# facebookresearch/robust-dynrf

Hardware: AMD Instinct MI355X
Metric: training rays/sec (Nvidia Balloon1, configs/Nvidia.txt, static+dynamic TensorVMSplit) (higher is better)
Workload: dtype f32; 1 GPU; BASELINE.json configs[1]: Nvidia Balloon1, configs/Nvidia.txt, 4096 rays/iter/GPU, 1xMI355X per rank, static+dynamic TensorVMSplit; one step = 5 dynamic + 5 static forward passes, scene-flow MLP, induced flow/disparity, per-frame depth loss, distortion loss, compositor, factor regularisers, full backward, Adam; config=nvidia, stage=stage0, samples_per_ray=115, global_batch=4096, rays_per_gpu=4096, parallelism=ray-sharded dp1, ranks=1, dead_work=executed (work the reference also computes although nothing consumes it)

## Files before the change

### include/rodynrf.h

```cpp
#ifndef RODYNRF_H
#define RODYNRF_H
#include <stddef.h>
#include <stdint.h>

#ifdef __cplusplus
extern "C" {
#endif

#define RDRF_ABI_VERSION 6

typedef void* rdrf_stream_t;

enum { RDRF_RAY_NDC = 0, RDRF_RAY_CONTRACT = 1, RDRF_RAY_OTHER = 2 };
enum { RDRF_ACT_RELU = 0, RDRF_ACT_SOFTPLUS = 1 };
enum { RDRF_HEAD_MLP_FEA = 0, RDRF_HEAD_MLP_FEA_TIMEEMBEDDING = 1 };
enum { RDRF_SCATTER_RAY = 0, RDRF_SCATTER_SORTED = 1, RDRF_SCATTER_AUTO = 2, RDRF_SCATTER_SORTED_PLAIN = 3 };

typedef struct {
  float* plane[3];
  float* line[3];
  int C[3];
  int H[3], W[3];
  int L[3];
  int sH[3], sW[3];
} RdrfVM;

typedef struct {
  float aabb[6];
  float distance_scale;
  float weight_thres;
  float density_shift;
  int act;
  int ray_type;
  int static_head;
} RdrfFieldCfg;

typedef struct {
  RdrfVM density, app;
  float* basis;
  float *w1, *b1;
  float *w2, *b2;
  float *w3, *b3;
  const float* packed_fwd;
  const float* packed_bwd;
} RdrfStaticParams;

typedef struct {
  RdrfVM density, blending, app;
  float* basis;
  float *rw1, *rb1;
  float *rw2, *rb2;
  float *rwv, *rbv;
  float *l1w, *l1b;
  float *l2w, *l2b;
  float *l3w, *l3b;
  float *l4w, *l4b;
  float *l5w, *l5b;
  float *dw1, *db1, *dw2, *db2;
  float *bw1, *bb1, *bw2, *bb2;
  float *sfw[4], *sfb[4];
  const float* packed_fwd;
  const float* packed_bwd;
} RdrfDynamicParams;

int rdrf_abi_version(void);
const char* rdrf_last_error(void);

size_t rdrf_workspace_bytes(int N, int S);
size_t rdrf_forward_workspace_bytes(int N, int S);
size_t rdrf_saved_bytes(int kind, int N, int S);
#define RDRF_SAVE_NO_APP 1
size_t rdrf_saved_bytes_ex(int kind, int N, int S, int flags);
size_t rdrf_saved_row_bytes(int phase);

int rdrf_generate_rays(const int64_t* ids, const float* poses9, const float* focal, int N, int T,
                       int H, int W, int ndc, float near, float* rays, rdrf_stream_t stream);
int rdrf_generate_rays_bwd(const int64_t* ids, const float* poses9, const float* focal, int N,
                           int T, int H, int W, int ndc, float near, const float* grad_rays,
                           float* grad_poses9, float* grad_focal, rdrf_stream_t stream);

int rdrf_generate_rays_uv(const int64_t* ids, const float* uv, int view_shift, const float* poses9,
                          const float* focal, int N, int T, int H, int W, int ndc, float near, float* rays,
                          rdrf_stream_t stream);
int rdrf_generate_rays_uv_bwd(const int64_t* ids, const float* uv, int view_shift, const float* poses9,
                              const float* focal, int N, int T, int H, int W, int ndc, float near,
                              const float* grad_rays, float* grad_poses9, float* grad_focal,
                              rdrf_stream_t stream);

int rdrf_sample_ndc(const float* rays, int N, int S, float near, float far, const float* jitter,
                    const float aabb_host[6], float* xyz, float* z, uint8_t* valid,
                    rdrf_stream_t stream);
int rdrf_sample_contract(const float* rays, int N, int S, float near, float far,
                         const float* jitter_inner, const float* jitter_outer, float* xyz,
                         float* z, uint8_t* valid, rdrf_stream_t stream);
int rdrf_sample_bwd(const float* rays, const float* z, int N, int S, int ray_type,
                    const float* grad_xyz, float* grad_rays, rdrf_stream_t stream);

int rdrf_static_fwd(const RdrfStaticParams* P, const RdrfFieldCfg* cfg, const float* rays,
                    const float* ts, const float* xyz, const float* z, const uint8_t* valid, int N,
                    int S, float* rgb, float* sigma, float* weight, float* dists, void* saved,
                    size_t saved_bytes, void* ws, size_t ws_bytes, rdrf_stream_t stream);
int rdrf_static_fwd_ex(const RdrfStaticParams* P, const RdrfFieldCfg* cfg, const float* rays,
                       const float* ts, const float* xyz, const float* z, const uint8_t* valid, int N,
                       int S, float* rgb, float* sigma, float* weight, float* dists, void* saved,
                       size_t saved_bytes, void* ws, size_t ws_bytes, rdrf_stream_t stream, int flags);
int rdrf_static_bwd(const RdrfStaticParams* P, const RdrfFieldCfg* cfg, const float* rays,
                    const float* ts, const float* xyz, const float* z, const uint8_t* valid, int N,
                    int S, const float* g_rgb, const float* g_sigma, const float* g_weight,
                    const float* g_dists, const RdrfStaticParams* G, float* g_xyz, float* g_z,
                    float* g_rays, void* saved, size_t saved_bytes, void* ws, size_t ws_bytes,
                    rdrf_stream_t stream);

int rdrf_dynamic_fwd(const RdrfDynamicParams* P, const RdrfFieldCfg* cfg, const float* rays,
                     const float* ts, const float* xyz, const float* z, const uint8_t* valid,
                     int N, int S, float* blending, float* weight, float* xyz_prime, float* rgb,
                     float* sigma, float* dists, void* saved, size_t saved_bytes, void* ws,
                     size_t ws_bytes, rdrf_stream_t stream);
int rdrf_dynamic_fwd_ex(const RdrfDynamicParams* P, const RdrfFieldCfg* cfg, const float* rays,
                        const float* ts, const float* xyz, const float* z, const uint8_t* valid,
                        int N, int S, float* blending, float* weight, float* xyz_prime, float* rgb,
                        float* sigma, float* dists, void* saved, size_t saved_bytes, void* ws,
                        size_t ws_bytes, rdrf_stream_t stream, int flags);
int rdrf_dynamic_bwd(const RdrfDynamicParams* P, const RdrfFieldCfg* cfg, const float* rays,
                     const float* ts, const float* xyz, const float* z, const uint8_t* valid,
                     int N, int S, const float* g_blending, const float* g_weight,
                     const float* g_xyz_prime, const float* g_rgb, const float* g_sigma,
                     const float* g_dists, const RdrfDynamicParams* G, float* g_xyz, float* g_z,
                     float* g_rays, void* saved, size_t saved_bytes, void* ws, size_t ws_bytes,
                     rdrf_stream_t stream);

size_t rdrf_features_saved_bytes(int dynamic, int M);
size_t rdrf_features_workspace_bytes(int M);
size_t rdrf_features_bwd_workspace_bytes(int M);
int rdrf_static_features_fwd(const RdrfStaticParams* P, const RdrfFieldCfg* cfg, const float* xn, int M,
                             float* density, float* app, void* saved, size_t saved_bytes, void* ws,
                             size_t ws_bytes, rdrf_stream_t stream);
int rdrf_static_features_bwd(const RdrfStaticParams* P, const RdrfFieldCfg* cfg, const float* xn, int M,
                             const float* g_density, const float* g_app, const RdrfStaticParams* G,
                             float* g_xn, void* saved, size_t saved_bytes, void* ws, size_t ws_bytes,
                             rdrf_stream_t stream);
int rdrf_dynamic_features_fwd(const RdrfDynamicParams* P, const RdrfFieldCfg* cfg, const float* x,
                              const float* t, int M, int x_is_normalized, float* density, float* blending,
                              float* app, float* xyz_prime, void* saved, size_t saved_bytes, void* ws,
                              size_t ws_bytes, rdrf_stream_t stream);
int rdrf_dynamic_features_bwd(const RdrfDynamicParams* P, const RdrfFieldCfg* cfg, const float* x,
                              const float* t, int M, int x_is_normalized, const float* g_density,
                              const float* g_blending, const float* g_app, const float* g_xyz_prime,
                              const RdrfDynamicParams* G, float* g_x, void* saved, size_t saved_bytes,
                              void* ws, size_t ws_bytes, rdrf_stream_t stream);

int rdrf_scene_flow_fwd(const RdrfDynamicParams* P, const RdrfFieldCfg* cfg, const float* pts,
                        const float* ts, int N, int S, float* sf_f, float* sf_b, void* saved,
                        size_t saved_bytes, void* ws, size_t ws_bytes, rdrf_stream_t stream);
int rdrf_scene_flow_bwd(const RdrfDynamicParams* P, const RdrfFieldCfg* cfg, const float* pts,
// ... 212 lines not shown
```

### robust-dynrf_amd/_lib.py

```python
import ctypes as C
import os

import torch

_HERE = os.path.dirname(os.path.abspath(__file__))
DETERMINISTIC = os.environ.get("RDRF_DETERMINISTIC", "0") == "1"
LIB_PATH = os.environ.get("RDRF_LIB", os.path.join(_HERE, "librodynrf_det.so" if DETERMINISTIC else "librodynrf.so"))

ABI_VERSION = 6

RAY_TYPES = {"ndc": 0, "contract": 1}
ACTS = {"relu": 0, "softplus": 1}
HEADS = {"MLP_Fea": 0, "MLP_Fea_TimeEmbedding": 1}
SAVE_NO_APP = 1

fp = C.POINTER(C.c_float)


class RdrfVM(C.Structure):
    _fields_ = [("plane", C.c_void_p * 3), ("line", C.c_void_p * 3), ("C", C.c_int * 3),
                ("H", C.c_int * 3), ("W", C.c_int * 3), ("L", C.c_int * 3),
                ("sH", C.c_int * 3), ("sW", C.c_int * 3)]


class RdrfFieldCfg(C.Structure):
    _fields_ = [("aabb", C.c_float * 6), ("distance_scale", C.c_float), ("weight_thres", C.c_float),
                ("density_shift", C.c_float), ("act", C.c_int), ("ray_type", C.c_int),
                ("static_head", C.c_int)]


class RdrfStaticParams(C.Structure):
    _fields_ = [("density", RdrfVM), ("app", RdrfVM), ("basis", C.c_void_p),
                ("w1", C.c_void_p), ("b1", C.c_void_p), ("w2", C.c_void_p), ("b2", C.c_void_p),
                ("w3", C.c_void_p), ("b3", C.c_void_p), ("packed_fwd", C.c_void_p), ("packed_bwd", C.c_void_p)]


class RdrfDynamicParams(C.Structure):
    _fields_ = [("density", RdrfVM), ("blending", RdrfVM), ("app", RdrfVM), ("basis", C.c_void_p),
                ("rw1", C.c_void_p), ("rb1", C.c_void_p), ("rw2", C.c_void_p), ("rb2", C.c_void_p),
                ("rwv", C.c_void_p), ("rbv", C.c_void_p),
                ("l1w", C.c_void_p), ("l1b", C.c_void_p), ("l2w", C.c_void_p), ("l2b", C.c_void_p),
                ("l3w", C.c_void_p), ("l3b", C.c_void_p), ("l4w", C.c_void_p), ("l4b", C.c_void_p),
                ("l5w", C.c_void_p), ("l5b", C.c_void_p),
                ("dw1", C.c_void_p), ("db1", C.c_void_p), ("dw2", C.c_void_p), ("db2", C.c_void_p),
                ("bw1", C.c_void_p), ("bb1", C.c_void_p), ("bw2", C.c_void_p), ("bb2", C.c_void_p),
                ("sfw", C.c_void_p * 4), ("sfb", C.c_void_p * 4), ("packed_fwd", C.c_void_p), ("packed_bwd", C.c_void_p)]


RENDER_MAPS = ("rgb", "depth", "acc", "rgb_s", "depth_s", "acc_s", "rgb_d", "depth_d", "acc_d", "blending")


class RenderMapsC(C.Structure):
    _fields_ = [(n, C.c_void_p) for n in RENDER_MAPS]


RENDER_MODES = {"auto": 0, "sequence": 1, "fused": 2}

MOTION_MAPS = ("flow_f", "flow_b", "flow_s_f", "flow_s_b", "delta_xyz")


class MotionMapsC(C.Structure):
    _fields_ = [(n, C.c_void_p) for n in MOTION_MAPS]


class MotionCamsC(C.Structure):
    _fields_ = [("H", C.c_int), ("W", C.c_int), ("focal", C.c_void_p), ("c2w_f", C.c_void_p), ("c2w_b", C.c_void_p),
                ("first_pixel", C.c_int64)]


class SceneTablesC(C.Structure):
    _fields_ = [("T", C.c_int), ("H", C.c_int), ("W", C.c_int), ("rgb_u8", C.c_int), ("rgb", C.c_void_p), ("disp", C.c_void_p),
                ("flow_f", C.c_void_p), ("flow_b", C.c_void_p), ("masks", C.c_void_p)]


BATCH_OUTPUTS = ("rgb", "disp", "fg", "mask_f", "mask_b", "flow_f", "flow_b", "ts", "ts_rand", "grid", "px", "view")


class BatchC(C.Structure):
    _fields_ = [(n, C.c_void_p) for n in BATCH_OUTPUTS]


def _load():
    if not os.path.exists(LIB_PATH):
        raise ImportError(
            f"{LIB_PATH} not found: build the HIP library first "
            "(python -c 'import __graft_entry__ as g; g.build()' or make -C robust-dynrf_amd/csrc)")
    lib = C.CDLL(LIB_PATH)
    if not hasattr(lib, "rdrf_abi_version") or lib.rdrf_abi_version() != ABI_VERSION:
        got = lib.rdrf_abi_version() if hasattr(lib, "rdrf_abi_version") else None
        raise ImportError(f"{LIB_PATH}: ABI version {got}, this binding is built against {ABI_VERSION} (include/rodynrf.h): rebuild "
                          "with make -C robust-dynrf_amd/csrc")
    lib.rdrf_last_error.restype = C.c_char_p
    lib.rdrf_workspace_bytes.restype = C.c_size_t
    lib.rdrf_workspace_bytes.argtypes = [C.c_int, C.c_int]
    lib.rdrf_forward_workspace_bytes.restype = C.c_size_t
    lib.rdrf_forward_workspace_bytes.argtypes = [C.c_int, C.c_int]
    lib.rdrf_saved_bytes.restype = C.c_size_t
# ... 173 lines not shown
```

### robust-dynrf_amd/csrc/rdrf_bwd.hip

```cpp
#ifdef RDRF_GROWS_TEMPORAL
#define RDRF_SAVE_TEMPORAL
#endif
#include "rdrf_kernels.hpp"
#ifdef RDRF_NO_BIAS_ATOMICS
#define BIAS_ATOMIC(p, v) ((void)0)
#else
#define BIAS_ATOMIC(p, v) grad_add(p, v)
#endif

namespace pkb {
constexpr int K1H_DEN2 = 0;
constexpr int K1H_BLE2 = K1H_DEN2 + 64;
#ifdef RDRF_HEADS_BWD_F32
constexpr int K1H_DEN1T_F = K1H_BLE2 + 64;
constexpr int K1H_DEN1T_X0 = K1H_DEN1T_F + 3 * 32 * 64;
constexpr int K1H_BLE1T_F = K1H_DEN1T_X0 + 2 * 32 * 64;
constexpr int K1H_BLE1T_X0 = K1H_BLE1T_F + 3 * 32 * 64;
constexpr int K1H_SIZE = K1H_BLE1T_X0 + 2 * 32 * 64;
#else
constexpr int K1H_DEN1T_F = K1H_BLE2 + 64;
constexpr int K1H_DEN1T_X0 = K1H_DEN1T_F + 3 * 32 * 96;
constexpr int K1H_BLE1T_F = K1H_DEN1T_X0 + 2 * 32 * 96;
constexpr int K1H_BLE1T_X0 = K1H_BLE1T_F + 3 * 32 * 96;
constexpr int K1H_SIZE = K1H_BLE1T_X0 + 2 * 32 * 96;
// ... 1458 lines not shown
    const float alpha = 1.0f - expf(-sigma * ds);
    const float p = act ? one_minus_alpha_eps(alpha) : 1.0f;
    float g_alpha = 0.f;
    if (a.g_weight) {
      const float incl = scan_mul32(p, s);
      float excl = __shfl_up(incl, 1, 32);
      if (s == 0) excl = 1.0f;
      const float T = carr[hw][tli] * excl;
      const float gwv = act ? a.g_weight[idx] : 0.f;
      float rinc = gwv * alpha * T;
#pragma unroll
      for (int d = 1; d < 32; d <<= 1) {
        const float o = __shfl_down(rinc, d, 32);
        if (s + d < 32) rinc += o;
      }
      float rex = __shfl_down(rinc, 1, 32);
      if (s == 31) rex = 0.f;
      g_alpha = gwv * T - (sufcarry + rex) / p;
      sufcarry += __shfl(rinc, 0, 32);
    }
    float g_sigma = (act && a.g_sigma) ? a.g_sigma[idx] : 0.f;
    g_sigma += g_alpha * ds * (1.0f - alpha);
    if (act) a.gsig[idx] = g_sigma;
    if ((a.g_rays || a.g_z) && act) {
      const float g_ds = (a.g_dists ? a.g_dists[idx] : 0.f) + g_alpha * sigma * (1.0f - alpha);
      if (a.g_rays) g_nrm += g_ds * ((j + 1 < a.S) ? (zn - zj) : 0.0f) * a.distance_scale;
      if (a.g_z && j + 1 < a.S) {
        const float gz = g_ds * nrm * a.distance_scale;
        atomicAdd(a.g_z + idx, -gz);
        atomicAdd(a.g_z + idx + 1, gz);
      }
    }
  }
  if (a.g_rays && a.ray_type != RDRF_RAY_OTHER) {
#pragma unroll
    for (int d = 16; d >= 1; d >>= 1) g_nrm += __shfl_xor(g_nrm, d, 64);
    if (ray && s < 3) atomicAdd(a.g_rays + (size_t)n * 6 + 3 + s, g_nrm * (s == 0 ? vx : (s == 1 ? vy : vz)));
  }
}

template <int PHASE, bool FEAT, bool FLAT = false>
__global__ __launch_bounds__(64 * RDRF_MAXW) void k_dyn_density_bwd(BwdArgs a, DynW w, DynG gw) {
  static_assert(!(FLAT && FEAT), "feature mode keeps its pseudo-ray geometry (S = 32: a ray is a tile)");
  __shared__ __attribute__((aligned(16))) float lds[PHASE == 0 ? pkb::K1H_SIZE : pkb::K1W_SIZE];
  __shared__ float carr[8][128];
  lds_fill(lds, a.pk + (PHASE == 0 ? pkb::REG_K1H : pkb::REG_K1W), PHASE == 0 ? pkb::K1H_SIZE : pkb::K1W_SIZE);
  const int lane = threadIdx.x & 63, h = lane >> 5, s = lane & 31;
  const int wave = threadIdx.x >> 6, nwaves = blockDim.x >> 6;
  const int tpr = (a.S + 31) >> 5;
  float sw[3] = {0.f, 0.f, 0.f}, sb[3] = {0.f, 0.f, 0.f};
  const int nunits = FLAT ? (a.N * a.S + 31) >> 5 : a.N;
  for (int n = blockIdx.x * nwaves + wave; n < nunits; n += gridDim.x * nwaves) {
    float vx = 0.f, vy = 0.f, vz = 0.f;
    float nrm = 1.0f;
    if constexpr (!FEAT && !FLAT) nrm = ray_norm(a.rays, n, a.ray_type, vx, vy, vz);
    if (!FEAT && !FLAT && PHASE == 0 && a.g_weight) {
      float carry = 1.0f;
      for (int j0 = 0; j0 < a.S; j0 += 32) {
        if (lane == 0) carr[wave][j0 >> 5] = carry;
        const int j = j0 + s;
        const bool act = j < a.S;
        const int idx = n * a.S + (act ? j : 0);
        const bool vld = act && a.valid[idx] != 0;
        const float sigma = vld ? density_act(a.sp.raw[(size_t)idx * 2], a.act, a.density_shift) : 0.f;
        const float zj = act ? a.z[idx] : 0.f;
        const float zn = (j + 1 < a.S) ? a.z[idx + 1] : zj;
        const float ds = ((j + 1 < a.S) ? (zn - zj) : 0.0f) * nrm * a.distance_scale;
        const float alpha = 1.0f - expf(-sigma * ds);
        const float p = act ? one_minus_alpha_eps(alpha) : 1.0f;
        carry *= __shfl(scan_mul32(p, s), 31, 32);
      }
    }
    float sufcarry = 0.f, g_nrm = 0.f;
    float dTacc[16];
#pragma unroll
    for (int i = 0; i < 16; ++i) dTacc[i] = 0.f;
    for (int tli = FLAT ? 0 : tpr - 1; tli >= 0; --tli) {
      const int j0 = tli << 5;
      const int j = j0 + s;
      const bool act = FLAT ? n * 32 + s < a.N * a.S : j < a.S && (!FEAT || n * a.S + j < a.M);
      const int idx = FLAT ? (act ? n * 32 + s : 0) : n * a.S + (act ? j : 0);
      const bool vld = act && (FEAT || a.valid[idx] != 0);
      const size_t tl = FLAT ? (size_t)n : (size_t)n * tpr + tli;
      const float* svb = a.sp.act1 + tl * sv::K1_ROWS * 32;
      float* gb = a.grows1 + tl * sv::K1G_ROWS * 32;
      if (PHASE == 0) {
        float g_fd, g_fb;
        if constexpr (FEAT) {
          g_fd = (act && a.g_sigma) ? a.g_sigma[idx] : 0.f;
          g_fb = (act && a.g_blending) ? a.g_blending[idx] : 0.f;
        } else if constexpr (FLAT) {
          const float fd = a.sp.raw[(size_t)idx * 2], fb = a.sp.raw[(size_t)idx * 2 + 1];
          const float g_sigma = act ? a.gsig[idx] : 0.f;
          g_fd = vld ? g_sigma * act_grad(fd, a.act, a.density_shift) : 0.f;
          const float bl = sigmoidf_(fb);
          g_fb = (vld && a.g_blending) ? a.g_blending[idx] * bl * (1.0f - bl) : 0.f;
        } else {
        const float fd = a.sp.raw[(size_t)idx * 2], fb = a.sp.raw[(size_t)idx * 2 + 1];
        const float sigma = vld ? density_act(fd, a.act, a.density_shift) : 0.f;
        const float zj = act ? a.z[idx] : 0.f;
        const float zn = (j + 1 < a.S) ? a.z[idx + 1] : zj;
        const float ds = ((j + 1 < a.S) ? (zn - zj) : 0.0f) * nrm * a.distance_scale;
        const float alpha = 1.0f - expf(-sigma * ds);
        const float p = act ? one_minus_alpha_eps(alpha) : 1.0f;
        float g_alpha = 0.f;
        if (a.g_weight) {
          const float incl = scan_mul32(p, s);
          float excl = __shfl_up(incl, 1, 32);
          if (s == 0) excl = 1.0f;
          const float T = carr[wave][tli] * excl;
          const float gwv = act ? a.g_weight[idx] : 0.f;
          float rinc = gwv * alpha * T;
#pragma unroll
          for (int d = 1; d < 32; d <<= 1) {
            const float o = __shfl_down(rinc, d, 32);
            if (s + d < 32) rinc += o;
          }
          float rex = __shfl_down(rinc, 1, 32);
          if (s == 31) rex = 0.f;
          g_alpha = gwv * T - (sufcarry + rex) / p;
          sufcarry += __shfl(rinc, 0, 32);
        }
        float g_sigma = (act && a.g_sigma) ? a.g_sigma[idx] : 0.f;
        g_sigma += g_alpha * ds * (1.0f - alpha);
        if ((a.g_rays || a.g_z) && act && h == 0) {
          const float g_ds = (a.g_dists ? a.g_dists[idx] : 0.f) + g_alpha * sigma * (1.0f - alpha);
          if (a.g_rays) g_nrm += g_ds * ((j + 1 < a.S) ? (zn - zj) : 0.0f) * a.distance_scale;
          if (a.g_z && j + 1 < a.S) {
            const float gz = g_ds * nrm * a.distance_scale;
            atomicAdd(a.g_z + idx, -gz);
            atomicAdd(a.g_z + idx + 1, gz);
          }
        }
        g_fd = vld ? g_sigma * act_grad(fd, a.act, a.density_shift) : 0.f;
        const float bl = sigmoidf_(fb);
        g_fb = (vld && a.g_blending) ? a.g_blending[idx] * bl * (1.0f - bl) : 0.f;
        }
        f32x16 accX[2];
        acc_zero<2>(accX);
        const bool live_d = FEAT ? a.g_sigma != nullptr : (a.g_sigma != nullptr || a.g_weight != nullptr);
        const bool live_b = a.g_blending != nullptr;
#pragma unroll
        for (int head = 0; head < 2; ++head) {
          if (!(head == 0 ? live_d : live_b)) continue;
          const float gfh = head == 0 ? g_fd : g_fb;
          float Hh[32], dzh[32];
          load_rows<32>(svb, head == 0 ? sv::K1_HD : sv::K1_HB, Hh, s, h);
          const float* w2 = lds + (head == 0 ? pkb::K1H_DEN2 : pkb::K1H_BLE2) + h * 32;
          float w2r[32];
#pragma unroll
          for (int q = 0; q < 8; ++q) {
            const f32x4 v = *reinterpret_cast<const f32x4*>(w2 + 4 * q);
            w2r[4 * q] = v.x; w2r[4 * q + 1] = v.y; w2r[4 * q + 2] = v.z; w2r[4 * q + 3] = v.w;
          }
#pragma unroll
          for (int kk = 0; kk < 32; ++kk) dzh[kk] = Hh[kk] > 0.f ? w2r[kk] * gfh : 0.f;
          save_rows<32>(gb, head == 0 ? sv::K1G_DZD : sv::K1G_DZB, dzh, s, h);
          if (!FEAT && a.small_dw) {
            float pw[32];
#pragma unroll
            for (int kk = 0; kk < 32; ++kk) pw[kk] = gfh * Hh[kk];
            sw[head] += reduce_scatter32(pw, s);
            sb[head] += gfh;
          }
          f32x16 accF[3];
          acc_zero<3>(accF);
#ifdef RDRF_HEADS_BWD_F32
// ... 1116 lines not shown
    hipLaunchKernelGGL(k_sort_keys, dim3((unsigned)g), dim3(256), 0, stream, ka);
    rdrf_prof_end("sort_keys", stream);
  }
  int rc = rdrf_sort_positions(b.keys_in, b.keys_out, b.order, (unsigned)(3 * ns), kb + 2, b.sort_tmp, b.sort_tmp_bytes, stream,
                               ka.compact ? ka.count : nullptr, 3u);
  if (rc) return rc;
  hipLaunchKernelGGL(k_sort_counts, dim3(1), dim3(64), 0, stream, (const unsigned*)b.keys_out, (int)ns, kb, b.counts,
                     ka.compact ? ka.count : (const int*)nullptr);
  rdrf_prof_end("scatter_sort", stream);
  RDRF_HIP(hipGetLastError());
  return 0;
}

static int scatter_dyn_app_sorted(const BwdArgs& a, const BwdWs& b, const RdrfDynamicParams* P, const RdrfDynamicParams* G,
                                  hipStream_t stream) {
  const size_t ns = (size_t)a.N * a.S;
  SortKeyArgs ka;
  memset(&ka, 0, sizeof(ka));
  ka.list = a.sp.list; ka.count = &a.sp.hdr->count;
#ifdef RDRF_TOOLS
  static const int compact_env = RDRF_ENV("RDRF_SORT_COMPACT") ? atoi(RDRF_ENV("RDRF_SORT_COMPACT")) : 1;
  ka.compact = compact_env && !(RDRF_ENV("RDRF_SS_TILED") && atoi(RDRF_ENV("RDRF_SS_TILED")) >= 2);
#else
  ka.compact = 1;
#endif
  int rc = sorted_scatter_prepare(ka, P->app, a, b, stream);
  if (rc) return rc;
  SortedScatterArgs sa;
  memset(&sa, 0, sizeof(sa));
  sa.vm[0] = P->app; sa.gvm[0] = G->app;
  sa.set_mask = 1; sa.dfs = b.dfa; sa.rec_floats = DFA_FLOATS; sa.list = a.sp.list; sa.xw = a.sp.xw; sa.dxw = b.dxw;
  for (int p = 0; p < 3; ++p) {
    sa.order = b.order + (size_t)p * ns; sa.count = b.counts + p; sa.base = (unsigned)(p * ns);
    if (ka.compact) { sa.order = b.order; sa.seg = ka.count; }
    const unsigned* ks = b.keys_out + (size_t)p * ns;
#ifdef RDRF_TOOLS
    rc = p == 0 ? launch_scatter_tiled<0, 12, 3>(sa, ks, ka.kb, (long)ns, stream)
                : (p == 1 ? launch_scatter_tiled<1, 12, 3>(sa, ks, ka.kb, (long)ns, stream)
                          : launch_scatter_tiled<2, 12, 3>(sa, ks, ka.kb, (long)ns, stream));
    if (rc < 0) return rc;
    if (rc == 1) continue;
#else
    (void)ks;
#endif
    rc = p == 0 ? launch_scatter_sorted<0, 12, 3>(sa, (long)ns, stream)
                : (p == 1 ? launch_scatter_sorted<1, 12, 3>(sa, (long)ns, stream) : launch_scatter_sorted<2, 12, 3>(sa, (long)ns, stream));
    if (rc) return rc;
  }
  return 0;
}

static int scatter_dyn_density_sorted(const BwdArgs& a, const BwdWs& b, const RdrfDynamicParams* P, const RdrfDynamicParams* G,
                                      int set_mask, hipStream_t stream) {
  const size_t ns = (size_t)a.N * a.S;
  for (int p = 0; p < 3; ++p)
    RDRF_CHECK(P->blending.W[p] == P->density.W[p] && P->blending.H[p] == P->density.H[p], -1,
               "sorted scatter: density and blending planes differ in size");
  SortKeyArgs ka;
  memset(&ka, 0, sizeof(ka));
  ka.grows1 = b.grows1;
  ka.flat = rdrf_flat_density() ? 1 : 0;
  int rc = sorted_scatter_prepare(ka, P->density, a, b, stream);
  if (rc) return rc;
  SortedScatterArgs sa;
  memset(&sa, 0, sizeof(sa));
  sa.vm[0] = P->density; sa.gvm[0] = G->density; sa.vm[1] = P->blending; sa.gvm[1] = G->blending;
  sa.set_mask = set_mask; sa.dfs = b.dfs; sa.rec_floats = DFS_FLOATS; sa.xw = a.sp.xw; sa.dxw = b.dxw;
  for (int p = 0; p < 3; ++p) {
    sa.order = b.order + (size_t)p * ns; sa.count = b.counts + p; sa.base = (unsigned)(p * ns);
    const unsigned* ks = b.keys_out + (size_t)p * ns;
    rc = p == 0 ? launch_scatter_tiled<0, 4, 1>(sa, ks, ka.kb, (long)ns, stream)
                : (p == 1 ? launch_scatter_tiled<1, 4, 1>(sa, ks, ka.kb, (long)ns, stream)
                          : launch_scatter_tiled<2, 4, 1>(sa, ks, ka.kb, (long)ns, stream));
    if (rc < 0) return rc;
    if (rc == 1) continue;
    rc = p == 0 ? launch_scatter_sorted<0, 4, 1>(sa, (long)ns, stream)
                : (p == 1 ? launch_scatter_sorted<1, 4, 1>(sa, (long)ns, stream) : launch_scatter_sorted<2, 4, 1>(sa, (long)ns, stream));
    if (rc) return rc;
  }
  return 0;
}

static void add_density_phase_dw(DwJobs& D, const float* grows1, const float* act1, const RdrfDynamicParams* G,
                                 int T1, bool live_d = true, bool live_b = true, bool small_in_kernel = false) {
  dw_add(D, grows1, sv::K1G_ROWS, sv::K1G_DZ3, 2, 64, 0, act1, sv::K1_ROWS, 93, 93, G->l3w, G->l3b, nullptr, T1);
  dw_blk(D, sv::K1_X0, SEG_WARP3_X0, 0);
  dw_blk(D, sv::K1_X0 + 32, SEG_WARP3_X0, 32);
  dw_blk(D, sv::K1_T, SEG_WARP3_T, 0);
  dw_add(D, grows1, sv::K1G_ROWS, sv::K1G_DZ4, 2, 64, 0, act1, sv::K1_ROWS, 64, 64, G->l4w, G->l4b, nullptr, T1);
  dw_blk(D, sv::K1_H3, SEG_IDENT, 0);
  dw_blk(D, sv::K1_H3 + 32, SEG_IDENT, 32);
  if (!small_in_kernel) {
  dw_add(D, grows1, sv::K1G_ROWS, sv::K1G_SM, 1, 3, 0, act1, sv::K1_ROWS, 64, 64, G->l5w, G->l5b, nullptr, T1);
  dw_blk(D, sv::K1_H4, SEG_IDENT, 0);
  dw_blk(D, sv::K1_H4 + 32, SEG_IDENT, 32);
  if (live_d) {
    dw_add(D, grows1, sv::K1G_ROWS, sv::K1G_SM, 1, 1, 3, act1, sv::K1_ROWS, 64, 64, G->dw2, G->db2, nullptr, T1);
    dw_blk(D, sv::K1_HD, SEG_IDENT, 0);
    dw_blk(D, sv::K1_HD + 32, SEG_IDENT, 32);
  }
  if (live_b) {
    dw_add(D, grows1, sv::K1G_ROWS, sv::K1G_SM, 1, 1, 4, act1, sv::K1_ROWS, 64, 64, G->bw2, G->bb2, nullptr, T1);
    dw_blk(D, sv::K1_HB, SEG_IDENT, 0);
    dw_blk(D, sv::K1_HB + 32, SEG_IDENT, 32);
  }
  }
  for (int head = 0; head < 2; ++head) {
    if (!(head ? live_b : live_d)) continue;
    dw_add(D, grows1, sv::K1G_ROWS, head ? sv::K1G_DZB : sv::K1G_DZD, 2, 64, 0, act1, sv::K1_ROWS, 152, 152,
           head ? G->bw1 : G->dw1, head ? G->bb1 : G->db1, nullptr, T1);
    const int f0 = head ? sv::K1_FB : sv::K1_FD;
    dw_blk(D, f0, SEG_IDENT72, 0);
    dw_blk(D, f0 + 32, SEG_IDENT72, 32);
    dw_blk(D, f0 + 64, SEG_IDENT72, 64);
    dw_blk(D, sv::K1_X0, SEG_DEN1_X0, 0);
    dw_blk(D, sv::K1_X0 + 32, SEG_DEN1_X0, 32);
    dw_blk(D, sv::K1_X1, SEG_DEN1_X1, 0);
  }
}

extern "C" int rdrf_static_bwd(const RdrfStaticParams* P, const RdrfFieldCfg* cfg, const float* rays,
                               const float* ts, const float* xyz, const float* z,
                               const uint8_t* valid, int N, int S, const float* g_rgb,
                               const float* g_sigma, const float* g_weight, const float* g_dists,
                               const RdrfStaticParams* G, float* g_xyz, float* g_z, float* g_rays,
                               void* saved, size_t saved_bytes, void* ws, size_t ws_bytes,
                               rdrf_stream_t stream_) {
  hipStream_t stream = (hipStream_t)stream_;
  if (N == 0) return 0;
  RDRF_CHECK(P && cfg && G && saved && N > 0 && S > 0 && S <= 4096, -1, "static_bwd: bad arguments (S <= 4096)");
  RDRF_CHECK((size_t)N * S * 3 < (size_t)INT32_MAX, -1, "static_bwd: N * S * 3 must stay below 2^31 (32-bit sample indices)");
  BwdArgs a;
  fill_bwd_common(a, cfg, rays, ts, xyz, z, valid, N, S);
  a.g_rgb = g_rgb; a.g_sigma = g_sigma; a.g_weight = g_weight; a.g_xyz = g_xyz;
  a.g_rays = g_rays; a.g_dists = g_dists; a.g_z = g_z;
  const int saved_kind = carve_saved_bwd(a.sp, saved, saved_bytes, 0, N, S);
  RDRF_CHECK(saved_kind >= 0, -3, "static_bwd: saved buffer too small");
  RDRF_CHECK(saved_kind == 1 || g_rgb == nullptr, -1,
             "static_bwd: the forward saved no appearance rows (RDRF_SAVE_NO_APP): no gradient can flow through rgb");
  BwdWs b;
  int rc = carve_bwd(b, ws, ws_bytes, N, S, 0);
  if (rc) return rc;
  a.pk = b.pk; a.grows3 = b.grows3;
  StaticW w;
  fill_static_w(w, P);
  StaticG gw;
  gw.density = G->density; gw.app = G->app; gw.b3 = G->b3; gw.w3 = G->w3;
  if (P->packed_bwd != nullptr) a.pk = P->packed_bwd;
  else {
    PackJobs J;
    static_pack_jobs_bwd(J, P, cfg->static_head);
    rc = pack_launch(J, b.pk, stream);
    if (rc) return rc;
  }
  const size_t t3 = ((size_t)N * S + 31) / 32;
  if (g_rgb != nullptr) {
    const Geo g = geo_for_units((long)t3);
    if (cfg->static_head == RDRF_HEAD_MLP_FEA)
      RDRF_LAUNCH("static_app_bwd", (k_static_app_bwd<RDRF_HEAD_MLP_FEA, false>), dim3(g.grid), dim3(g.block),
                  stream, a, w, gw);
    else
      RDRF_LAUNCH("static_app_bwd", (k_static_app_bwd<RDRF_HEAD_MLP_FEA_TIMEEMBEDDING, false>), dim3(g.grid),
                  dim3(g.block), stream, a, w, gw);
    {
      ScatterArgs sa;
      fill_scatter_common(sa, a);
      sa.vm[0] = P->app; sa.gvm[0] = G->app; sa.nsets = 1;
      sa.rows = b.grows3; sa.stride = sv::K3G_ROWS; sa.row0[0] = sv::K3G_DA;
      sa.list = a.sp.list; sa.count = &a.sp.hdr->count;
      sa.g_xyz = g_xyz;
      { int rc_ = launch_scatter("scatter_static_app", k_scatter<12, 3, 9>, sa, (long)t3, stream); if (rc_) return rc_; }
    }
    const bool fea = cfg->static_head == RDRF_HEAD_MLP_FEA;
    const int in1 = fea ? 138 : 135;
    const int* cnt = &a.sp.hdr->count;
    DwJobs D;
    D.n = 0;
    dw_add(D, b.grows3, sv::K3G_ROWS, sv::K3G_DZV, 1, 3, 0, a.sp.act3, sv::S3_ROWS, 128,
           fea ? 128 : 131, G->w3, G->b3, cnt, 0);
    for (int i = 0; i < 4; ++i) dw_blk(D, sv::S3_H2 + 32 * i, SEG_IDENT, 32 * i);
    if (!fea) dw_blk(D, sv::S3_VD, SEG_VIEW3, 0);
    dw_add(D, b.grows3, sv::K3G_ROWS, sv::K3G_DF, 1, 27, 0, a.sp.act3, sv::S3_ROWS, 72, 72, G->basis,
           nullptr, cnt, 0);
    for (int i = 0; i < 3; ++i) dw_blk(D, sv::S3_G + 32 * i, SEG_IDENT, 32 * i);
    dw_add(D, b.grows3, sv::K3G_ROWS, sv::K3G_DZ2, 4, 128, 0, a.sp.act3, sv::S3_ROWS, 128, 128, G->w2,
           G->b2, cnt, 0);
    for (int i = 0; i < 4; ++i) dw_blk(D, sv::S3_H1 + 32 * i, SEG_IDENT, 32 * i);
    dw_add(D, b.grows3, sv::K3G_ROWS, sv::K3G_DZ1, 4, 128, 0, a.sp.act3, sv::S3_ROWS, in1, in1, G->w1,
           G->b1, cnt, 0);
    dw_blk(D, sv::S3_F, fea ? SEG_STAT1_F_FEA : SEG_STAT1_F_TE, 0);
    for (int i = 0; i < 4; ++i) dw_blk(D, sv::S3_P + 32 * i, fea ? SEG_STAT1_P_FEA : SEG_STAT1_P_TE, 32 * i);
    rc = dw_launch(D, stream, "dw_static");
    if (rc) return rc;
  }
  if (g_sigma != nullptr || g_weight != nullptr || ((g_rays != nullptr || g_z != nullptr) && g_dists != nullptr)) {
    RDRF_LAUNCH("static_density_bwd", k_static_density_bwd, dim3(N), dim3(64), stream, a, w, b.gf);
    if (g_sigma != nullptr || g_weight != nullptr) {
      ScatterArgs sa;
      fill_scatter_common(sa, a);
      sa.vm[0] = P->density; sa.gvm[0] = G->density; sa.nsets = 1;
      sa.rows = b.gf; sa.stride = 1; sa.row0[0] = 0; sa.bcast = 1;
      sa.g_xyz = g_xyz;
      const long t1 = (long)N * ((S + 31) / 32);
      { int rc_ = launch_scatter("scatter_static_density", k_scatter<4, 1, 3>, sa, t1, stream); if (rc_) return rc_; }
    }
  }
  return 0;
}

extern "C" int rdrf_dynamic_bwd(const RdrfDynamicParams* P, const RdrfFieldCfg* cfg,
                                const float* rays, const float* ts, const float* xyz,
                                const float* z, const uint8_t* valid, int N, int S,
                                const float* g_blending, const float* g_weight,
                                const float* g_xyz_prime, const float* g_rgb, const float* g_sigma,
                                const float* g_dists, const RdrfDynamicParams* G, float* g_xyz,
                                float* g_z, float* g_rays, void* saved, size_t saved_bytes, void* ws,
                                size_t ws_bytes, rdrf_stream_t stream_) {
  hipStream_t stream = (hipStream_t)stream_;
  if (N == 0) return 0;
  RDRF_CHECK(P && cfg && G && saved && N > 0 && S > 0 && S <= 4096, -1, "dynamic_bwd: bad arguments (S <= 4096)");
  RDRF_CHECK((size_t)N * S * 3 < (size_t)INT32_MAX, -1, "dynamic_bwd: N * S * 3 must stay below 2^31 (32-bit sample indices)");
  BwdArgs a;
  fill_bwd_common(a, cfg, rays, ts, xyz, z, valid, N, S);
  a.g_rgb = g_rgb; a.g_sigma = g_sigma; a.g_weight = g_weight; a.g_blending = g_blending;
  a.g_xyz_prime = g_xyz_prime; a.g_xyz = g_xyz; a.g_rays = g_rays; a.g_dists = g_dists; a.g_z = g_z;
  static const bool small_dw = !(RDRF_ENV("RDRF_DW_SMALL") && atoi(RDRF_ENV("RDRF_DW_SMALL")) == 0);
  a.small_dw = small_dw ? 1 : 0;
  const int saved_kind = carve_saved_bwd(a.sp, saved, saved_bytes, 1, N, S);
  RDRF_CHECK(saved_kind >= 0, -3, "dynamic_bwd: saved buffer too small");
  RDRF_CHECK(saved_kind == 1 || g_rgb == nullptr, -1,
             "dynamic_bwd: the forward saved no appearance rows (RDRF_SAVE_NO_APP): no gradient can flow through rgb");
  BwdWs b;
  int rc = carve_bwd(b, ws, ws_bytes, N, S, 1);
  if (rc) return rc;
  a.pk = b.pk; a.grows1 = b.grows1; a.grows3 = b.grows3; a.dxw_app = b.dxw; a.dxn_app = b.dxn;
  a.dtout = b.dtout;
  const bool flat = rdrf_flat_density();
  a.gsig = b.gsig; a.dtp = b.dtp;
  DynW w;
  fill_dyn_w(w, P);
  DynG gw;
  gw.density = G->density; gw.blending = G->blending; gw.app = G->app;
  gw.rbv = G->rbv; gw.rwv = G->rwv; gw.l5b = G->l5b; gw.db2 = G->db2; gw.bb2 = G->bb2;
  gw.l5w = G->l5w; gw.dw2 = G->dw2; gw.bw2 = G->bw2;
  if (P->packed_bwd != nullptr) a.pk = P->packed_bwd;
  else {
    PackJobs J;
    dyn_pack_jobs_bwd(J, P);
    rc = pack_launch(J, b.pk, stream);
    if (rc) return rc;
  }
  const size_t ns = (size_t)N * S, t3 = (ns + 31) / 32, t1 = flat ? t3 : (size_t)N * ((S + 31) / 32);
  RDRF_FILL(b.dxw, 0, ns * 3 * 4, stream);
  RDRF_FILL(b.dxn, 0, ns * 3 * 4, stream);
  const int* cnt = &a.sp.hdr->count;
  DwJobs D;
  D.n = 0;
  if (g_rgb != nullptr) {
    const Geo g = geo_for_units((long)t3);
    const int smode_app = scatter_mode(ns, stream);
    a.dfa = smode_app != 0 ? b.dfa : nullptr;
    if (smode_app != 0) RDRF_LAUNCH("dyn_app_bwd", (k_dyn_app_bwd<false, true>), dim3(g.grid), dim3(g.block), stream, a, w, gw);
    else RDRF_LAUNCH("dyn_app_bwd", (k_dyn_app_bwd<false, false>), dim3(g.grid), dim3(g.block), stream, a, w, gw);
    if (smode_app != 0) {
      rdrf_prof_begin("scatter_dyn_app", stream);
      rc = scatter_dyn_app_sorted(a, b, P, G, stream);
      rdrf_prof_end("scatter_dyn_app", stream);
      if (rc) return rc;
    } else {
      ScatterArgs sa;
      fill_scatter_common(sa, a);
      sa.vm[0] = P->app; sa.gvm[0] = G->app; sa.nsets = 1;
      sa.rows = b.grows3; sa.stride = sv::K3G_ROWS; sa.row0[0] = sv::K3G_DA;
      sa.xw = a.sp.xw; sa.list = a.sp.list; sa.count = cnt;
      sa.dxw = b.dxw; sa.dxw_accumulate = 0;
      { int rc_ = launch_scatter("scatter_dyn_app", k_scatter<12, 3, 27>, sa, (long)t3, stream); if (rc_) return rc_; }
    }
    dw_add(D, b.grows3, sv::K3G_ROWS, sv::K3G_DZV, 1, 3, 0, a.sp.act3, sv::K3_ROWS, 128, 131, G->rwv,
           G->rbv, cnt, 0);
    for (int i = 0; i < 4; ++i) dw_blk(D, sv::K3_H2 + 32 * i, SEG_IDENT, 32 * i);
    dw_blk(D, sv::K3_VD, SEG_VIEW3, 0);
    dw_add(D, b.grows3, sv::K3G_ROWS, sv::K3G_DF, 1, 27, 0, a.sp.act3, sv::K3_ROWS, 216, 216, G->basis,
           nullptr, cnt, 0);
    for (int i = 0; i < 7; ++i) dw_blk(D, sv::K3_A + 32 * i, SEG_IDENT, 32 * i);
    dw_add(D, b.grows3, sv::K3G_ROWS, sv::K3G_DZ2, 4, 128, 0, a.sp.act3, sv::K3_ROWS, 128, 128, G->rw2,
           G->rb2, cnt, 0);
    for (int i = 0; i < 4; ++i) dw_blk(D, sv::K3_H1 + 32 * i, SEG_IDENT, 32 * i);
    dw_add(D, b.grows3, sv::K3G_ROWS, sv::K3G_DZ1, 4, 128, 0, a.sp.act3, sv::K3_ROWS, 107, 107, G->rw1,
           G->rb1, cnt, 0);
    dw_blk(D, sv::K3_F, SEG_RGB1_F, 0);
    dw_blk(D, sv::K3_X0, SEG_RGB1_X0, 0);
    dw_blk(D, sv::K3_X0 + 32, SEG_RGB1_X0, 32);
    dw_blk(D, sv::K3_X1, SEG_RGB1_X1, 0);
  }
  {
    const Geo g = geo_for_units(flat ? (long)t1 : (long)N);
    const int smode = scatter_mode(ns, stream);
    a.dfs = smode != 0 ? b.dfs : nullptr;
    if (flat) {
      RDRF_LAUNCH("ray_scan_bwd", k_ray_scan_bwd, dim3((N + 15) / 16), dim3(512), stream, a);
      RDRF_LAUNCH("dyn_heads_bwd", (k_dyn_density_bwd<0, false, true>), dim3(g.grid), dim3(g.block), stream, a, w, gw);
    } else RDRF_LAUNCH("dyn_heads_bwd", (k_dyn_density_bwd<0, false>), dim3(g.grid), dim3(g.block), stream, a, w, gw);
    if (smode != 0) {
      const int set_mask = ((g_sigma != nullptr || g_weight != nullptr) ? 1 : 0) | (g_blending != nullptr ? 2 : 0);
      if (set_mask != 0) {
        rdrf_prof_begin("scatter_dyn_density", stream);
        rc = scatter_dyn_density_sorted(a, b, P, G, set_mask, stream);
        rdrf_prof_end("scatter_dyn_density", stream);
        if (rc) return rc;
      }
    } else {
      const bool has_d = g_sigma != nullptr || g_weight != nullptr, has_b = g_blending != nullptr;
      if (has_d || has_b) {
        ScatterArgs sa;
        fill_scatter_common(sa, a);
        sa.nsets = 0;
        if (has_d) { sa.vm[sa.nsets] = P->density; sa.gvm[sa.nsets] = G->density; sa.row0[sa.nsets] = sv::K1G_DFD; ++sa.nsets; }
        if (has_b) { sa.vm[sa.nsets] = P->blending; sa.gvm[sa.nsets] = G->blending; sa.row0[sa.nsets] = sv::K1G_DFB; ++sa.nsets; }
        sa.rows = b.grows1; sa.stride = sv::K1G_ROWS; sa.flat = flat ? 1 : 0;
        sa.xw = a.sp.xw;
        sa.dxw = b.dxw; sa.dxw_accumulate = 1;
        { int rc_ = launch_scatter("scatter_dyn_density", k_scatter<4, 1, 9>, sa, (long)t1, stream); if (rc_) return rc_; }
      }
    }
    if (flat) RDRF_LAUNCH("dyn_warp_bwd", (k_dyn_density_bwd<1, false, true>), dim3(g.grid), dim3(g.block), stream, a, w, gw);
    else RDRF_LAUNCH("dyn_warp_bwd", (k_dyn_density_bwd<1, false>), dim3(g.grid), dim3(g.block), stream, a, w, gw);
    RDRF_LAUNCH("time_branch_bwd", k_time_branch_bwd, dim3((N + TB_RPB - 1) / TB_RPB), dim3(128), stream, ts, w,
                N, b.dtout, flat ? (const float*)b.dtp : nullptr, S, G->l1w, G->l1b, G->l2w, G->l2b);
    const bool small_in_kernel = a.small_dw != 0;
    add_density_phase_dw(D, b.grows1, a.sp.act1, G, (int)t1, g_sigma != nullptr || g_weight != nullptr, g_blending != nullptr,
                         small_in_kernel);
  }
  rc = dw_launch(D, stream, "dw_dyn");
  return rc;
}

struct FeatWs {
  float *pk, *grows3, *grows1, *dxw, *dxn, *dtout, *gpad, *xpad;
  uint8_t* valid;
};
static int carve_feat_bwd(FeatWs& b, void* ws, size_t ws_bytes, int M, int dynamic) {
  WsCarver c(ws, ws_bytes);
  const size_t t = ((size_t)M + 31) / 32, mp = t * 32;
  b.pk = c.take<float>(PACK_AREA_FLOATS);
  b.grows3 = c.take<float>(t * sv::K3G_ROWS * 32);
  b.grows1 = dynamic ? c.take<float>(t * sv::K1G_ROWS * 32) : nullptr;
  b.dxw = dynamic ? c.take<float>(mp * 3) : nullptr;
  b.dxn = dynamic ? c.take<float>(mp * 3) : nullptr;
  b.dtout = dynamic ? c.take<float>(mp * 32) : nullptr;
  b.gpad = dynamic ? nullptr : c.take<float>(mp);
  b.xpad = dynamic ? nullptr : c.take<float>(mp * 3);
  b.valid = c.take<uint8_t>(mp);
  RDRF_CHECK(c.ok(), -3, "features backward: workspace too small: need %zu have %zu", c.off, ws_bytes);
  return 0;
}
extern "C" size_t rdrf_features_bwd_workspace_bytes(int M) {
  const size_t t = ((size_t)M + 31) / 32, mp = t * 32;
  return (size_t)PACK_AREA_FLOATS * 4 + t * (sv::K3G_ROWS + sv::K1G_ROWS) * 32 * 4 + mp * (6 + 32 + 4) * 4 + mp +
         (1 << 14);
}

extern "C" int rdrf_static_features_bwd(const RdrfStaticParams* P, const RdrfFieldCfg* cfg, const float* xn,
                                        int M, const float* g_density, const float* g_app,
                                        const RdrfStaticParams* G, float* g_xn, void* saved, size_t saved_bytes,
                                        void* ws, size_t ws_bytes, rdrf_stream_t stream_) {
  hipStream_t stream = (hipStream_t)stream_;
  if (M == 0) return 0;
  RDRF_CHECK(P && cfg && G && xn && M > 0 && (g_density || g_app), -1, "static_features_bwd: bad arguments");
  RDRF_CHECK(g_app == nullptr || saved != nullptr, -1, "static_features_bwd: the appearance features need the "
             "saved buffer of their forward call");
  const int Np = (M + 31) / 32;
  const size_t mp = (size_t)Np * 32;
  FeatWs b;
  int rc = carve_feat_bwd(b, ws, ws_bytes, M, 0);
  if (rc) return rc;
  BwdArgs a;
  fill_bwd_common(a, cfg, nullptr, nullptr, xn, nullptr, b.valid, Np, 32);
  a.M = M; a.in_norm = 1; a.g_feat = g_app; a.pk = b.pk; a.grows3 = b.grows3;
  if (saved != nullptr)
    RDRF_CHECK(carve_saved_feat(a.sp, saved, saved_bytes, 0, M), -3, "static_features_bwd: saved buffer too small");
  RDRF_FILL(b.valid, 0, mp, stream);
  RDRF_FILL(b.valid, 1, (size_t)M, stream);
  RDRF_FILL(b.xpad, 0, mp * 3 * 4, stream);
  RDRF_HIP(hipMemcpyAsync(b.xpad, xn, (size_t)M * 3 * 4, hipMemcpyDeviceToDevice, stream));
  ScatterArgs sa0;
  fill_scatter_common(sa0, a);
  sa0.xw = b.xpad;
  sa0.box.inv[0] = sa0.box.inv[1] = sa0.box.inv[2] = 1.0f;
  sa0.g_xyz = g_xn;
  if (g_density != nullptr) {
    RDRF_FILL(b.gpad, 0, mp * 4, stream);
    RDRF_HIP(hipMemcpyAsync(b.gpad, g_density, (size_t)M * 4, hipMemcpyDeviceToDevice, stream));
    ScatterArgs sa = sa0;
    sa.vm[0] = P->density; sa.gvm[0] = G->density; sa.nsets = 1;
    sa.rows = b.gpad; sa.stride = 1; sa.row0[0] = 0; sa.bcast = 1;
    { int rc_ = launch_scatter("feat_scatter_static_density", k_scatter<4, 1, 3>, sa, (long)Np, stream); if (rc_) return rc_; }
  }
  if (g_app != nullptr) {
    StaticW w;
    fill_static_w(w, P);
    StaticG gw;
    gw.density = G->density; gw.app = G->app; gw.b3 = G->b3; gw.w3 = G->w3;
    if (P->packed_bwd != nullptr) a.pk = P->packed_bwd;
    else {
      PackJobs J;
      static_pack_jobs_bwd(J, P, cfg->static_head);
      rc = pack_launch(J, b.pk, stream);
      if (rc) return rc;
    }
    const Geo g = geo_for_units(Np);
    RDRF_LAUNCH("feat_static_app_bwd", (k_static_app_bwd<RDRF_HEAD_MLP_FEA, true>), dim3(g.grid), dim3(g.block),
                stream, a, w, gw);
    ScatterArgs sa = sa0;
    sa.vm[0] = P->app; sa.gvm[0] = G->app; sa.nsets = 1;
    sa.rows = b.grows3; sa.stride = sv::K3G_ROWS; sa.row0[0] = sv::K3G_DA;
    { int rc_ = launch_scatter("feat_scatter_static_app", k_scatter<12, 3, 9>, sa, (long)Np, stream); if (rc_) return rc_; }
    DwJobs D;
    D.n = 0;
    dw_add(D, b.grows3, sv::K3G_ROWS, sv::K3G_DF, 1, 27, 0, a.sp.act3, sv::S3_ROWS, 72, 72, G->basis, nullptr,
           nullptr, Np);
    for (int i = 0; i < 3; ++i) dw_blk(D, sv::S3_G + 32 * i, SEG_IDENT, 32 * i);
    rc = dw_launch(D, stream, "feat_dw_static");
    if (rc) return rc;
  }
  return 0;
}

extern "C" int rdrf_dynamic_features_bwd(const RdrfDynamicParams* P, const RdrfFieldCfg* cfg, const float* x,
                                         const float* t, int M, int x_is_normalized, const float* g_density,
                                         const float* g_blending, const float* g_app, const float* g_xyz_prime,
                                         const RdrfDynamicParams* G, float* g_x, void* saved, size_t saved_bytes,
                                         void* ws, size_t ws_bytes, rdrf_stream_t stream_) {
  hipStream_t stream = (hipStream_t)stream_;
  if (M == 0) return 0;
  RDRF_CHECK(P && cfg && G && x && t && saved && M > 0 && (g_density || g_blending || g_app || g_xyz_prime), -1,
             "dynamic_features_bwd: bad arguments");
  const int Np = (M + 31) / 32;
  const size_t mp = (size_t)Np * 32;
  FeatWs b;
  int rc = carve_feat_bwd(b, ws, ws_bytes, M, 1);
  if (rc) return rc;
  BwdArgs a;
  fill_bwd_common(a, cfg, nullptr, t, x, nullptr, b.valid, Np, 32);
  a.M = M; a.in_norm = x_is_normalized ? 1 : 0;
  a.g_sigma = g_density; a.g_blending = g_blending; a.g_feat = g_app; a.g_xyz_prime = g_xyz_prime; a.g_xyz = g_x;
  RDRF_CHECK(carve_saved_feat(a.sp, saved, saved_bytes, 1, M), -3, "dynamic_features_bwd: saved buffer too small");
  a.pk = b.pk; a.grows1 = b.grows1; a.grows3 = b.grows3; a.dxw_app = b.dxw; a.dxn_app = b.dxn; a.dtout = b.dtout;
  DynW w;
  fill_dyn_w(w, P);
  DynG gw;
  gw.density = G->density; gw.blending = G->blending; gw.app = G->app;
  gw.rbv = G->rbv; gw.rwv = G->rwv; gw.l5b = G->l5b; gw.db2 = G->db2; gw.bb2 = G->bb2;
  gw.l5w = G->l5w; gw.dw2 = G->dw2; gw.bw2 = G->bw2;
  if (P->packed_bwd != nullptr) a.pk = P->packed_bwd;
  else {
    PackJobs J;
    dyn_pack_jobs_bwd(J, P);
    rc = pack_launch(J, b.pk, stream);
    if (rc) return rc;
  }
  RDRF_FILL(b.valid, 0, mp, stream);
  RDRF_FILL(b.valid, 1, (size_t)M, stream);
  RDRF_FILL(b.dxw, 0, mp * 3 * 4, stream);
  RDRF_FILL(b.dxn, 0, mp * 3 * 4, stream);
  const Geo g = geo_for_units(Np);
  DwJobs D;
  D.n = 0;
  if (g_app != nullptr) {
    RDRF_LAUNCH("feat_dyn_app_bwd", k_dyn_app_bwd<true>, dim3(g.grid), dim3(g.block), stream, a, w, gw);
    ScatterArgs sa;
    fill_scatter_common(sa, a);
    sa.vm[0] = P->app; sa.gvm[0] = G->app; sa.nsets = 1;
    sa.rows = b.grows3; sa.stride = sv::K3G_ROWS; sa.row0[0] = sv::K3G_DA;
    sa.xw = a.sp.xw;
    sa.dxw = b.dxw; sa.dxw_accumulate = 0;
    { int rc_ = launch_scatter("feat_scatter_dyn_app", k_scatter<12, 3, 27>, sa, (long)Np, stream); if (rc_) return rc_; }
    dw_add(D, b.grows3, sv::K3G_ROWS, sv::K3G_DF, 1, 27, 0, a.sp.act3, sv::K3_ROWS, 216, 216, G->basis, nullptr,
           nullptr, Np);
    for (int i = 0; i < 7; ++i) dw_blk(D, sv::K3_A + 32 * i, SEG_IDENT, 32 * i);
  }
  RDRF_LAUNCH("feat_dyn_heads_bwd", (k_dyn_density_bwd<0, true>), dim3(g.grid), dim3(g.block), stream, a, w, gw);
  if (g_density != nullptr || g_blending != nullptr) {
    ScatterArgs sa;
    fill_scatter_common(sa, a);
    sa.nsets = 0;
    if (g_density != nullptr) { sa.vm[sa.nsets] = P->density; sa.gvm[sa.nsets] = G->density; sa.row0[sa.nsets] = sv::K1G_DFD; ++sa.nsets; }
    if (g_blending != nullptr) { sa.vm[sa.nsets] = P->blending; sa.gvm[sa.nsets] = G->blending; sa.row0[sa.nsets] = sv::K1G_DFB; ++sa.nsets; }
    sa.rows = b.grows1; sa.stride = sv::K1G_ROWS;
    sa.xw = a.sp.xw;
    sa.dxw = b.dxw; sa.dxw_accumulate = 1;
    { int rc_ = launch_scatter("feat_scatter_dyn_density", k_scatter<4, 1, 9>, sa, (long)Np, stream); if (rc_) return rc_; }
  }
  RDRF_LAUNCH("feat_dyn_warp_bwd", (k_dyn_density_bwd<1, true>), dim3(g.grid), dim3(g.block), stream, a, w, gw);
  RDRF_LAUNCH("time_branch_bwd", k_time_branch_bwd, dim3((M + TB_RPB - 1) / TB_RPB), dim3(128), stream, t, w, M,
              b.dtout, (const float*)nullptr, 32, G->l1w, G->l1b, G->l2w, G->l2b);
  add_density_phase_dw(D, b.grows1, a.sp.act1, G, Np, g_density != nullptr, g_blending != nullptr);
  return dw_launch(D, stream, "feat_dw_dyn");
}

extern "C" int rdrf_scene_flow_bwd(const RdrfDynamicParams* P, const RdrfFieldCfg* cfg,
                                   const float* pts, const float* ts, int N, int S,
                                   const float* g_sf_f, const float* g_sf_b,
                                   const RdrfDynamicParams* G, float* g_pts, void* saved,
                                   size_t saved_bytes, void* ws, size_t ws_bytes,
                                   rdrf_stream_t stream_) {
  hipStream_t stream = (hipStream_t)stream_;
  if (N == 0) return 0;
  RDRF_CHECK(P && cfg && G && saved && N > 0 && S > 0, -1, "scene_flow_bwd: bad arguments");
  RDRF_CHECK((size_t)N * S * 3 < (size_t)INT32_MAX, -1, "scene_flow_bwd: N * S * 3 must stay below 2^31 (32-bit sample indices)");
  const size_t tiles = ((size_t)N * S + 31) / 32;
  RDRF_CHECK(saved_bytes >= tiles * sv::SF_ROWS * 32 * 4, -3, "scene_flow_bwd: saved buffer too small");
  WsCarver c(ws, ws_bytes);
  float* pkbuf = c.take<float>(PACK_AREA_FLOATS);
  float* grows = c.take<float>(tiles * sv::SFG_ROWS * 32);
  RDRF_CHECK(c.ok(), -3, "scene_flow_bwd: workspace too small: need %zu have %zu", c.off, ws_bytes);
  const float* pkimg = pkbuf;
  int rc = 0;
  if (P->packed_bwd != nullptr) pkimg = P->packed_bwd;
  else {
    PackJobs J;
    dyn_pack_jobs_bwd(J, P);
    rc = pack_launch(J, pkbuf, stream);
    if (rc) return rc;
  }
  const Geo g = geo_for_units((long)tiles);
  RDRF_LAUNCH("scene_flow_bwd", k_scene_flow_bwd, dim3(g.grid), dim3(g.block), stream, N, S,
              make_box(cfg), pkimg, (const float*)saved, grows, g_sf_f, g_sf_b, G->sfb[3], g_pts);
  const float* act = (const float*)saved;
  const int T = (int)tiles;
  DwJobs D;
  D.n = 0;
  dw_add(D, grows, sv::SFG_ROWS, sv::SFG_DZ6, 1, 6, 0, act, sv::SF_ROWS, 64, 64, G->sfw[3], G->sfb[3],
         nullptr, T);
  dw_blk(D, sv::SF_H4, SEG_IDENT, 0);
  dw_blk(D, sv::SF_H4 + 32, SEG_IDENT, 32);
  dw_add(D, grows, sv::SFG_ROWS, sv::SFG_DZ4, 2, 64, 0, act, sv::SF_ROWS, 64, 64, G->sfw[2], G->sfb[2],
         nullptr, T);
  dw_blk(D, sv::SF_H2, SEG_IDENT, 0);
  dw_blk(D, sv::SF_H2 + 32, SEG_IDENT, 32);
  dw_add(D, grows, sv::SFG_ROWS, sv::SFG_DZ2, 2, 64, 0, act, sv::SF_ROWS, 64, 64, G->sfw[1], G->sfb[1],
         nullptr, T);
  dw_blk(D, sv::SF_H0, SEG_IDENT, 0);
  dw_blk(D, sv::SF_H0 + 32, SEG_IDENT, 32);
  dw_add(D, grows, sv::SFG_ROWS, sv::SFG_DZ0, 2, 64, 0, act, sv::SF_ROWS, 36, 36, G->sfw[0], G->sfb[0],
         nullptr, T);
  dw_blk(D, sv::SF_X, SEG_SF_X, 0);
  dw_blk(D, sv::SF_X + 32, SEG_SF_X, 32);
  return dw_launch(D, stream, "dw_sf");
}

#define GRB_LDS_POSES 448
__global__ __launch_bounds__(256) void k_generate_rays_bwd(const int64_t* __restrict__ ids, const float* __restrict__ uv, int view_shift,
                                    const float* __restrict__ poses9,
                                    const float* __restrict__ focal_p, int N, int T, int H, int W,
                                    int ndc, float near, const float* __restrict__ g_rays,
                                    float* __restrict__ g_poses, float* __restrict__ g_focal) {
  __shared__ float s_gp[GRB_LDS_POSES * 9];
  __shared__ float s_gf[4];
  const bool in_lds = T <= GRB_LDS_POSES;
  if (in_lds) {
    for (int i = threadIdx.x; i < T * 9; i += blockDim.x) s_gp[i] = 0.f;
    __syncthreads();
  }
  const int n = blockIdx.x * blockDim.x + threadIdx.x;
  float gf = 0.f;
  if (n < N) {
    const long id = ids[n];
    const int col = (int)(id % W), row = (int)((id / W) % H);
    int view = (int)(id / ((long)W * H)) + view_shift;
    view = view < 0 ? 0 : (view >= T ? T - 1 : view);
    const float f = focal_p[0];
    const float pu = uv ? uv[2 * n] : (float)col + 0.5f, pv = uv ? uv[2 * n + 1] : (float)row + 0.5f;
    const float dir[3] = {(pu - 0.5f * W) / f, -(pv - 0.5f * H) / f, -1.0f};
    const float* p = poses9 + view * 9;
    float b1[3] = {p[0], p[1], p[2]};
    const float n1 = sqrtf(b1[0] * b1[0] + b1[1] * b1[1] + b1[2] * b1[2]);
    for (int k = 0; k < 3; ++k) b1[k] /= n1;
    const float dt = b1[0] * p[3] + b1[1] * p[4] + b1[2] * p[5];
    float u[3] = {p[3] - dt * b1[0], p[4] - dt * b1[1], p[5] - dt * b1[2]};
// ... 156 lines not shown
```

### robust-dynrf_amd/csrc/rdrf_fwd.hip

```cpp
#include "rdrf_fwd_dev.hpp"

template <bool FEAT>
__global__ __launch_bounds__(256) __attribute__((amdgpu_waves_per_eu(5, 8))) void k_static_density(FieldArgs a, StaticW w) { static_density_body<FEAT>(a, w, grid_ctx()); }

template <int HEAD, bool FEAT, bool SAVE = true>
__global__ __launch_bounds__(64 * RDRF_MAXW) void k_static_app(FieldArgs a, StaticW w) {
  static_app_body<HEAD, FEAT, SAVE>(a, w, nullptr, grid_ctx());
}

#ifdef RDRF_TOOLS
template <int HEAD, bool SAVE>
__global__ __launch_bounds__(1024) void k_static_app16(FieldArgs a, StaticW w) { static_app16_body<HEAD, SAVE>(a, w); }
#endif

template <bool FEAT, bool SAVE = true>
__global__ __launch_bounds__(64 * RDRF_MAXW) void k_dyn_density(FieldArgs a, DynW w) {
  dyn_density_body<FEAT, SAVE>(a, w, nullptr, grid_ctx());
}

template <bool FEAT, bool SAVE = true>
__global__ __launch_bounds__(64 * RDRF_MAXW) void k_dyn_app(FieldArgs a, DynW w) {
  dyn_app_body<FEAT, SAVE>(a, w, nullptr, grid_ctx());
}

__global__ __launch_bounds__(256) void k_time_branch(const float* __restrict__ ts, DynW w, int N,
                                                     float* __restrict__ tout, int* __restrict__ zero64) {
  __shared__ float s_h[8 * 64];
  if (zero64 != nullptr && blockIdx.x == 0 && threadIdx.x < 64) zero64[threadIdx.x] = 0;
  time_branch_body(ts, w, N, tout, s_h, grid_ctx());
}

template <bool SAVE>
__global__ __launch_bounds__(64 * RDRF_MAXW) void k_dyn_density_flat(FieldArgs a, DynW w) {
  dyn_density_body<false, SAVE, false, true>(a, w, nullptr, grid_ctx());
}
__global__ __launch_bounds__(512) void k_ray_scan(FieldArgs a) { ray_scan_body(a); }

__global__ __launch_bounds__(64 * RDRF_MAXW) void k_scene_flow(const float* __restrict__ pts,
                                                   const float* __restrict__ ts, int N, int S,
                                                   Box box, const float* __restrict__ pkg, DynW w,
                                                   float* __restrict__ sf_f,
                                                   float* __restrict__ sf_b,
                                                   float* __restrict__ act_rows, int dynq) {
  __shared__ __attribute__((aligned(16))) float lds[pk::SF_SIZE];
  __shared__ int s_next;
  if (threadIdx.x == 0) s_next = blockDim.x >> 6;
  lds_fill(lds, pkg + pk::REG_SF, pk::SF_SIZE);
  const int lane = threadIdx.x & 63, h = lane >> 5, s = lane & 31;
  const int wave = threadIdx.x >> 6, nwaves = blockDim.x >> 6;
  const float* pkw = lds;
  const int total = N * S;
  const int ntiles = (total + 31) >> 5;
  for (int k = wave, tile; (tile = blockIdx.x + k * gridDim.x) < ntiles; k = tile_queue_next(&s_next, k, nwaves, dynq != 0)) {
    const int li = tile * 32 + s;
    const bool act = li < total;
    const int idx = act ? li : 0;
    const float t = ts[idx / S];
    const float xn0 = norm_c(pts[(size_t)idx * 3 + 0], box.lo[0], box.inv[0]);
    const float xn1 = norm_c(pts[(size_t)idx * 3 + 1], box.lo[1], box.inv[1]);
    const float xn2 = norm_c(pts[(size_t)idx * 3 + 2], box.lo[2], box.inv[2]);
    float X[20];
    fill_sf_x(X, xn0, xn1, xn2, t, h);
    float* svb = act_rows ? act_rows + (size_t)tile * sv::SF_ROWS * 32 : nullptr;
    save_rows<20>(svb, sv::SF_X, X, s, h);
    f32x16 acc[2];
    acc_bias<2>(acc, pkw + pk::SF_B0, h);
    mfma_seg<2, 20>(acc, X, pkw + pk::SF_W0, lane);
    float H[32];
    acc_relu<2>(H, acc);
    save_rows<32>(svb, sv::SF_H0, H, s, h);
    acc_bias<2>(acc, pkw + pk::SF_B2, h);
    mfma_seg<2, 32>(acc, H, pkw + pk::SF_W2, lane);
    acc_relu<2>(H, acc);
    save_rows<32>(svb, sv::SF_H2, H, s, h);
    acc_bias<2>(acc, pkw + pk::SF_B4, h);
    mfma_seg<2, 32>(acc, H, pkw + pk::SF_W4, lane);
    acc_relu<2>(H, acc);
    save_rows<32>(svb, sv::SF_H4, H, s, h);
#pragma unroll
    for (int o = 0; o < 6; ++o) {
      const float v = dot_small<32>(H, pkw + pk::SF_W6 + o * 64, h) + w.sfb6[o];
      if (act && h == 0) {
        if (o < 3) sf_f[(size_t)idx * 3 + o] = v;
        else sf_b[(size_t)idx * 3 + (o - 3)] = v;
      }
    }
  }
}

void fill_common(FieldArgs& a, const RdrfFieldCfg* cfg, const float* rays, const float* ts,
                        const float* xyz, const float* z, const uint8_t* valid, int N, int S) {
  memset(&a, 0, sizeof(a));
  a.rays = rays; a.ts = ts; a.xyz = xyz; a.z = z; a.valid = valid;
  a.N = N; a.S = S;
  a.box = make_box(cfg);
  a.distance_scale = cfg->distance_scale;
  a.weight_thres = cfg->weight_thres;
  a.density_shift = cfg->density_shift;
  a.act = cfg->act;
  a.ray_type = cfg->ray_type;
  a.static_head = cfg->static_head;
}

void dyn_pack_jobs_fwd(PackJobs& J, const RdrfDynamicParams* P) {
  using namespace pk;
  J.n = 0;
  const int k1 = REG_K1, k3 = REG_K3, sf = REG_SF;
  pack_add(J, P->l3w, 93, 64, 93, SEG_WARP3_X0, 0, 2, 32, k1 + K1_W3_X0);
  pack_add(J, P->l3w, 93, 64, 93, SEG_WARP3_T, 0, 2, 16, k1 + K1_W3_T);
  pack_add(J, P->l4w, 64, 64, 64, SEG_IDENT, 0, 2, 32, k1 + K1_W4);
  pack_add(J, P->l5w, 64, 3, 64, SEG_IDENT, 1, 3, 32, k1 + K1_W5);
#ifdef RDRF_HEADS_F32
  pack_add(J, P->dw1, 152, 64, 72, SEG_IDENT, 0, 2, 36, k1 + K1_DEN1_F);
  pack_add(J, P->dw1, 152, 64, 152, SEG_DEN1_X0, 0, 2, 32, k1 + K1_DEN1_X0);
  pack_add(J, P->dw1, 152, 64, 152, SEG_DEN1_X1, 0, 2, 8, k1 + K1_DEN1_X1);
  pack_add(J, P->bw1, 152, 64, 72, SEG_IDENT, 0, 2, 36, k1 + K1_BLE1_F);
  pack_add(J, P->bw1, 152, 64, 152, SEG_DEN1_X0, 0, 2, 32, k1 + K1_BLE1_X0);
  pack_add(J, P->bw1, 152, 64, 152, SEG_DEN1_X1, 0, 2, 8, k1 + K1_BLE1_X1);
#else
  for (int head = 0; head < 2; ++head) {
    const float* w1 = head == 0 ? P->dw1 : P->bw1;
    const int img = k1 + (head == 0 ? K1_DEN1 : K1_BLE1), tail = k1 + (head == 0 ? K1_DEN1_X1T : K1_BLE1_X1T);
    pack_add_b3(J, w1, 152, 64, 72, SEG_IDENT, 2, 36, 0, 0, K1_HEAD_KK, img);
    pack_add_b3(J, w1, 152, 64, 152, SEG_DEN1_X0, 2, 32, 0, 36, K1_HEAD_KK, img);
    pack_add_b3(J, w1, 152, 64, 152, SEG_DEN1_X1, 2, 4, 0, 68, K1_HEAD_KK, img);
    pack_add_from(J, w1, 152, 64, 152, SEG_DEN1_X1, 2, 4, 4, tail);
  }
#endif
  pack_add(J, P->dw2, 64, 1, 64, SEG_IDENT, 1, 1, 32, k1 + K1_DEN2);
  pack_add(J, P->bw2, 64, 1, 64, SEG_IDENT, 1, 1, 32, k1 + K1_BLE2);
  pack_add(J, P->l3b, 0, 64, 0, 0, 3, 0, 32, k1 + K1_B3);
  pack_add(J, P->l4b, 0, 64, 0, 0, 3, 0, 32, k1 + K1_B4);
  pack_add(J, P->db1, 0, 64, 0, 0, 3, 0, 32, k1 + K1_BD1);
  pack_add(J, P->bb1, 0, 64, 0, 0, 3, 0, 32, k1 + K1_BB1);
  pack_add(J, P->basis, 216, 27, 216, SEG_IDENT, 0, 1, 108, k3 + K3_BASIS);
#ifdef RDRF_APP_F32
  pack_add(J, P->rw1, 107, 128, 107, SEG_RGB1_F, 0, 4, 16, k3 + K3_RGB1_F);
  pack_add(J, P->rw1, 107, 128, 107, SEG_RGB1_X0, 0, 4, 32, k3 + K3_RGB1_X0);
  pack_add(J, P->rw1, 107, 128, 107, SEG_RGB1_X1, 0, 4, 8, k3 + K3_RGB1_X1);
  pack_add(J, P->rw2, 128, 128, 128, SEG_IDENT, 0, 4, 64, k3 + K3_RGB2);
#else
  pack_add_b3s(J, P->rw1, 107, 128, 107, SEG_RGB1_F, 4, 16, 0, 0, 16, k3 + K3_RGB1_F, REG_K3_LO + K3_LO_RGB1_F);
  pack_add_b3s(J, P->rw1, 107, 128, 107, SEG_RGB1_X0, 4, 32, 0, 0, 32, k3 + K3_RGB1_X0, REG_K3_LO + K3_LO_RGB1_X0);
  pack_add_b3s(J, P->rw1, 107, 128, 107, SEG_RGB1_X1, 4, 8, 0, 0, 8, k3 + K3_RGB1_X1, REG_K3_LO + K3_LO_RGB1_X1);
  pack_add_b3s(J, P->rw2, 128, 128, 128, SEG_IDENT, 4, 64, 0, 0, 64, k3 + K3_RGB2, REG_K3_LO + K3_LO_RGB2);
#endif
  pack_add(J, P->rwv, 131, 3, 128, SEG_IDENT, 1, 3, 64, k3 + K3_RGBV);
  pack_add(J, P->rb1, 0, 128, 0, 0, 3, 0, 64, k3 + K3_B1);
  pack_add(J, P->rb2, 0, 128, 0, 0, 3, 0, 64, k3 + K3_B2);
  pack_add(J, P->sfw[0], 36, 64, 36, SEG_SF_X, 0, 2, 20, sf + SF_W0);
  pack_add(J, P->sfw[1], 64, 64, 64, SEG_IDENT, 0, 2, 32, sf + SF_W2);
  pack_add(J, P->sfw[2], 64, 64, 64, SEG_IDENT, 0, 2, 32, sf + SF_W4);
  pack_add(J, P->sfw[3], 64, 6, 64, SEG_IDENT, 1, 6, 32, sf + SF_W6);
  pack_add(J, P->sfb[0], 0, 64, 0, 0, 3, 0, 32, sf + SF_B0);
  pack_add(J, P->sfb[1], 0, 64, 0, 0, 3, 0, 32, sf + SF_B2);
  pack_add(J, P->sfb[2], 0, 64, 0, 0, 3, 0, 32, sf + SF_B4);
}

void static_pack_jobs_fwd(PackJobs& J, const RdrfStaticParams* P, int head) {
  using namespace pk;
  J.n = 0;
  const bool fea = head == RDRF_HEAD_MLP_FEA;
  const int in1 = fea ? 138 : 135;
  pack_add(J, P->basis, 72, 27, 72, SEG_IDENT, 0, 1, 36, REG_S3 + S3_BASIS);
#ifdef RDRF_APP_F32
  pack_add(J, P->w1, in1, 128, in1, fea ? SEG_STAT1_F_FEA : SEG_STAT1_F_TE, 0, 4, 16, REG_S3 + S3_W1_F);
  pack_add(J, P->w1, in1, 128, in1, fea ? SEG_STAT1_P_FEA : SEG_STAT1_P_TE, 0, 4, 64, REG_S3 + S3_W1_P);
  pack_add(J, P->w2, 128, 128, 128, SEG_IDENT, 0, 4, 64, REG_S3 + S3_W2);
#else
  pack_add_b3s(J, P->w1, in1, 128, in1, fea ? SEG_STAT1_F_FEA : SEG_STAT1_F_TE, 4, 16, 0, 0, 16, REG_S3 + S3_W1_F, REG_S3_LO + S3_LO_W1_F);
  pack_add_b3s(J, P->w1, in1, 128, in1, fea ? SEG_STAT1_P_FEA : SEG_STAT1_P_TE, 4, 64, 0, 0, 64, REG_S3 + S3_W1_P, REG_S3_LO + S3_LO_W1_P);
  pack_add_b3s(J, P->w2, 128, 128, 128, SEG_IDENT, 4, 64, 0, 0, 64, REG_S3 + S3_W2, REG_S3_LO + S3_LO_W2);
#endif
  pack_add(J, P->w3, fea ? 128 : 131, 3, 128, SEG_IDENT, 1, 3, 64, REG_S3 + S3_W3);
  pack_add(J, P->b1, 0, 128, 0, 0, 3, 0, 64, REG_S3 + S3_B1);
  pack_add(J, P->b2, 0, 128, 0, 0, 3, 0, 64, REG_S3 + S3_B2);
#ifdef RDRF_TOOLS
  pack_add(J, P->basis, 72, 27, 72, SEG16_APP_G, 4, 2, 20, REG_S16 + S16_BASIS);
  pack_add(J, P->w1, in1, 128, in1, fea ? SEG_STAT1_F_FEA : SEG_STAT1_F_TE, 4, 8, 8, REG_S16 + S16_W1_F);
  pack_add(J, P->w1, in1, 128, in1, fea ? SEG_STAT1_P_FEA : SEG_STAT1_P_TE, 4, 8, 32, REG_S16 + S16_W1_P);
  pack_add(J, P->w2, 128, 128, 128, SEG_IDENT, 4, 8, 32, REG_S16 + S16_W2);
  pack_add(J, P->w3, fea ? 128 : 131, 3, 128, SEG_IDENT, 5, 3, 32, REG_S16 + S16_W3);
  pack_add(J, P->b1, 0, 128, 0, 0, 6, 0, 32, REG_S16 + S16_B1);
  pack_add(J, P->b2, 0, 128, 0, 0, 6, 0, 32, REG_S16 + S16_B2);
#endif
}

void fill_static_w(StaticW& w, const RdrfStaticParams* P) {
  w.density = P->density; w.app = P->app;
  w.b1 = P->b1; w.b2 = P->b2; w.b3 = P->b3; w.w3 = P->w3;
}
void fill_dyn_w(DynW& w, const RdrfDynamicParams* P) {
  w.density = P->density; w.blending = P->blending; w.app = P->app;
  w.l1w = P->l1w; w.l1b = P->l1b; w.l2w = P->l2w; w.l2b = P->l2b;
  w.l3b = P->l3b; w.l4b = P->l4b; w.l5b = P->l5b;
  w.db1 = P->db1; w.db2 = P->db2; w.bb1 = P->bb1; w.bb2 = P->bb2;
  w.rb1 = P->rb1; w.rb2 = P->rb2; w.rbv = P->rbv; w.rwv = P->rwv;
  w.sfb0 = P->sfb[0]; w.sfb2 = P->sfb[1]; w.sfb4 = P->sfb[2]; w.sfb6 = P->sfb[3];
}

#define PACK_AREA_FLOATS (1 << 20)


static int ws_carve_fwd_ex(FieldArgs& a, void* ws, size_t ws_bytes, int N, int S, void* saved,
                           size_t saved_bytes, int dynamic, int flags) {
  WsCarver c(ws, ws_bytes);
  size_t ns = (size_t)N * S;
  a.pk = c.take<float>(PACK_AREA_FLOATS);
  a.counter = c.take<int>(64);
  a.tout = c.take<float>((size_t)N * 32);
  a.xw = c.take<float>(ns * 3);
  a.list = c.take<int>(ns);
  RDRF_CHECK(c.ok(), -3, "workspace too small: need %zu have %zu", c.off, ws_bytes);
  if (saved != nullptr) {
    SavedPtrs sp;
    RDRF_CHECK(carve_saved(sp, saved, saved_bytes, dynamic, N, S, flags), -3,
               "saved buffer too small: need %zu have %zu", saved_bytes_field(dynamic, N, S, flags),
               saved_bytes);
    a.counter = &sp.hdr->count;
    a.list = sp.list;
    a.xw = sp.xw;
    a.tout = sp.tout;
    a.raw = sp.raw;
    a.act1 = sp.act1;
    a.act3 = sp.act3;
  }
  return 0;
}

int ws_carve_fwd(FieldArgs& a, void* ws, size_t ws_bytes, int N, int S, void* saved,
                 size_t saved_bytes, int dynamic) {
  return ws_carve_fwd_ex(a, ws, ws_bytes, N, S, saved, saved_bytes, dynamic, 0);
}

extern "C" size_t rdrf_saved_bytes_ex(int kind, int N, int S, int flags) {
  if (kind == 2) return ((size_t)N * S + 31) / 32 * sv::SF_ROWS * 32 * 4 + 256;
  return saved_bytes_field(kind == 1, N, S, flags);
}
extern "C" size_t rdrf_saved_bytes(int kind, int N, int S) { return rdrf_saved_bytes_ex(kind, N, S, 0); }

extern "C" size_t rdrf_saved_row_bytes(int phase) {
  return (size_t)4 * (phase == 0 ? sv::K1_ROWS : phase == 1 ? sv::K3_ROWS : phase == 2 ? sv::S3_ROWS : sv::SF_ROWS);
}

struct Geo {
  int grid, block;
};
#ifndef RDRF_GEO_TPW_DEFAULT
#define RDRF_GEO_TPW_DEFAULT 1
#endif
static Geo geo_for_units(long units) {
  Geo g;
  const int ncu = 256;
  int waves = (int)((units + ncu - 1) / ncu);
  waves = waves < 1 ? 1 : (waves > RDRF_MAXW ? RDRF_MAXW : waves);
  g.block = waves * 64;
  static const int tpw_env = RDRF_ENV("RDRF_GEO_TPW") ? atoi(RDRF_ENV("RDRF_GEO_TPW")) : RDRF_GEO_TPW_DEFAULT;
  const long per_block = (long)waves * (tpw_env < 1 ? 1 : tpw_env);
  long blocks = (units + per_block - 1) / per_block;
  g.grid = (int)(blocks < 1 ? 1 : (blocks > ncu ? ncu : blocks));
  return g;
}
static Geo geo_for_tiles(int N, int S) { return geo_for_units(((long)N * S + 31) / 32); }

#ifndef RDRF_DYNQ_DEFAULT
#define RDRF_DYNQ_DEFAULT 1
#endif
#ifndef RDRF_WPRIO_DEFAULT
#define RDRF_WPRIO_DEFAULT 0
#endif
#ifndef RDRF_STAGGER_DEFAULT
#define RDRF_STAGGER_DEFAULT 0
#endif
int fwd_dynq() {
  static const int dynq = RDRF_ENV("RDRF_DYNQ") ? atoi(RDRF_ENV("RDRF_DYNQ")) : RDRF_DYNQ_DEFAULT;
  static const int wprio = RDRF_ENV("RDRF_WPRIO") ? atoi(RDRF_ENV("RDRF_WPRIO")) : RDRF_WPRIO_DEFAULT;
  static const int stagger = RDRF_ENV("RDRF_STAGGER") ? atoi(RDRF_ENV("RDRF_STAGGER")) : RDRF_STAGGER_DEFAULT;
  return (dynq ? 1 : 0) | (wprio ? 2 : 0) | (stagger << 8);
}

extern "C" int rdrf_static_fwd_ex(const RdrfStaticParams* P, const RdrfFieldCfg* cfg, const float* rays,
                                  const float* ts, const float* xyz, const float* z,
                                  const uint8_t* valid, int N, int S, float* rgb, float* sigma,
                                  float* weight, float* dists, void* saved, size_t saved_bytes,
                                  void* ws, size_t ws_bytes, rdrf_stream_t stream_, int flags) {
  hipStream_t stream = (hipStream_t)stream_;
  if (N == 0) return 0;
  RDRF_CHECK(P && cfg && N > 0 && S > 0, -1, "static_fwd: bad arguments");
  RDRF_CHECK((flags & ~RDRF_SAVE_NO_APP) == 0, -1, "static_fwd: unknown flags 0x%x", flags);
  RDRF_CHECK((size_t)N * S * 3 < (size_t)INT32_MAX, -1, "static_fwd: N * S * 3 must stay below 2^31 (32-bit sample indices): render / train in smaller chunks");
  RDRF_CHECK(vm_ok(P->density, 16, 4) && vm_ok(P->app, 48, 12), -1,
             "static_fwd: only density comps {16,4,4} / app comps {48,12,12}, the planes and lines of a set spanning one grid, are built");
  FieldArgs a;
  fill_common(a, cfg, rays, ts, xyz, z, valid, N, S);
  a.rgb = rgb; a.sigma = sigma; a.weight = weight; a.dists = dists;
  int rc = ws_carve_fwd_ex(a, ws, ws_bytes, N, S, saved, saved_bytes, 0, flags);
  if (rc) return rc;
  const bool save_app = saved != nullptr && !(flags & RDRF_SAVE_NO_APP);
  StaticW w;
  fill_static_w(w, P);
  if (P->packed_fwd != nullptr) a.pk = P->packed_fwd;
  else {
    PackJobs J;
    static_pack_jobs_fwd(J, P, cfg->static_head);
    rc = pack_launch(J, (float*)a.pk, stream);
    if (rc) return rc;
  }
  RDRF_FILL(a.counter, 0, 256, stream);
#ifdef RDRF_DETERMINISTIC
  RDRF_FILL(a.list, 0x7f, (size_t)N * S * sizeof(int), stream);
#endif
  RDRF_LAUNCH("static_density", k_static_density<false>, dim3((N + 3) / 4), dim3(256), stream, a, w);
  if (rgb == nullptr) return 0;
#ifdef RDRF_DETERMINISTIC
  { int rc_ = rdrf_sort_ints_inplace(a.list, (unsigned)((size_t)N * S), stream); if (rc_) return rc_; }
#endif
  const Geo g = geo_for_tiles(N, S);
  const bool fea = cfg->static_head == RDRF_HEAD_MLP_FEA;
  a.dynq = fwd_dynq();
#ifdef RDRF_TOOLS
  static const int sa16 = RDRF_ENV("RDRF_SA16") ? atoi(RDRF_ENV("RDRF_SA16")) : 0;
  if (sa16) {
    const long t16 = (((long)N * S + 31) / 32) * 2;
    int waves = (int)((t16 + 255) / 256);
    waves = waves < 1 ? 1 : (waves > 16 ? 16 : waves);
    const long blocks = (t16 + waves - 1) / waves;
    const dim3 gr((unsigned)(blocks > 256 ? 256 : blocks)), bl(waves * 64);
    if (save_app) {
      if (fea) RDRF_LAUNCH("static_app", (k_static_app16<RDRF_HEAD_MLP_FEA, true>), gr, bl, stream, a, w);
      else RDRF_LAUNCH("static_app", (k_static_app16<RDRF_HEAD_MLP_FEA_TIMEEMBEDDING, true>), gr, bl, stream, a, w);
    } else {
      if (fea) RDRF_LAUNCH("static_app", (k_static_app16<RDRF_HEAD_MLP_FEA, false>), gr, bl, stream, a, w);
      else RDRF_LAUNCH("static_app", (k_static_app16<RDRF_HEAD_MLP_FEA_TIMEEMBEDDING, false>), gr, bl, stream, a, w);
    }
    return 0;
  }
#endif
  if (save_app) {
    if (fea) RDRF_LAUNCH("static_app", (k_static_app<RDRF_HEAD_MLP_FEA, false, true>), dim3(g.grid), dim3(g.block), stream, a, w);
    else RDRF_LAUNCH("static_app", (k_static_app<RDRF_HEAD_MLP_FEA_TIMEEMBEDDING, false, true>), dim3(g.grid), dim3(g.block), stream, a, w);
  } else {
    if (fea) RDRF_LAUNCH("static_app", (k_static_app<RDRF_HEAD_MLP_FEA, false, false>), dim3(g.grid), dim3(g.block), stream, a, w);
    else RDRF_LAUNCH("static_app", (k_static_app<RDRF_HEAD_MLP_FEA_TIMEEMBEDDING, false, false>), dim3(g.grid), dim3(g.block), stream, a, w);
  }
  return 0;
}

extern "C" int rdrf_static_fwd(const RdrfStaticParams* P, const RdrfFieldCfg* cfg, const float* rays,
                               const float* ts, const float* xyz, const float* z,
                               const uint8_t* valid, int N, int S, float* rgb, float* sigma,
                               float* weight, float* dists, void* saved, size_t saved_bytes,
                               void* ws, size_t ws_bytes, rdrf_stream_t stream_) {
  return rdrf_static_fwd_ex(P, cfg, rays, ts, xyz, z, valid, N, S, rgb, sigma, weight, dists, saved, saved_bytes, ws, ws_bytes,
                            stream_, 0);
}

extern "C" int rdrf_dynamic_fwd_ex(const RdrfDynamicParams* P, const RdrfFieldCfg* cfg,
                                   const float* rays, const float* ts, const float* xyz,
                                   const float* z, const uint8_t* valid, int N, int S,
                                   float* blending, float* weight, float* xyz_prime, float* rgb,
                                   float* sigma, float* dists, void* saved, size_t saved_bytes,
                                   void* ws, size_t ws_bytes, rdrf_stream_t stream_, int flags) {
  hipStream_t stream = (hipStream_t)stream_;
  if (N == 0) return 0;
  RDRF_CHECK(P && cfg && N > 0 && S > 0, -1, "dynamic_fwd: bad arguments");
  RDRF_CHECK((flags & ~RDRF_SAVE_NO_APP) == 0, -1, "dynamic_fwd: unknown flags 0x%x", flags);
  RDRF_CHECK((size_t)N * S * 3 < (size_t)INT32_MAX, -1, "dynamic_fwd: N * S * 3 must stay below 2^31 (32-bit sample indices): render / train in smaller chunks");
  RDRF_CHECK(vm_ok(P->density, 16, 4) && vm_ok(P->blending, 16, 4) && vm_ok(P->app, 48, 12) && vm_same_grid(P->density, P->blending), -1,
             "dynamic_fwd: only density comps {16,4,4} / app comps {48,12,12}, the planes and lines of a set spanning one grid, are built");
  FieldArgs a;
  fill_common(a, cfg, rays, ts, xyz, z, valid, N, S);
  a.rgb = rgb; a.sigma = sigma; a.weight = weight; a.dists = dists;
  a.blending = blending; a.xyz_prime = xyz_prime;
  a.dynq = fwd_dynq();
  int rc = ws_carve_fwd_ex(a, ws, ws_bytes, N, S, saved, saved_bytes, 1, flags);
  if (rc) return rc;
  DynW w;
  fill_dyn_w(w, P);
  if (P->packed_fwd != nullptr) a.pk = P->packed_fwd;
  else {
    PackJobs J;
    dyn_pack_jobs_fwd(J, P);
    rc = pack_launch(J, (float*)a.pk, stream);
    if (rc) return rc;
  }
  const bool flat = rdrf_flat_density();
  if (!flat && rgb != nullptr) RDRF_FILL(rgb, 0, (size_t)N * S * 3 * sizeof(float), stream);
  RDRF_LAUNCH("time_branch", k_time_branch, dim3((N + 7) / 8), dim3(256), stream, ts, w, N, a.tout, a.counter);
  const Geo g1 = geo_for_units(N), g3 = geo_for_tiles(N, S);
#ifdef RDRF_DETERMINISTIC
  RDRF_FILL(a.list, 0x7f, (size_t)N * S * sizeof(int), stream);
#endif
  if (flat) {
    if (saved != nullptr) RDRF_LAUNCH("dyn_density", k_dyn_density_flat<true>, dim3(g3.grid), dim3(g3.block), stream, a, w);
    else RDRF_LAUNCH("dyn_density", k_dyn_density_flat<false>, dim3(g3.grid), dim3(g3.block), stream, a, w);
    RDRF_LAUNCH("ray_scan", k_ray_scan, dim3((N + 15) / 16), dim3(512), stream, a);
  } else if (saved != nullptr) RDRF_LAUNCH("dyn_density", (k_dyn_density<false, true>), dim3(g1.grid), dim3(g1.block), stream, a, w);
  else RDRF_LAUNCH("dyn_density", (k_dyn_density<false, false>), dim3(g1.grid), dim3(g1.block), stream, a, w);
#ifdef RDRF_DETERMINISTIC
  { int rc_ = rdrf_sort_ints_inplace(a.list, (unsigned)((size_t)N * S), stream); if (rc_) return rc_; }
#endif
  if (rgb == nullptr) return 0;
  if (saved != nullptr && !(flags & RDRF_SAVE_NO_APP)) RDRF_LAUNCH("dyn_app", (k_dyn_app<false, true>), dim3(g3.grid), dim3(g3.block), stream, a, w);
  else RDRF_LAUNCH("dyn_app", (k_dyn_app<false, false>), dim3(g3.grid), dim3(g3.block), stream, a, w);
  return 0;
}

extern "C" int rdrf_dynamic_fwd(const RdrfDynamicParams* P, const RdrfFieldCfg* cfg,
                                const float* rays, const float* ts, const float* xyz,
                                const float* z, const uint8_t* valid, int N, int S,
                                float* blending, float* weight, float* xyz_prime, float* rgb,
                                float* sigma, float* dists, void* saved, size_t saved_bytes,
                                void* ws, size_t ws_bytes, rdrf_stream_t stream_) {
  return rdrf_dynamic_fwd_ex(P, cfg, rays, ts, xyz, z, valid, N, S, blending, weight, xyz_prime, rgb, sigma, dists, saved,
                             saved_bytes, ws, ws_bytes, stream_, 0);
}

extern "C" size_t rdrf_features_saved_bytes(int dynamic, int M) { return saved_bytes_feat(dynamic, M); }
extern "C" size_t rdrf_features_workspace_bytes(int M) {
  const int Np = (M + 31) / 32;
  return rdrf_workspace_bytes(Np, 32) + (size_t)Np * 32 * (32 * 4 + 27 * 4 + 8) + (1 << 14);
}

static int feat_carve_fwd(FieldArgs& a, void* ws, size_t ws_bytes, int M, void* saved, size_t saved_bytes,
                          int dynamic) {
  WsCarver c(ws, ws_bytes);
  const size_t mp = ((size_t)M + 31) / 32 * 32;
  a.pk = c.take<float>(PACK_AREA_FLOATS);
  a.tout = c.take<float>(mp * 32);
  a.xw = c.take<float>(mp * 3);
  RDRF_CHECK(c.ok(), -3, "features: workspace too small: need %zu have %zu", c.off, ws_bytes);
  if (saved != nullptr) {
    SavedPtrs sp;
    RDRF_CHECK(carve_saved_feat(sp, saved, saved_bytes, dynamic, M), -3,
               "features: saved buffer too small: need %zu have %zu", saved_bytes_feat(dynamic, M), saved_bytes);
    a.xw = sp.xw; a.tout = sp.tout; a.raw = sp.raw; a.act1 = sp.act1; a.act3 = sp.act3;
  }
  return 0;
}

extern "C" int rdrf_static_features_fwd(const RdrfStaticParams* P, const RdrfFieldCfg* cfg, const float* xn,
                                        int M, float* density, float* app, void* saved, size_t saved_bytes,
                                        void* ws, size_t ws_bytes, rdrf_stream_t stream_) {
  hipStream_t stream = (hipStream_t)stream_;
  if (M == 0) return 0;
  RDRF_CHECK(P && cfg && xn && M > 0 && (density || app), -1, "static_features_fwd: bad arguments");
  RDRF_CHECK(vm_ok(P->density, 16, 4) && vm_ok(P->app, 48, 12), -1,
             "static_features_fwd: only density comps {16,4,4} / app comps {48,12,12}, the planes and lines of a set spanning one grid, are built");
  const int Np = (M + 31) / 32;
  FieldArgs a;
  fill_common(a, cfg, nullptr, nullptr, xn, nullptr, nullptr, Np, 32);
  a.M = M; a.in_norm = 1; a.sigma = density; a.feat = app;
  int rc = feat_carve_fwd(a, ws, ws_bytes, M, saved, saved_bytes, 0);
  if (rc) return rc;
  StaticW w;
  fill_static_w(w, P);
  if (density != nullptr)
    RDRF_LAUNCH("feat_static_density", k_static_density<true>, dim3(Np), dim3(64), stream, a, w);
  if (app != nullptr) {
    if (P->packed_fwd != nullptr) a.pk = P->packed_fwd;
    else {
      PackJobs J;
      static_pack_jobs_fwd(J, P, cfg->static_head);
      rc = pack_launch(J, (float*)a.pk, stream);
      if (rc) return rc;
    }
    const Geo g = geo_for_units(Np);
    RDRF_LAUNCH("feat_static_app", (k_static_app<RDRF_HEAD_MLP_FEA, true>), dim3(g.grid), dim3(g.block), stream,
                a, w);
  }
  return 0;
}

extern "C" int rdrf_dynamic_features_fwd(const RdrfDynamicParams* P, const RdrfFieldCfg* cfg, const float* x,
                                         const float* t, int M, int x_is_normalized, float* density,
                                         float* blending, float* app, float* xyz_prime, void* saved,
                                         size_t saved_bytes, void* ws, size_t ws_bytes,
                                         rdrf_stream_t stream_) {
  hipStream_t stream = (hipStream_t)stream_;
  if (M == 0) return 0;
  RDRF_CHECK(P && cfg && x && t && M > 0 && (density || blending || app || xyz_prime), -1,
             "dynamic_features_fwd: bad arguments");
  RDRF_CHECK(vm_ok(P->density, 16, 4) && vm_ok(P->blending, 16, 4) && vm_ok(P->app, 48, 12) && vm_same_grid(P->density, P->blending), -1,
             "dynamic_features_fwd: only density comps {16,4,4} / app comps {48,12,12}, the planes and lines of a set spanning one grid, are built");
  const int Np = (M + 31) / 32;
  FieldArgs a;
  fill_common(a, cfg, nullptr, t, x, nullptr, nullptr, Np, 32);
  a.M = M; a.in_norm = x_is_normalized ? 1 : 0;
  a.sigma = density; a.blending = blending; a.feat = app; a.xyz_prime = xyz_prime;
  int rc = feat_carve_fwd(a, ws, ws_bytes, M, saved, saved_bytes, 1);
  if (rc) return rc;
  DynW w;
  fill_dyn_w(w, P);
  if (P->packed_fwd != nullptr) a.pk = P->packed_fwd;
  else {
    PackJobs J;
    dyn_pack_jobs_fwd(J, P);
    rc = pack_launch(J, (float*)a.pk, stream);
    if (rc) return rc;
  }
  RDRF_LAUNCH("time_branch", k_time_branch, dim3((M + 7) / 8), dim3(256), stream, t, w, M, a.tout, (int*)nullptr);
  const Geo g = geo_for_units(Np);
  RDRF_LAUNCH("feat_dyn_density", k_dyn_density<true>, dim3(g.grid), dim3(g.block), stream, a, w);
  if (app != nullptr) RDRF_LAUNCH("feat_dyn_app", k_dyn_app<true>, dim3(g.grid), dim3(g.block), stream, a, w);
  return 0;
}

extern "C" int rdrf_scene_flow_fwd(const RdrfDynamicParams* P, const RdrfFieldCfg* cfg,
                                   const float* pts, const float* ts, int N, int S, float* sf_f,
                                   float* sf_b, void* saved, size_t saved_bytes, void* ws,
                                   size_t ws_bytes, rdrf_stream_t stream_) {
  hipStream_t stream = (hipStream_t)stream_;
  if (N == 0) return 0;
  RDRF_CHECK(P && cfg && N > 0 && S > 0, -1, "scene_flow_fwd: bad arguments");
  RDRF_CHECK((size_t)N * S * 3 < (size_t)INT32_MAX, -1, "scene_flow_fwd: N * S * 3 must stay below 2^31 (32-bit sample indices): render / train in smaller chunks");
  FieldArgs a;
  memset(&a, 0, sizeof(a));
  RDRF_CHECK(saved == nullptr || saved_bytes >= rdrf_saved_bytes(2, N, S), -3,
             "scene_flow_fwd: saved buffer too small");
// ... 17 lines not shown
```

### robust-dynrf_amd/csrc/rdrf_fwd_dev.hpp

```cpp
#pragma once
#include "rdrf_kernels.hpp"

struct GridCtx {
  int bid, nblk, tid, nthr;
};
RDRF_D GridCtx grid_ctx() { return GridCtx{(int)blockIdx.x, (int)gridDim.x, (int)threadIdx.x, (int)blockDim.x}; }
#define GC_BID (FUSED ? gc.bid : (int)blockIdx.x)
#define GC_NBLK (FUSED ? gc.nblk : (int)gridDim.x)
#define GC_TID (FUSED ? gc.tid : (int)threadIdx.x)
#define GC_NTHR (FUSED ? gc.nthr : (int)blockDim.x)

RDRF_D int block_append_base(int* counter, int cnt, int* s_cnt, int tid, int nthr) {
  const int wave = tid >> 6, nwaves = nthr >> 6;
  __syncthreads();
  if ((tid & 63) == 0) s_cnt[wave] = cnt;
  __syncthreads();
  if (tid == 0) {
    int tot = 0;
    for (int w = 0; w < nwaves; ++w) {
      const int c = s_cnt[w];
      s_cnt[w] = tot;
      tot += c;
    }
    const int b = tot ? atomicAdd(counter, tot) : 0;
// ... 376 lines not shown
  mfma_seg_b3<2, pk::K1_HEAD_KK>(acc, U, wb3, lane);
  const float V[4] = {X1[4], X1[5], X1[6], X1[7]};
  mfma_seg<2, 4>(acc, V, wtail, lane);
}
#endif

template <bool FEAT, bool SAVE = true, bool FUSED = false, bool FLAT = false>
RDRF_D void dyn_density_body(const FieldArgs a, const DynW w, float* lds_fused, const GridCtx gc) {
  static_assert(!FLAT || (!FEAT && !FUSED), "the flat-tile form is a ray-path kernel of its own");
  float* lds;
  if constexpr (FUSED) lds = lds_fused;
  else {
    __shared__ __attribute__((aligned(16))) float lds_own[pk::K1_SIZE];
    lds = lds_own;
  }
  const int lane = GC_TID & 63, h = lane >> 5, s = lane & 31;
  const int wave = GC_TID >> 6, nwaves = GC_NTHR >> 6;
  __shared__ int s_next;
  if (FLAT && GC_TID == 0) s_next = nwaves;
  lds_fill(lds, a.pk + pk::REG_K1, pk::K1_SIZE);
  const float* pkw = lds;
  const int nunits = FLAT ? (int)(((long)a.N * a.S + 31) >> 5) : a.N;
  const bool dynq = FLAT && (a.dynq & 1) != 0;
  int k = wave;
  for (int n = FLAT ? GC_BID + k * GC_NBLK : GC_BID * nwaves + wave; n < nunits;
       n = FLAT ? GC_BID + (k = tile_queue_next(&s_next, k, nwaves, dynq)) * GC_NBLK : n + GC_NBLK * nwaves) {
  float t = 0.f, nrm = 1.0f;
  float T[16];
  float X1[8];
  if constexpr (!FEAT && !FLAT) {
    t = a.ts[n];
    float vx, vy, vz;
    nrm = ray_norm(a.rays, n, a.ray_type, vx, vy, vz);
#pragma unroll
    for (int q = 0; q < 4; ++q) {
      f32x4 v = ld4(a.tout + n * 32 + 8 * q + 4 * h);
      T[q * 4 + 0] = v.x; T[q * 4 + 1] = v.y; T[q * 4 + 2] = v.z; T[q * 4 + 3] = v.w;
    }
    fill_x1(X1, t, h);
  }
  float carry = 1.0f;
  int nmask = 0;
  for (int j0 = 0; j0 < (FLAT ? 32 : a.S); j0 += 32) {
    const int j = j0 + s;
    bool act;
    int idx;
    if constexpr (FLAT) {
      const long i = (long)n * 32 + s;
      act = i < (long)a.N * a.S;
      idx = act ? (int)i : 0;
    } else {
      act = j < a.S && (!FEAT || n * a.S + j < a.M);
      idx = n * a.S + (act ? j : 0);
    }
    const bool vld = act && (FEAT || a.valid[idx] != 0);
    if constexpr (FEAT || FLAT) {
      const int ti = FLAT ? idx / a.S : idx;
      t = a.ts[ti];
#pragma unroll
      for (int q = 0; q < 4; ++q) {
        f32x4 v = ld4(a.tout + (size_t)ti * 32 + 8 * q + 4 * h);
        T[q * 4 + 0] = v.x; T[q * 4 + 1] = v.y; T[q * 4 + 2] = v.z; T[q * 4 + 3] = v.w;
      }
      fill_x1(X1, t, h);
    }
#ifndef RDRF_T_RESIDENT
    if constexpr (!FEAT && !FLAT) {
      int nn = n;
      asm volatile("" : "+v"(nn));
#pragma unroll
      for (int q = 0; q < 4; ++q) {
        f32x4 v = ld4(a.tout + nn * 32 + 8 * q + 4 * h);
        T[q * 4 + 0] = v.x; T[q * 4 + 1] = v.y; T[q * 4 + 2] = v.z; T[q * 4 + 3] = v.w;
      }
    }
#endif
    const float px = a.xyz[idx * 3 + 0], py = a.xyz[idx * 3 + 1], pz = a.xyz[idx * 3 + 2];
    const bool raw_in = FEAT && a.in_norm;
    const float xn0 = raw_in ? px : norm_c(px, a.box.lo[0], a.box.inv[0]);
    const float xn1 = raw_in ? py : norm_c(py, a.box.lo[1], a.box.inv[1]);
    const float xn2 = raw_in ? pz : norm_c(pz, a.box.lo[2], a.box.inv[2]);
    float X0[32];
    fill_x0(X0, xn0, xn1, xn2, t, h);
    float* svb = (SAVE && a.act1) ? a.act1 + (FLAT ? (size_t)n : (size_t)n * ((a.S + 31) >> 5) + (j0 >> 5)) * sv::K1_ROWS * 32 : nullptr;
    save_rows<32>(svb, sv::K1_X0, X0, s, h);
    save_rows<8>(svb, sv::K1_X1, X1, s, h);
    save_rows<16>(svb, sv::K1_T, T, s, h);
    float d0, d1, d2;
    {
      f32x16 acc[2];
      acc_bias<2>(acc, pkw + pk::K1_B3, h);
      mfma_seg<2, 32>(acc, X0, pkw + pk::K1_W3_X0, lane);
      mfma_seg<2, 16>(acc, T, pkw + pk::K1_W3_T, lane);
      float H3[32];
      acc_relu<2>(H3, acc);
      save_rows<32>(svb, sv::K1_H3, H3, s, h);
      acc_bias<2>(acc, pkw + pk::K1_B4, h);
      mfma_seg<2, 32>(acc, H3, pkw + pk::K1_W4, lane);
      acc_relu<2>(H3, acc);
      save_rows<32>(svb, sv::K1_H4, H3, s, h);
      d0 = dot_small<32>(H3, pkw + pk::K1_W5 + 0 * 64, h) + w.l5b[0];
      d1 = dot_small<32>(H3, pkw + pk::K1_W5 + 1 * 64, h) + w.l5b[1];
      d2 = dot_small<32>(H3, pkw + pk::K1_W5 + 2 * 64, h) + w.l5b[2];
    }
    const float xw0 = norm_c(unnorm_c(xn0, a.box.lo[0], a.box.inv[0]) + d0, a.box.lo[0], a.box.inv[0]);
    const float xw1 = norm_c(unnorm_c(xn1, a.box.lo[1], a.box.inv[1]) + d1, a.box.lo[1], a.box.inv[1]);
    const float xw2 = norm_c(unnorm_c(xn2, a.box.lo[2], a.box.inv[2]) + d2, a.box.lo[2], a.box.inv[2]);
    if (act && h == 0) {
      if (!FEAT || a.xyz_prime != nullptr) {
        a.xyz_prime[(size_t)idx * 3 + 0] = (raw_in ? unnorm_c(xn0, a.box.lo[0], a.box.inv[0]) : px) + d0;
        a.xyz_prime[(size_t)idx * 3 + 1] = (raw_in ? unnorm_c(xn1, a.box.lo[1], a.box.inv[1]) : py) + d1;
        a.xyz_prime[(size_t)idx * 3 + 2] = (raw_in ? unnorm_c(xn2, a.box.lo[2], a.box.inv[2]) : pz) + d2;
      }
      a.xw[(size_t)idx * 3 + 0] = xw0;
      a.xw[(size_t)idx * 3 + 1] = xw1;
      a.xw[(size_t)idx * 3 + 2] = xw2;
    }
    float fd, fb;
    {
      float Fv[36];
      gather_level_den<0>(w.density, point_taps(w.density, xw0, xw1, xw2, 0), h, Fv);
      gather_level_den<12>(w.density, point_taps(w.density, xw0, xw1, xw2, 1), h, Fv);
      gather_level_den<24>(w.density, point_taps(w.density, xw0, xw1, xw2, 2), h, Fv);
      if (!vld) {
#pragma unroll
        for (int i = 0; i < 36; ++i) Fv[i] = 0.f;
      }
      f32x16 acc[2];
      acc_bias<2>(acc, pkw + pk::K1_BD1, h);
#ifdef RDRF_HEADS_F32
      mfma_seg<2, 36>(acc, Fv, pkw + pk::K1_DEN1_F, lane);
      mfma_seg<2, 32>(acc, X0, pkw + pk::K1_DEN1_X0, lane);
      mfma_seg<2, 8>(acc, X1, pkw + pk::K1_DEN1_X1, lane);
#else
      head_layer1(acc, Fv, X0, X1, pkw + pk::K1_DEN1, pkw + pk::K1_DEN1_X1T, lane);
#endif
      float Hd[32];
      acc_relu<2>(Hd, acc);
      save_rows<36>(svb, sv::K1_FD, Fv, s, h);
      save_rows<32>(svb, sv::K1_HD, Hd, s, h);
      fd = dot_small<32>(Hd, pkw + pk::K1_DEN2, h) + w.db2[0];
    }
    {
      float Fv[36];
      gather_level_den<0>(w.blending, point_taps(w.blending, xw0, xw1, xw2, 0), h, Fv);
      gather_level_den<12>(w.blending, point_taps(w.blending, xw0, xw1, xw2, 1), h, Fv);
      gather_level_den<24>(w.blending, point_taps(w.blending, xw0, xw1, xw2, 2), h, Fv);
      if (!vld) {
#pragma unroll
        for (int i = 0; i < 36; ++i) Fv[i] = 0.f;
      }
      f32x16 acc[2];
      acc_bias<2>(acc, pkw + pk::K1_BB1, h);
#ifdef RDRF_HEADS_F32
      mfma_seg<2, 36>(acc, Fv, pkw + pk::K1_BLE1_F, lane);
      mfma_seg<2, 32>(acc, X0, pkw + pk::K1_BLE1_X0, lane);
      mfma_seg<2, 8>(acc, X1, pkw + pk::K1_BLE1_X1, lane);
#else
      head_layer1(acc, Fv, X0, X1, pkw + pk::K1_BLE1, pkw + pk::K1_BLE1_X1T, lane);
#endif
      float Hd[32];
      acc_relu<2>(Hd, acc);
      save_rows<36>(svb, sv::K1_FB, Fv, s, h);
      save_rows<32>(svb, sv::K1_HB, Hd, s, h);
      fb = dot_small<32>(Hd, pkw + pk::K1_BLE2, h) + w.bb2[0];
    }
    if constexpr (FEAT) {
      if (act && h == 0) {
        if (a.sigma != nullptr) a.sigma[idx] = fd;
        if (a.blending != nullptr) a.blending[idx] = fb;
        if (a.raw != nullptr) { a.raw[(size_t)idx * 2] = fd; a.raw[(size_t)idx * 2 + 1] = fb; }
      }
    } else if constexpr (FLAT) {
      if (act && h == 0) {
        a.sigma[idx] = vld ? density_act(fd, a.act, a.density_shift) : 0.0f;
        a.blending[idx] = vld ? sigmoidf_(fb) : 0.0f;
        if (SAVE && a.raw != nullptr) { a.raw[(size_t)idx * 2] = fd; a.raw[(size_t)idx * 2 + 1] = fb; }
      }
    } else {
    const float sigma = vld ? density_act(fd, a.act, a.density_shift) : 0.0f;
    const float blend = vld ? sigmoidf_(fb) : 0.0f;
    const float zj = act ? a.z[idx] : 0.f;
    const float zn = (j + 1 < a.S) ? a.z[idx + 1] : zj;
    const float ds = ((j + 1 < a.S) ? (zn - zj) : 0.0f) * nrm * a.distance_scale;
    const float alpha = 1.0f - expf(-sigma * ds);
    const float p = act ? one_minus_alpha_eps(alpha) : 1.0f;
    const float incl = scan_mul32(p, s);
    float excl = __shfl_up(incl, 1, 32);
    if (s == 0) excl = 1.0f;
    const float Tr = carry * excl;
    const float wt = alpha * Tr;
    carry *= __shfl(incl, 31, 32);
    const bool m = act && h == 0 && wt > a.weight_thres;
    if (act && h == 0) {
      a.sigma[idx] = sigma;
      a.weight[idx] = wt;
      a.dists[idx] = ds;
      a.blending[idx] = blend;
      if (SAVE && a.raw != nullptr) { a.raw[(size_t)idx * 2] = fd; a.raw[(size_t)idx * 2 + 1] = fb; }
    }
    nmask += __popcll(__ballot(m));
    }
  }
  if constexpr (!FEAT && !FLAT) {
    if (nmask) {
      int base = 0;
      if (lane == 0) base = atomicAdd(a.counter, nmask);
      base = __shfl(base, 0, 64);
      for (int j0 = 0; j0 < a.S; j0 += 32) {
        const int j = j0 + s;
        const bool act = j < a.S && h == 0;
        const int idx = n * a.S + (act ? j : 0);
        const bool m = act && a.weight[idx] > a.weight_thres;
        const unsigned long long bal = __ballot(m);
        if (m) a.list[base + __builtin_amdgcn_mbcnt_hi((unsigned)(bal >> 32), __builtin_amdgcn_mbcnt_lo((unsigned)bal, 0u))] = idx;
        base += __popcll(bal);
      }
    }
  }
  }
}

RDRF_D void ray_scan_body(const FieldArgs a) {
  __shared__ int s_cnt[16];
  const int lane = threadIdx.x & 63, h = lane >> 5, s = lane & 31;
  const int n_ = (blockIdx.x * (blockDim.x >> 6) + (threadIdx.x >> 6)) * 2 + h;
  const bool ray = n_ < a.N;
  const int n = ray ? n_ : 0;
  float vx, vy, vz;
  const float nrm = ray_norm(a.rays, n, a.ray_type, vx, vy, vz);
  float carry = 1.0f;
  int cnt = 0;
  for (int j0 = 0; j0 < a.S; j0 += 32) {
    const int j = j0 + s;
    const bool act = ray && j < a.S;
    const int idx = n * a.S + (act ? j : 0);
    const float sigma = act ? a.sigma[idx] : 0.0f;
    const float zj = act ? a.z[idx] : 0.f;
    const float zn = (j + 1 < a.S) ? a.z[idx + 1] : zj;
    const float ds = ((j + 1 < a.S) ? (zn - zj) : 0.0f) * nrm * a.distance_scale;
    const float alpha = 1.0f - expf(-sigma * ds);
    const float p = act ? one_minus_alpha_eps(alpha) : 1.0f;
    const float incl = scan_mul32(p, s);
    float excl = __shfl_up(incl, 1, 32);
    if (s == 0) excl = 1.0f;
    const float Tr = carry * excl;
    const float wt = alpha * Tr;
// ... 215 lines not shown
```

### robust-dynrf_amd/csrc/rdrf_kernels.hpp

```cpp
#pragma once
#include "rdrf_host.hpp"

struct FieldArgs {
  const float* rays;
  const float* ts;
  const float* xyz;
  const float* z;
  const uint8_t* valid;
  int N, S;
  Box box;
  float distance_scale, weight_thres, density_shift;
  int act, ray_type, static_head;
  float *rgb, *sigma, *weight, *dists, *blending, *xyz_prime;
  const float* pk;
  float* tout;
  float* xw;
  int* list;
  int* counter;
  float* act1;
  float* act3;
  float* raw;
  int M;
  int in_norm;
  float* feat;
  int dynq;
};

struct StaticW {
  RdrfVM density, app;
  const float *b1, *b2, *b3, *w3;
};
struct DynW {
  RdrfVM density, blending, app;
  const float *l1w, *l1b, *l2w, *l2b;
  const float *l3b, *l4b, *l5b, *db1, *db2, *bb1, *bb2, *rb1, *rb2, *rbv, *rwv;
  const float *sfb0, *sfb2, *sfb4, *sfb6;
};

RDRF_D float density_act(float f, int act, float shift) {
  return act == RDRF_ACT_RELU ? fmaxf(f, 0.0f) : softplusf_(f + shift);
}

RDRF_D float ray_norm(const float* rays, int n, int ray_type, float& vx, float& vy, float& vz) {
  vx = rays[n * 6 + 3];
  vy = rays[n * 6 + 4];
  vz = rays[n * 6 + 5];
  float nrm = 1.0f;
  if (ray_type != RDRF_RAY_OTHER) {
    nrm = sqrtf(vx * vx + vy * vy + vz * vz);
    vx /= nrm;
    vy /= nrm;
    vz /= nrm;
  }
  return nrm;
}


RDRF_D int tile_queue_next(int* s_next, int k, int nwaves, bool dyn) {
  if (!dyn) return k + nwaves;
  int v = 0;
  if ((threadIdx.x & 63) == 0) v = atomicAdd(s_next, 1);
  return __builtin_amdgcn_readfirstlane(v);
}

namespace sv {
constexpr int K1_X0 = 0, K1_X1 = 64, K1_T = 96, K1_H3 = 128, K1_H4 = 192, K1_FD = 256, K1_HD = 352,
              K1_FB = 416, K1_HB = 512, K1_ROWS = 576;
constexpr int K3_A = 0, K3_F = 224, K3_X0 = 256, K3_X1 = 320, K3_H1 = 352, K3_H2 = 480, K3_VD = 608,
              K3_ROWS = 640;
constexpr int S3_G = 0, S3_F = 96, S3_P = 128, S3_H1 = 256, S3_H2 = 384, S3_VD = 512, S3_ROWS = 544;
constexpr int SF_X = 0, SF_H0 = 64, SF_H2 = 128, SF_H4 = 192, SF_ROWS = 256;
constexpr int K1G_DZ3 = 0, K1G_DZ4 = 64, K1G_SM = 128, K1G_DZD = 160, K1G_DZB = 224, K1G_DFD = 288,
              K1G_DFB = 384, K1G_DX0 = 480, K1G_ROWS = 544;
constexpr int K3G_DZV = 0, K3G_DZ2 = 32, K3G_DZ1 = 160, K3G_DF = 288, K3G_DA = 320, K3G_ROWS = 544;
constexpr int SFG_DZ6 = 0, SFG_DZ4 = 32, SFG_DZ2 = 96, SFG_DZ0 = 160, SFG_ROWS = 224;
}

template <int KK>
RDRF_D void save_rows(float* __restrict__ tile_base, int row0, const float (&v)[KK], int s, int h) {
  if (tile_base == nullptr) return;
#ifdef RDRF_ABL_NOSAVE
  return;
#endif
#pragma unroll
  for (int kk = 0; kk < KK; ++kk) {
#ifdef RDRF_SAVE_TEMPORAL
    tile_base[(size_t)(row0 + elem_of(kk, h)) * 32 + s] = v[kk];
#else
    __builtin_nontemporal_store(v[kk], tile_base + (size_t)(row0 + elem_of(kk, h)) * 32 + s);
#endif
  }
}
template <int KK>
RDRF_D void load_rows(const float* __restrict__ tile_base, int row0, float (&v)[KK], int s, int h) {
#pragma unroll
#ifdef RDRF_NT_ROWS
  for (int kk = 0; kk < KK; ++kk) v[kk] = __builtin_nontemporal_load(tile_base + (size_t)(row0 + elem_of(kk, h)) * 32 + s);
#else
  for (int kk = 0; kk < KK; ++kk) v[kk] = tile_base[(size_t)(row0 + elem_of(kk, h)) * 32 + s];
#endif
}

struct SavedHdr {
  int count;
  int pad[63];
};

struct SavedPtrs {
  SavedHdr* hdr;
  int* list;
  float* xw;
  float* tout;
  float* raw;
  float* act1;
  float* act3;
};

static inline size_t saved_bytes_feat(int dynamic, int M) {
  size_t t = ((size_t)M + 31) / 32, mp = t * 32;
  size_t b = sizeof(SavedHdr) + 256;
  b += mp * 3 * 4 + 256 + mp * 32 * 4 + 256 + mp * 2 * 4 + 256;
  if (dynamic) b += t * sv::K1_ROWS * 32 * 4 + 256;
  b += t * (dynamic ? sv::K3_ROWS : sv::S3_ROWS) * 32 * 4 + 256;
  return b;
}
static inline bool carve_saved_feat(SavedPtrs& p, void* saved, size_t bytes, int dynamic, int M) {
  WsCarver c(saved, bytes);
  size_t t = ((size_t)M + 31) / 32, mp = t * 32;
  p.hdr = c.take<SavedHdr>(1);
  p.list = nullptr;
  p.xw = c.take<float>(mp * 3);
  p.tout = c.take<float>(mp * 32);
  p.raw = c.take<float>(mp * 2);
  p.act1 = dynamic ? c.take<float>(t * sv::K1_ROWS * 32) : nullptr;
  p.act3 = c.take<float>(t * (dynamic ? sv::K3_ROWS : sv::S3_ROWS) * 32);
  return c.ok();
}
static inline size_t saved_bytes_field(int dynamic, int N, int S, int flags = 0) {
  size_t ns = (size_t)N * S, t1 = (size_t)N * ((S + 31) / 32), t3 = (ns + 31) / 32;
  size_t b = sizeof(SavedHdr) + 256;
  b += ns * 4 + 256;
  b += ns * 3 * 4 + 256 + (size_t)N * 32 * 4 + 256;
  b += ns * 2 * 4 + 256;
  if (dynamic) b += t1 * sv::K1_ROWS * 32 * 4 + 256;
  if (!(flags & RDRF_SAVE_NO_APP)) b += t3 * (dynamic ? sv::K3_ROWS : sv::S3_ROWS) * 32 * 4 + 256;
  return b;
}
static inline bool carve_saved(SavedPtrs& p, void* saved, size_t bytes, int dynamic, int N, int S, int flags = 0) {
  WsCarver c(saved, bytes);
  size_t ns = (size_t)N * S, t1 = (size_t)N * ((S + 31) / 32), t3 = (ns + 31) / 32;
  p.hdr = c.take<SavedHdr>(1);
  p.list = c.take<int>(ns);
  p.xw = c.take<float>(ns * 3);
  p.tout = c.take<float>((size_t)N * 32);
  p.raw = c.take<float>(ns * 2);
  p.act1 = dynamic ? c.take<float>(t1 * sv::K1_ROWS * 32) : nullptr;
  p.act3 = (flags & RDRF_SAVE_NO_APP) ? nullptr : c.take<float>(t3 * (dynamic ? sv::K3_ROWS : sv::S3_ROWS) * 32);
  return c.ok();
}
static inline int carve_saved_bwd(SavedPtrs& p, void* saved, size_t bytes, int dynamic, int N, int S) {
  if (carve_saved(p, saved, bytes, dynamic, N, S, 0)) return 1;
  return carve_saved(p, saved, bytes, dynamic, N, S, RDRF_SAVE_NO_APP) ? 0 : -1;
}
```

### robust-dynrf_amd/fields.py

```python
import collections
import ctypes as C

import os

import torch
import torch.nn as nn
import torch.nn.functional as F

from . import _lib as L
from .regularizers import dense_l1, tv_family, vector_diffs

MAT_MODE = [[0, 1], [0, 2], [1, 2]]
VEC_MODE = [2, 1, 0]


class _Head(nn.Module):
    def forward(self, *a, **k):
        raise RuntimeError("the RGB head is fused into the HIP appearance kernel; call the field")


class MLPRender_Fea(_Head):
    def __init__(self, inChanel, viewpe=6, feape=6, featureC=128):
        super().__init__()
        self.in_mlpC = 2 * viewpe * 3 + 2 * feape * inChanel + 3 + inChanel
# ... 68 lines not shown
def _cfg_struct(field, ray_type, weight_thres=None):
    c = L.RdrfFieldCfg()
    ab = field._aabb_host
    for i in range(6):
        c.aabb[i] = ab[i]
    c.distance_scale = float(field.distance_scale)
    c.weight_thres = float(field.rayMarch_weight_thres if weight_thres is None else weight_thres)
    c.density_shift = float(field.density_shift)
    c.act = L.ACTS[field.fea2denseAct]
    c.ray_type = L.RAY_TYPES.get(ray_type, 2)
    c.static_head = L.HEADS.get(field.shadingMode, 0)
    return c


STATIC_KEYS = (["density_plane.%d" % i for i in range(3)] + ["density_line.%d" % i for i in range(3)]
               + ["app_plane.%d" % i for i in range(3)] + ["app_line.%d" % i for i in range(3)]
               + ["basis_mat.weight"])
DYN_VM = (["density_plane.%d" % i for i in range(3)] + ["density_line.%d" % i for i in range(3)]
          + ["blending_plane.%d" % i for i in range(3)] + ["blending_line.%d" % i for i in range(3)]
          + ["app_plane.%d" % i for i in range(3)] + ["app_line.%d" % i for i in range(3)])


def _static_struct(t):
    P = L.RdrfStaticParams()
    P.density = _vm_struct(t[0:3], t[3:6])
    P.app = _vm_struct(t[6:9], t[9:12])
    for name, ten in zip(("basis", "w1", "b1", "w2", "b2", "w3", "b3"), t[12:19]):
        setattr(P, name, ten.data_ptr())
    return P


def _dynamic_struct(t):
    P = L.RdrfDynamicParams()
    P.density = _vm_struct(t[0:3], t[3:6])
    P.blending = _vm_struct(t[6:9], t[9:12])
    P.app = _vm_struct(t[12:15], t[15:18])
    names = ("basis", "rw1", "rb1", "rw2", "rb2", "rwv", "rbv", "l1w", "l1b", "l2w", "l2b", "l3w",
             "l3b", "l4w", "l4b", "l5w", "l5b", "dw1", "db1", "dw2", "db2", "bw1", "bb1", "bw2", "bb2")
    for name, ten in zip(names, t[18:43]):
        setattr(P, name, ten.data_ptr())
    for i in range(4):
        P.sfw[i] = t[43 + 2 * i].data_ptr()
        P.sfb[i] = t[44 + 2 * i].data_ptr()
    return P


PACK_CACHE = os.environ.get("RDRF_PACK_CACHE", "1") == "1"


def _attach_packed(field, P, params, backward, dynamic):
    if not PACK_CACHE or field is None:
        return
    first = 18 if dynamic else 12
    stream = torch.cuda.current_stream(params[0].device).cuda_stream
    key = (tuple((p.data_ptr(), p._version) for p in params[first:]), field._pack_epoch)
    cache = field.__dict__.setdefault("_pack_cache", {})
    slot = cache.get((backward, stream))
    if slot is None or slot[0] != key:
        img = slot[1] if slot is not None else torch.empty(int(L.lib.rdrf_pack_floats()), device=params[0].device)
        if dynamic:
            L.check(L.lib.rdrf_dynamic_pack(C.byref(P), int(backward), L.ptr(img), C.c_void_p(stream)), "rdrf_dynamic_pack")
        else:
            L.check(L.lib.rdrf_static_pack(C.byref(P), L.HEADS.get(field.shadingMode, 0), int(backward), L.ptr(img),
                                           C.c_void_p(stream)), "rdrf_static_pack")
        cache[(backward, stream)] = slot = (key, img)
    if backward:
        P.packed_bwd = slot[1].data_ptr()
    else:
        P.packed_fwd = slot[1].data_ptr()


SAVE_STATS = collections.Counter()


def _grad_mode(grad_mode):
    return torch.is_grad_enabled() if grad_mode is None else bool(grad_mode)


def _alloc_saved(ctx, kind, N, S, dev, grad_mode=None, flags=0):
    if not _grad_mode(grad_mode) or not any(ctx.needs_input_grad):
        SAVE_STATS[(kind, "none")] += 1
        return None, 0
    nbytes = int(L.lib.rdrf_saved_bytes_ex(kind, N, S, flags))
    SAVE_STATS[(kind, "no_app" if flags & L.SAVE_NO_APP else "full")] += 1
    SAVE_STATS[(kind, "bytes")] += nbytes
    return torch.empty(nbytes, dtype=torch.uint8, device=dev), nbytes


_RGB_SUFFIX = {True: "", False: "-norgb", "value": "-valrgb"}


def _call_mode(ray_type, rgb):
    rgb = rgb if isinstance(rgb, str) else bool(rgb)
    if rgb not in _RGB_SUFFIX:
        raise ValueError(f"forward(..., rgb=...) takes True, False or 'value', not {rgb!r}")
    return ray_type + _RGB_SUFFIX[rgb] + ("" if torch.is_grad_enabled() else "-nograd")


def _parse_mode(mode):
    grad_mode = not mode.endswith("-nograd")
    mode = mode.replace("-nograd", "")
    rgb = "value" if mode.endswith("-valrgb") else not mode.endswith("-norgb")
    return mode.replace("-valrgb", "").replace("-norgb", ""), rgb, grad_mode


def _prep_inputs(rays, ts, xyz, z, valid):
    L.require_device(rays, ts, xyz, z, valid)
    rays, ts, xyz, z = L.f32c(rays), L.f32c(ts), L.f32c(xyz), L.f32c(z)
    valid = valid.contiguous()
    if valid.dtype == torch.bool:
        valid = valid.view(torch.uint8)
    return rays, ts, xyz, z, valid


class _StaticFn(torch.autograd.Function):
    @staticmethod
    def forward(ctx, field, ray_type, rays, ts, xyz, z, valid, *params):
        ctx.set_materialize_grads(False)
        rays, ts, xyz, z, valid = _prep_inputs(rays, ts, xyz, z, valid)
        N, S = z.shape
        dev = z.device
        ray_type, rgb_mode, grad_mode = _parse_mode(ray_type)
        want_rgb, flags = rgb_mode is not False, L.SAVE_NO_APP if rgb_mode == "value" else 0
        rgb = torch.empty(N, S, 3, device=dev) if want_rgb else None
        sigma = torch.empty(N, S, device=dev)
        weight = torch.empty(N, S, device=dev)
        dists = torch.empty(N, S, device=dev)
        saved, sbytes = _alloc_saved(ctx, 0, N, S, dev, grad_mode, flags)
        ws = L.workspace(dev, (L.lib.rdrf_workspace_bytes if saved is not None else L.lib.rdrf_forward_workspace_bytes)(N, S))
        P = _static_struct(params)
        _attach_packed(field, P, params, False, False)
        cfg = _cfg_struct(field, ray_type)
        L.check(L.lib.rdrf_static_fwd_ex(C.byref(P), C.byref(cfg), L.ptr(rays), L.ptr(ts), L.ptr(xyz),
                                         L.ptr(z), L.ptr(valid), N, S, L.ptr(rgb), L.ptr(sigma),
                                         L.ptr(weight), L.ptr(dists), L.ptr(saved), C.c_size_t(sbytes),
                                         L.ptr(ws), C.c_size_t(ws.numel()), L.stream_of(z), flags),
                "rdrf_static_fwd")
        if rgb_mode == "value":
            ctx.mark_non_differentiable(rgb)
        ctx.field, ctx.ray_type, ctx.saved, ctx.want_rgb = field, ray_type, saved, rgb_mode is True
        ctx.save_for_backward(rays, ts, xyz, z, valid, *params)
        return rgb, sigma, weight, dists

    @staticmethod
    def backward(ctx, g_rgb, g_sigma, g_weight, g_dists):
        rays, ts, xyz, z, valid, *params = ctx.saved_tensors
        if g_rgb is not None and not ctx.want_rgb:
            raise L.RdrfError("forward(..., rgb=False | 'value') saved no appearance rows: no gradient can flow through rgb")
        need = ctx.needs_input_grad
        if g_rgb is None and g_sigma is None and g_weight is None and not (need[2] or need[5]):
            ctx.saved = None
            return (None,) * (7 + len(params))
        if ctx.saved is None:
            raise L.RdrfError("TensorVMSplit.forward: backward called twice (the saved activations are released "
                              "after the first backward; retain_graph is not supported)")
        N, S = z.shape
        dev = z.device
        fused = ctx.field.fused_grad
        ctx.field._det_bind()
        grads = ctx.field.fused_grads() if fused else [torch.zeros_like(p) for p in params]
        G = _static_struct(grads)
        P = _static_struct(params)
        _attach_packed(ctx.field, P, params, True, False)
        cfg = _cfg_struct(ctx.field, ctx.ray_type)
        need = ctx.needs_input_grad
        g_rays, g_xyz, g_z = L.zeros_like_many([rays, xyz, z], [need[2], need[4], need[5]])
        cont = lambda g: None if g is None else L.f32c(g)
        g_rgb, g_sigma, g_weight, g_dists = cont(g_rgb), cont(g_sigma), cont(g_weight), cont(g_dists)
        ws = L.workspace(dev, L.lib.rdrf_workspace_bytes(N, S))
        L.check(L.lib.rdrf_static_bwd(C.byref(P), C.byref(cfg), L.ptr(rays), L.ptr(ts), L.ptr(xyz),
                                      L.ptr(z), L.ptr(valid), N, S, L.ptr(g_rgb), L.ptr(g_sigma),
                                      L.ptr(g_weight), L.ptr(g_dists), C.byref(G), L.ptr(g_xyz),
                                      L.ptr(g_z), L.ptr(g_rays), L.ptr(ctx.saved),
                                      C.c_size_t(ctx.saved.numel()), L.ptr(ws), C.c_size_t(ws.numel()),
                                      L.stream_of(z)), "rdrf_static_bwd")
        ctx.saved = None
        if fused:
            grads = [None] * len(params)
        return (None, None, g_rays, None, g_xyz, g_z, None, *grads)


class _DynamicFn(torch.autograd.Function):
    @staticmethod
    def forward(ctx, field, ray_type, rays, ts, xyz, z, valid, *params):
        ctx.set_materialize_grads(False)
        rays, ts, xyz, z, valid = _prep_inputs(rays, ts, xyz, z, valid)
        N, S = z.shape
        dev = z.device
        ray_type, rgb_mode, grad_mode = _parse_mode(ray_type)
        want_rgb, flags = rgb_mode is not False, L.SAVE_NO_APP if rgb_mode == "value" else 0
        rgb = torch.empty(N, S, 3, device=dev) if want_rgb else None
        xyz_prime = torch.empty(N, S, 3, device=dev)
        sigma, weight, dists, blending = (torch.empty(N, S, device=dev) for _ in range(4))
        saved, sbytes = _alloc_saved(ctx, 1, N, S, dev, grad_mode, flags)
        ws = L.workspace(dev, (L.lib.rdrf_workspace_bytes if saved is not None else L.lib.rdrf_forward_workspace_bytes)(N, S))
        P = _dynamic_struct(params)
        _attach_packed(field, P, params, False, True)
        cfg = _cfg_struct(field, ray_type)
        L.check(L.lib.rdrf_dynamic_fwd_ex(C.byref(P), C.byref(cfg), L.ptr(rays), L.ptr(ts), L.ptr(xyz),
                                          L.ptr(z), L.ptr(valid), N, S, L.ptr(blending), L.ptr(weight),
                                          L.ptr(xyz_prime), L.ptr(rgb), L.ptr(sigma), L.ptr(dists),
                                          L.ptr(saved), C.c_size_t(sbytes), L.ptr(ws),
                                          C.c_size_t(ws.numel()), L.stream_of(z), flags), "rdrf_dynamic_fwd")
        if rgb_mode == "value":
            ctx.mark_non_differentiable(rgb)
        ctx.field, ctx.ray_type, ctx.saved, ctx.want_rgb = field, ray_type, saved, rgb_mode is True
        ctx.save_for_backward(rays, ts, xyz, z, valid, *params)
        return blending, weight, xyz_prime, rgb, sigma, dists

    @staticmethod
    def backward(ctx, g_blending, g_weight, g_xyz_prime, g_rgb, g_sigma, g_dists):
        rays, ts, xyz, z, valid, *params = ctx.saved_tensors
        if g_rgb is not None and not ctx.want_rgb:
            raise L.RdrfError("forward(..., rgb=False | 'value') saved no appearance rows: no gradient can flow through rgb")
        need = ctx.needs_input_grad
        if all(g is None for g in (g_blending, g_weight, g_xyz_prime, g_rgb, g_sigma)) and not (need[2] or need[5]):
            ctx.saved = None
            return (None,) * (7 + len(params))
        if ctx.saved is None:
            raise L.RdrfError("TensorVMSplit_TimeEmbedding.forward: backward called twice (the saved activations "
                              "are released after the first backward; retain_graph is not supported)")
        N, S = z.shape
        dev = z.device
        fused = ctx.field.fused_grad
        ctx.field._det_bind()
        grads = ctx.field.fused_grads() if fused else [torch.zeros_like(p) for p in params]
        G = _dynamic_struct(grads)
        P = _dynamic_struct(params)
        _attach_packed(ctx.field, P, params, True, True)
        cfg = _cfg_struct(ctx.field, ctx.ray_type)
        need = ctx.needs_input_grad
        g_rays, g_xyz, g_z = L.zeros_like_many([rays, xyz, z], [need[2], need[4], need[5]])
        cont = lambda g: None if g is None else L.f32c(g)
        gb, gw, gxp, gr, gs, gd = (cont(g) for g in (g_blending, g_weight, g_xyz_prime, g_rgb,
                                                      g_sigma, g_dists))
        ws = L.workspace(dev, L.lib.rdrf_workspace_bytes(N, S))
        L.check(L.lib.rdrf_dynamic_bwd(C.byref(P), C.byref(cfg), L.ptr(rays), L.ptr(ts), L.ptr(xyz),
                                       L.ptr(z), L.ptr(valid), N, S, L.ptr(gb), L.ptr(gw),
                                       L.ptr(gxp), L.ptr(gr), L.ptr(gs), L.ptr(gd), C.byref(G),
                                       L.ptr(g_xyz), L.ptr(g_z), L.ptr(g_rays), L.ptr(ctx.saved),
                                       C.c_size_t(ctx.saved.numel()), L.ptr(ws),
                                       C.c_size_t(ws.numel()), L.stream_of(z)), "rdrf_dynamic_bwd")
        ctx.saved = None
        if fused:
            grads = [None] * len(params)
        return (None, None, g_rays, None, g_xyz, g_z, None, *grads)


class _SceneFlowFn(torch.autograd.Function):
    @staticmethod
    def forward(ctx, field, grad_mode, pts, ts, *params):
        ctx.set_materialize_grads(False)
        L.require_device(pts, ts)
        pts, ts = L.f32c(pts), L.f32c(ts)
        N, S, _ = pts.shape
        sf_f = torch.empty(N, S, 3, device=pts.device)
        sf_b = torch.empty(N, S, 3, device=pts.device)
        ws = L.workspace(pts.device, L.lib.rdrf_workspace_bytes(N, S))
        saved, sbytes = _alloc_saved(ctx, 2, N, S, pts.device, grad_mode)
        P = _dynamic_struct(params)
        _attach_packed(field, P, params, False, True)
        cfg = _cfg_struct(field, "ndc")
        L.check(L.lib.rdrf_scene_flow_fwd(C.byref(P), C.byref(cfg), L.ptr(pts), L.ptr(ts), N, S,
                                          L.ptr(sf_f), L.ptr(sf_b), L.ptr(saved), C.c_size_t(sbytes),
                                          L.ptr(ws), C.c_size_t(ws.numel()), L.stream_of(pts)),
                "rdrf_scene_flow_fwd")
        ctx.field, ctx.saved = field, saved
        ctx.save_for_backward(pts, ts, *params)
        return sf_f, sf_b

    @staticmethod
    def backward(ctx, g_f, g_b):
        pts, ts, *params = ctx.saved_tensors
        if ctx.saved is None:
            raise L.RdrfError("get_forward_backward_scene_flow: backward called twice (retain_graph is not supported)")
        N, S, _ = pts.shape
        fused = ctx.field.fused_grad
        ctx.field._det_bind()
        grads = ctx.field.fused_grads() if fused else [torch.zeros_like(p) for p in params]
        G = _dynamic_struct(grads)
        P = _dynamic_struct(params)
        _attach_packed(ctx.field, P, params, True, True)
        cfg = _cfg_struct(ctx.field, "ndc")
        g_pts = torch.zeros_like(pts) if ctx.needs_input_grad[2] else None
        g_f = None if g_f is None else L.f32c(g_f)
        g_b = None if g_b is None else L.f32c(g_b)
        ws = L.workspace(pts.device, L.lib.rdrf_workspace_bytes(N, S))
        L.check(L.lib.rdrf_scene_flow_bwd(C.byref(P), C.byref(cfg), L.ptr(pts), L.ptr(ts), N, S,
                                          L.ptr(g_f), L.ptr(g_b), C.byref(G), L.ptr(g_pts),
                                          L.ptr(ctx.saved), C.c_size_t(ctx.saved.numel()), L.ptr(ws),
                                          C.c_size_t(ws.numel()), L.stream_of(pts)),
                "rdrf_scene_flow_bwd")
        ctx.saved = None
        if fused:
            grads = [None] * len(params)
        return (None, None, g_pts, None, *grads)

# ... 400 lines not shown
        return dense_l1(self, self.density_plane, self.density_line)

    def TV_loss_density(self, reg):
        return tv_family(self, reg, self.density_plane, self.density_line)

    def TV_loss_app(self, reg):
        return tv_family(self, reg, self.app_plane, self.app_line)

    def forward(self, rays_chunk, ts_chunk, timeembeddings_chunk, xyz_sampled, z_vals, ray_valid,
                white_bg=True, is_train=False, ray_type="ndc", N_samples=-1, rgb=True):
        if timeembeddings_chunk is not None:
            raise NotImplementedError("timeembeddings_chunk is None at every reference call site")
        rgb, sigma, weight, dists = _StaticFn.apply(self, _call_mode(ray_type, rgb), rays_chunk, ts_chunk,
                                                    xyz_sampled, z_vals, ray_valid, *self._param_list())
        return (None, None, None, xyz_sampled, weight, None, rgb, sigma, z_vals, dists)

    @torch.no_grad()
    def upsample_volume_grid(self, res_target):
        self.app_plane, self.app_line = self.up_sampling_VM(self.app_plane, self.app_line, res_target)
        self.density_plane, self.density_line = self.up_sampling_VM(self.density_plane,
                                                                    self.density_line, res_target)
        self.update_stepSize(res_target, 1)


class TensorVMSplit_TimeEmbedding(TensorBase):

    def __init__(self, aabb, gridSize, tSize, device, **kargs):
        super().__init__(aabb, gridSize, tSize, device, **kargs)
        self.layer1 = nn.Linear(1 + 8 * 2 * 1, 64).to(device)
        self.layer2 = nn.Linear(64, 30).to(device)
        self.layer3 = nn.Linear((3 + 10 * 2 * 3) + 30, 64).to(device)
        self.layer4 = nn.Linear(64, 64).to(device)
        self.layer5 = nn.Linear(64, 3).to(device)
        nin = sum(self.density_n_comp) * 3 + 3 + 10 * 2 * 3 + 1 + 8 * 2 * 1
        self.density_layer1 = nn.Linear(nin, 64).to(device)
        self.density_layer2 = nn.Linear(64, 1).to(device)
        self.blending_layer1 = nn.Linear(nin, 64).to(device)
        self.blending_layer2 = nn.Linear(64, 1).to(device)
        self.scene_flow_mlp = nn.Sequential(
            nn.Linear(4 * 2 * 4 + 4, 64), nn.ReLU(inplace=True), nn.Linear(64, 64),
            nn.ReLU(inplace=True), nn.Linear(64, 64), nn.ReLU(inplace=True), nn.Linear(64, 6),
        ).to(device)
        if self.shadingMode != "MLP_Fea_late_view" or self.fea_pe != 0:
            raise NotImplementedError("dynamic head is built for MLP_Fea_late_view, fea_pe=0 "
                                      "(configs/*.txt, train.py:918)")

    def init_svd_volume(self, res, device):
        self.blending_plane, self.blending_line = self.init_one_svd(self.density_n_comp,
                                                                    self.gridSize, 0.1, device)
        self.density_plane, self.density_line = self.init_one_svd(self.density_n_comp, self.gridSize,
                                                                  0.1, device)
        self.app_plane, self.app_line = self.init_one_svd(self.app_n_comp, self.gridSize, 0.1, device)
        self.basis_mat = nn.Linear(sum(self.app_n_comp) * 3, self.app_dim, bias=False).to(device)

    def get_optparam_groups(self, lr_init_spatialxyz=0.02, lr_init_network=0.001):
        g = [{"params": self.density_line, "lr": lr_init_spatialxyz},
             {"params": self.density_plane, "lr": lr_init_spatialxyz},
             {"params": self.blending_line, "lr": lr_init_spatialxyz},
             {"params": self.blending_plane, "lr": lr_init_spatialxyz},
             {"params": self.app_line, "lr": lr_init_spatialxyz},
             {"params": self.app_plane, "lr": lr_init_spatialxyz},
             {"params": self.basis_mat.parameters(), "lr": lr_init_network},
             {"params": self.scene_flow_mlp.parameters(), "lr": lr_init_network}]
        for m in (self.layer1, self.layer2, self.layer3, self.layer4, self.layer5, self.density_layer1,
                  self.density_layer2, self.blending_layer1, self.blending_layer2):
            g.append({"params": m.parameters(), "lr": lr_init_network})
        g.append({"params": self.renderModule.parameters(), "lr": lr_init_network})
        return g

    def _param_list(self):
        rm = self.renderModule
        t = (list(self.density_plane) + list(self.density_line) + list(self.blending_plane)
             + list(self.blending_line) + list(self.app_plane) + list(self.app_line))
        t += [self.basis_mat.weight, rm.mlp[0].weight, rm.mlp[0].bias, rm.mlp[2].weight,
              rm.mlp[2].bias, rm.mlp_view[0].weight, rm.mlp_view[0].bias]
        for m in (self.layer1, self.layer2, self.layer3, self.layer4, self.layer5, self.density_layer1,
                  self.density_layer2, self.blending_layer1, self.blending_layer2):
            t += [m.weight, m.bias]
        for i in (0, 2, 4, 6):
            t += [self.scene_flow_mlp[i].weight, self.scene_flow_mlp[i].bias]
        return t

    def forward(self, rays_chunk, ts_chunk, timeembeddings_chunk, xyz_sampled, z_vals, ray_valid,
                white_bg=True, is_train=False, ray_type="ndc", N_samples=-1, rgb=True):
        if timeembeddings_chunk is not None:
            raise NotImplementedError("timeembeddings_chunk is None at every reference call site")
        blending, weight, xyz_prime, rgb, sigma, dists = _DynamicFn.apply(
            self, _call_mode(ray_type, rgb), rays_chunk, ts_chunk, xyz_sampled, z_vals, ray_valid,
            *self._param_list())
        return (None, None, blending, xyz_sampled, weight, xyz_prime, rgb, sigma, z_vals, dists)

    def density_L1(self):
        return dense_l1(self, self.density_plane, self.density_line)

    def blending_L1(self):
        return dense_l1(self, self.blending_plane, self.blending_line)

    def TV_loss_blending(self, reg):
        return tv_family(self, reg, self.blending_plane, self.blending_line)

    def TV_loss_density(self, reg):
        return tv_family(self, reg, self.density_plane, self.density_line)

    def TV_loss_app(self, reg):
        return tv_family(self, reg, self.app_plane, self.app_line)

    def get_forward_backward_scene_flow(self, unnormalized_pts, t_sampled):
        return _SceneFlowFn.apply(self, torch.is_grad_enabled(), unnormalized_pts, t_sampled, *self._param_list())

    def _features(self, want, x, t, normalized):
        x2 = x.reshape(-1, 3)
        t2 = t.reshape(-1)
        if t2.numel() != x2.shape[0]:
            raise L.RdrfError(f"compute_*: {x2.shape[0]} points but {t2.numel()} times")
        return _DynFeatFn.apply(self, torch.is_grad_enabled(), want, normalized, x2, t2, *self._param_list())

    def warp_coordinate(self, unnormalized_xyz_sampled, t_sampled):
        out = self._features(("warp",), unnormalized_xyz_sampled, t_sampled, False)[3]
        return out.reshape(unnormalized_xyz_sampled.shape)

    def compute_densityfeature(self, xyz_sampled, t_sampled, time_embedding_sampled=None):
        return self._features(("density",), xyz_sampled, t_sampled, True)[0]

    def compute_blendingfeature(self, xyz_sampled, t_sampled, time_embedding_sampled=None):
        return self._features(("blending",), xyz_sampled, t_sampled, True)[1]

    def compute_appfeature(self, xyz_sampled, t_sampled, time_embedding_sampled=None):
        return self._features(("app",), xyz_sampled, t_sampled, True)[2]

    @torch.no_grad()
    def upsample_volume_grid(self, res_target):
        self.app_plane, self.app_line = self.up_sampling_VM(self.app_plane, self.app_line, res_target)
        self.density_plane, self.density_line = self.up_sampling_VM(self.density_plane,
                                                                    self.density_line, res_target)
        self.blending_plane, self.blending_line = self.up_sampling_VM(self.blending_plane,
                                                                      self.blending_line, res_target)
        self.update_stepSize(res_target, 1)
```

### robust-dynrf_amd/step.py

```python
import collections
import math
import os
import types

import torch
import torch.nn as nn

from .fields import TensorVMSplit, TensorVMSplit_TimeEmbedding
from .optim import FlatAdam
from .parallel import require_even_shards
from .ray_utils import gather_rows, generate_rays, ids2pixel, pose_to_mtx
from .regularizers import TVLoss
from .losses import LossTerms, frame_depth_loss
from .renderer import distloss_rays, induce_flow, raw2outputs, sampleXYZ

NDC_AABB = [[-1.5, -1.67, -1.0], [1.5, 1.67, 1.0]]


def scene_config(name="nvidia", stage="stage0"):
    if name == "nvidia":
        cfg = dict(aabb=NDC_AABB, near_far=[0.0, 1.0], T=12, H=135, W=240, ray_type="ndc", batch_size=4096,
                   static_head="MLP_Fea", optimize_poses=False, tv_density=1.0, tv_app=1.0, dist_static=0.0,
                   dist_dynamic=0.01, l1_weight=0.0, N_voxel_init=128 ** 3, N_voxel_final=300 ** 3)
        stages = {"stage0": ([141, 157, 94], 115), "up1": ([174, 194, 116], 142), "up2": ([216, 240, 144], 176),
# ... 150 lines not shown
        return self.perm[off: off + bs]

    def ts_of(self, ids):
        return self.ts_table[ids]

    def make_batch(self, it, bs, shard=None, ids=None):
        ids, ids2 = (self.batch(it, bs, 0), self.batch(it, bs, 1)) if ids is None else ids
        if shard is not None:
            r, w = shard
            lo, hi = r * bs // w, (r + 1) * bs // w
            ids, ids2 = ids[lo:hi], ids2[lo:hi]
        sc, v2 = self._scalars[:, ids], self._vec2[:, ids]
        return dict(ids=ids, ts=sc[0], ts_rand=self.ts_of(ids2), grid=v2[2], px=v2[3], view=self.view_table[ids], rgb=self.rgb[ids],
                    disp=sc[1], fg=sc[2], flow_f=v2[0], flow_b=v2[1], mask_f=sc[3][:, None], mask_b=sc[4][:, None])


SyntheticBalloon = SyntheticScene


class StepRng:

    def __init__(self, seed=7):
        self.gen = torch.Generator().manual_seed(seed)
        self._pool, self._cur = None, 0

    def coin(self):
        return bool(torch.rand(1, generator=self.gen).item() < 0.5)

    def _take(self, n, device):
        n_al = (n + 63) // 64 * 64
        if self._pool is None or self._pool.device != torch.device(device) or self._cur + n_al > self._pool.numel():
            self._pool, self._cur = torch.rand(max(16 * n_al, 8192), device=device), 0
        v = self._pool[self._cur: self._cur + n]
        self._cur += n_al
        return v

    def jitter(self, S, ray_type, device):
        if ray_type == "ndc":
            return self._take(S, device), None
        return self._take(S - S // 2 + 1, device), self._take(S // 2 + 1, device)


class GraphRng:
    N_COINS = 16

    def __init__(self, device, pool_floats=1 << 16):
        self.pool = torch.rand(pool_floats, device=device)
        self.coins = torch.round(self.pool[: self.N_COINS])
        self.frozen = False
        self._cur, self._ncoin = 64, 0

    def begin(self):
        if not self.frozen:
            self.pool.uniform_()
            torch.round(self.pool[: self.N_COINS], out=self.coins)
        self._cur, self._ncoin = 64, 0

    def coin(self):
        if self._ncoin >= self.N_COINS:
            raise RuntimeError("GraphRng: more than N_COINS coins in one iteration")
        k = self._ncoin
        self._ncoin += 1
        return self.coins[k: k + 1]

    def _take(self, n, device):
        n_al = (n + 63) // 64 * 64
        if self._cur + n_al > self.pool.numel():
            raise RuntimeError("GraphRng: the jitter pool is too small for one iteration of this shape")
        v = self.pool[self._cur: self._cur + n]
        self._cur += n_al
        return v

    jitter = StepRng.jitter


PASSES = collections.Counter()


def _rgb_or_zeros(rgb, like):
    return rgb if rgb is not None else torch.zeros(*like.shape, 3, device=like.device)


def ray_pass(st, dy, rays, ts, n_samples, ray_type, rng, is_train=True, static_grad=False, dynamic=True, rgb_s=True,
             rgb_d=True):
    jit, jit_o = rng.jitter(n_samples, ray_type, rays.device) if is_train else (None, None)
    xyz, z, valid = sampleXYZ(dy, rays, n_samples, ray_type=ray_type, is_train=is_train, jitter=jit,
                              jitter_outer=jit_o)
    PASSES.update(static=1, static_grad=int(static_grad), dynamic=int(dynamic), dynamic_dead=int(dynamic and static_grad))
    if static_grad:
        o_s = st(rays, ts, None, xyz, z, valid, is_train=is_train, ray_type=ray_type, rgb=rgb_s)
    else:
        with torch.no_grad():
            o_s = st(rays, ts, None, xyz, z, valid, is_train=is_train, ray_type=ray_type, rgb=rgb_s)
    sigma_s = o_s[7]
    rgb_s = _rgb_or_zeros(o_s[6], sigma_s)
    if dynamic:
        dead = static_grad
        if dead and rgb_d is True:
            rgb_d = "value"
        with torch.set_grad_enabled(torch.is_grad_enabled() and (not dead or rays.requires_grad or z.requires_grad)):
            o_d = dy(rays, ts, None, xyz, z, valid, is_train=is_train, ray_type=ray_type, rgb=rgb_d)
        rgb_d, sigma_d, dists, blending, zv = _rgb_or_zeros(o_d[6], o_d[7]), o_d[7], o_d[9], o_d[2], o_d[8]
    else:
        o_d = None
        rgb_d = torch.zeros_like(rgb_s)
        sigma_d = torch.zeros_like(sigma_s)
        blending = torch.zeros_like(sigma_s)
        dists, zv = o_s[9], z
    white = rng.coin() if is_train else False
    outs = raw2outputs(rgb_s, sigma_s, rgb_d, sigma_d, dists, blending, zv, rays, is_train=is_train,
                       ray_type=ray_type, add_white_bg=white)
    return o_s, o_d, outs, xyz


BATCH_MAX_SAMPLES = int(float(os.environ.get("RDRF_BATCH_MAX_SAMPLES", 6e6)))


def batch_groups(idxs, n_samples_per_pass):
    per = max(1, BATCH_MAX_SAMPLES // max(1, n_samples_per_pass))
    idxs = list(idxs)
    return [idxs[i:i + per] for i in range(0, len(idxs), per)]


def batched_field(field, rays_list, ts_list, samples, idxs, ray_type, grad=True, rgb=True):
    if len(idxs) == 1:
        k = idxs[0]
        with torch.set_grad_enabled(grad and torch.is_grad_enabled()):
            return [field(rays_list[k], ts_list[k], None, *samples[k], is_train=True, ray_type=ray_type, rgb=rgb)]
    N = rays_list[idxs[0]].shape[0]
    cat = lambda ts: torch.cat([ts[k] for k in idxs])
    with torch.set_grad_enabled(grad and torch.is_grad_enabled()):
        o = field(cat(rays_list), cat(ts_list), None, *(torch.cat([samples[k][i] for k in idxs]) for i in range(3)),
                  is_train=True, ray_type=ray_type, rgb=rgb)
    parts = [None if t is None else t.view(len(idxs), N, *t.shape[1:]).unbind(0) for t in o]
    return [tuple(None if pt is None else pt[j] for pt in parts) for j in range(len(idxs))]


def ray_passes(st, dy, rays_list, ts_list, n_samples, ray_type, rng, groups, rgb=None):
    P, N, dev = len(rays_list), rays_list[0].shape[0], rays_list[0].device
    PASSES.update(static=P, dynamic=P)
    samples, coins = [], []
    for rays in rays_list:
        jit, jit_o = rng.jitter(n_samples, ray_type, dev)
        samples.append(sampleXYZ(dy, rays, n_samples, ray_type=ray_type, is_train=True, jitter=jit, jitter_outer=jit_o))
        coins.append(rng.coin())
    ns = N * samples[0][1].shape[1]
    rgb = [True] * P if rgb is None else list(rgb)
    o_ss, o_ds = [None] * P, [None] * P
    runs, lo = [], 0
    want_s = [bool(f) for f in rgb]
    for p in range(1, P + 1):
        if p == P or want_s[p] != want_s[lo]:
            runs.append(list(range(lo, p)))
            lo = p
    for run in runs:
        for g in batch_groups(run, ns):
            for k, o in zip(g, batched_field(st, rays_list, ts_list, samples, g, ray_type, grad=False, rgb=want_s[run[0]])):
                o_ss[k] = o
    for group in groups:
        assert list(group) == list(range(group[0], group[0] + len(group)))
        assert all(rgb[k] == rgb[group[0]] for k in group), "a dynamic group must agree on its colour flag"
        for g in batch_groups(group, ns):
            for k, o in zip(g, batched_field(dy, rays_list, ts_list, samples, g, ray_type, rgb=rgb[group[0]])):
                o_ds[k] = o
    out = []
    for p in range(P):
        o_sp, o_d = o_ss[p], o_ds[p]
        outs = raw2outputs(_rgb_or_zeros(o_sp[6], o_sp[7]), o_sp[7], _rgb_or_zeros(o_d[6], o_d[7]), o_d[7], o_d[9], o_d[2],
                           o_d[8], rays_list[p], is_train=True,
                           ray_type=ray_type, add_white_bg=coins[p])
        out.append((o_sp, o_d, outs, samples[p][0]))
    return out


def masked_mean(x, m):
    return (x * m).sum() / (m.sum() + 1e-8)


class Trainer:
    def __init__(self, cfg, device, weights="dense", lr_init=0.02, lr_basis=1e-3, dead_work=False,
                 dp_mode="allreduce", lr_pose=3e-3, dp_exact_stats=False, batch_passes=None, graph=False, data=None):
        self.batch_passes = (os.environ.get("RDRF_BATCH_PASSES", "1") != "0") if batch_passes is None else bool(batch_passes)
        self.dead_work = dead_work
        self.dp_exact_stats = bool(dp_exact_stats)
        if data is not None:
            data.bind(cfg)
            if "grid" not in cfg:
                it0 = int(cfg.get("start_iteration", 0))
                _, cfg["grid"], cfg["n_samples"] = [s for s in resolution_stages(cfg) if s[0] <= it0][-1]
        self.cfg = cfg
        self.device = device
        self.st, self.dy = build_fields(cfg, device)
        if weights == "sparse":
            sparsify_(self.st, self.dy, cfg, device)
        self.data = SyntheticScene(cfg, device) if data is None else data
        lr_factor = cfg.get("lr_decay_target_ratio", 0.1) ** (1.0 / cfg.get("n_iters", 100000))
        self.opt = FlatAdam([self.st, self.dy], lr_init, lr_basis, betas=(0.9, 0.99), lr_factor=lr_factor,
                            mode=dp_mode)
        self.lr_factor = lr_factor
        self.optimize_poses = bool(cfg.get("optimize_poses", False))
        self.it = int(cfg.get("start_iteration", 0))
        if self.optimize_poses:
            self.poses = nn.Parameter(self.data.poses.clone())
            self.fov = nn.Parameter(torch.full((1,), 30.0 / 180.0 * math.pi, device=device))
            self.lr_pose = lr_pose
            ups = cfg.get("upsamp_list", [0, 0, 0, 0])
            self.pose_gamma = (1e-5 / lr_pose) ** (1.0 / max(1, cfg.get("n_iters", 100000) // 2 - ups[-1]))
            self.opt_pose = torch.optim.Adam([self.poses], lr=lr_pose)
            self.opt_focal = torch.optim.Adam([self.fov], lr=lr_pose if self.it >= ups[3] else 0.0)
        self.rng = StepRng()
        self.graph = bool(graph)
        self._graphs, self._graph_seen, self._gs = {}, None, None
        self._dyn = None
        self.tv = TVLoss()
        self.grad_flats = self.opt.grad_flats()
        self.last = {}
        self._c2w_fixed = None

    def _dp(self):
        ex = self.opt.ex
        return (self.opt._group, ex.rank, ex.world) if (self.dp_exact_stats and ex.active) else None

    def _loss_terms(self):
        dp = self._dp()
        if dp is None:
            return LossTerms()
        import torch.distributed as dist

        def reducer(stats):
            g = stats.clone()
            dist.all_reduce(g, op=dist.ReduceOp.SUM, group=dp[0])
            return g, dp[2]
        return LossTerms(reducer)

    def _dead_rgb(self):
        return "value" if self.dead_work else False

    def focal(self):
        if self.optimize_poses:
            return max(self.cfg["H"], self.cfg["W"]) / 2.0 / torch.tan(self.fov[0])
        return self.data.focal

    def pose_table(self):
        return self.poses if self.optimize_poses else self.data.poses

    def _coef(self, const, name, value):
        if self._dyn is None:
            return const * value
        return (const, self._dyn[name])

    def rays_for(self, ids, poses=None, focal=None, uv=None, view_shift=0):
        c = self.cfg
        poses = self.pose_table() if poses is None else poses
        focal = self.focal() if focal is None else focal
        return generate_rays(ids, poses, focal, c["H"], c["W"], ndc=c["ray_type"] == "ndc", near=1.0, uv=uv,
                             view_shift=view_shift)

    def losses(self, b, terms="all", capture=None):
        c = self.cfg
        S, rt, T, H, W = c["n_samples"], c["ray_type"], c["T"], c["H"], c["W"]
        it, rng = self.it, self.rng
        ids, ts, rgb_t, disp_t, fg = b["ids"], b["ts"], b["rgb"], b["disp"], b["fg"]
        N = ids.shape[0]
        poses, focal = self.pose_table(), self.focal()
        if terms not in ("all", "image_AE"):
            raise ValueError(terms)
        full = terms == "all"
        rays = b["rays"] if "rays" in b else self.rays_for(ids, poses, focal)
        rays_d = rays.detach()
        poses_d, focal_d = poses.detach(), (focal.detach() if torch.is_tensor(focal) else focal)
        dt = 2.0 / (T - 1)
        if "grid" in b:
            grid, view = b["grid"], b["view"]
        else:
            col, row, view = ids2pixel(W, H, ids)
            grid = torch.stack([col.float() + 0.5, row.float() + 0.5], -1)
        px = b["px"] if "px" in b else grid - 0.5
        if self.optimize_poses:
            c2w_all = pose_to_mtx(poses)
        else:
            if self._c2w_fixed is None:
                self._c2w_fixed = pose_to_mtx(poses).detach()
            c2w_all = self._c2w_fixed
        temp = 1.0 / (10 ** (it // 100000))
        temp_disp_tv = 1.0 / (10 ** (it // 50000))
        temp_static = 1.0 / (10 ** (it / 100000.0))
        ups = c.get("upsamp_list", [0, 0, 0, 0])
        early, late = it >= ups[0], it >= ups[3]
        gt_depth = -disp_t if rt == "ndc" else disp_t
        to_depth = (lambda d: d) if rt == "ndc" else (lambda d: 1.0 / (d + 1e-6))
        Ld = self._loss_terms()

        def skewed(dyn):
            m2 = torch.clamp(dyn, min=1e-6, max=1.0 - 1e-6) ** 2
            return torch.mean(-(m2 * torch.log(m2) + (1 - m2) * torch.log(1 - m2)))

        def order_terms(outs):
            return to_depth(outs[9]), to_depth(outs[5].detach()), (1.0 - outs[12].detach())

        if full and self.batch_passes:
            rays_n_of = {sgn: self.rays_for(ids, poses_d, focal_d, uv=grid + b["flow_f" if sgn > 0 else "flow_b"], view_shift=sgn)
                         for sgn in (1, -1)}
            groups = [[0], [1, 2, 3]] if not late else [[0], [1], [2, 3]]
            pA, pB, pC, pD = ray_passes(self.st, self.dy, [rays_d, rays_d, rays_n_of[1], rays_n_of[-1]],
                                        [ts, b["ts_rand"], ts + dt, ts - dt], S, rt, rng, groups,
                                        rgb=[True] + [self._dead_rgb()] * 3)
            osA, oA, outA, xyzA = pA
            batched = {"B": pB, 1: pC, -1: pD}
        else:
            osA, oA, outA, xyzA = ray_pass(self.st, self.dy, rays_d, ts, S, rt, rng)
            batched = None
        if capture is not None:
            capture["A"] = (osA, oA, outA, xyzA)
        Ld.add(3.0, "square", outA[0], rgb_t).add(1.0, "square", outA[8], rgb_t)
        if not full:
            oE, oEd, outE, xyzE = ray_pass(self.st, self.dy, rays, ts, S, rt, rng, static_grad=True, dynamic=self.dead_work)
            if capture is not None:
                capture["E"] = (oE, oEd, outE, xyzE)
            Ls = self._loss_terms().add(1.0 / 3.0, "square", outE[4], rgb_t, w=(1.0 - fg)[:, None], norm="weight")
            self.terms = (Ld, Ls)
            return Ld.total(), Ls.total()
        if early:
            Ld.add(0.1 * temp_disp_tv, "abs", outA[12], fg)
        if late:
            Ld.add(0.01, "identity", skewed(outA[12]))
            Ld.add(0.01, "abs", outA[12])
        xo, yo, wo = order_terms(outA)
        Ld.add(10.0, "square", xo, yo, w=wo, norm="weight")
        Ld.add(1.0, "identity", frame_depth_loss(to_depth(outA[9]), gt_depth, view, T, coef=c["monodepth_dynamic"] * temp,
                                                 dp=self._dp()))
        w_dist = c["dist_dynamic"] * (it / c["n_iters"])
        k_dist = self._coef(c["dist_dynamic"], "ramp", it / c["n_iters"])
        if w_dist > 0:
            Ld.add(k_dist, "identity", distloss_rays(outA[11], oA[8].detach(), 1.0 / S))
        _, oB, outB, _ = batched["B"] if batched else ray_pass(self.st, self.dy, rays_d, b["ts_rand"], S, rt, rng,
                                                               rgb_s=self._dead_rgb(), rgb_d=self._dead_rgb())
        if late:
            Ld.add(0.01, "identity", skewed(outB[12]))
            Ld.add(0.01, "abs", outB[12])
        xo, yo, wo = order_terms(outB)
        Ld.add(10.0, "square", xo, yo, w=wo, norm="weight")
        if w_dist > 0:
            Ld.add(k_dist, "identity", distloss_rays(outB[11], oB[8].detach(), 1.0 / S))
        sf_f, sf_b = self.dy.get_forward_backward_scene_flow(oA[3], ts)
        Ld.add(c["small_scene_flow_weight"], "abs", sf_f).add(c["small_scene_flow_weight"], "abs", sf_b)
        Ld.add(c["smooth_scene_flow_weight"], "abs", sf_f, sf_b, ysign=1.0)
        weights_d, pts_ref = outA[11], oA[3]
        disp_A = {}
        for sgn, sf, flow_t, mask_t in ((1, sf_f, b["flow_f"], b["mask_f"]), (-1, sf_b, b["flow_b"], b["mask_b"])):
            pose_n = c2w_all[(view + sgn).clamp(0, T - 1)].detach()
            pts_n = pts_ref + sf if rt == "ndc" else torch.clamp(pts_ref + sf, min=-2.0 + 1e-6, max=2.0 - 1e-6)
            ind_flow, ind_disp = induce_flow(H, W, focal_d, pose_n, weights_d, pts_n, px, rays_d, ray_type=rt)
            Ld.add(0.01 * temp, "abs", ind_flow, flow_t, w=mask_t, norm="weight")
            disp_A[sgn] = (ind_disp, mask_t, pose_n, flow_t)
        for sgn in (1, -1):
            ind_disp, mask_t, pose_n, flow_t = disp_A[sgn]
            if batched:
                rays_n = rays_n_of[sgn]
                _, oN, outN, _ = batched[sgn]
            else:
                rays_n = self.rays_for(ids, poses_d, focal_d, uv=grid + flow_t, view_shift=sgn)
                _, oN, outN, _ = ray_pass(self.st, self.dy, rays_n, ts + sgn * dt, S, rt, rng, rgb_s=self._dead_rgb(),
                                          rgb_d=self._dead_rgb())
            _, ind_disp_n = induce_flow(H, W, focal_d, pose_n, outN[11], oN[3], px, rays_n, ray_type=rt)
            Ld.add(0.04 * temp, "abs", ind_disp, ind_disp_n, w=mask_t, norm="weight")
            if w_dist > 0:
                Ld.add(k_dist, "identity", distloss_rays(outN[11], oN[8].detach(), 1.0 / S))
        oE, _, outE, _ = ray_pass(self.st, self.dy, rays, ts, S, rt, rng, static_grad=True, dynamic=self.dead_work)
        m = (1.0 - fg)[:, None]
        Ls = self._loss_terms()
        Ls.add(1.0 / 3.0, "square", outE[4], rgb_t, w=m, norm="weight")
        if c["dist_static"] > 0 and it > 0:
            Ls.add(self._coef(c["dist_static"], "ramp", it / c["n_iters"]), "identity",
                   distloss_rays(outE[7], oE[8].detach(), 1.0 / S))
        if self.optimize_poses:
            self._pose_block(b, rays, oE, outE, poses, focal, c2w_all, grid, px, view, m, temp_disp_tv, temp_static, gt_depth,
                             to_depth, Ls)
        if c["l1_weight"] > 0:
            Ld.add(c["l1_weight"], "identity", self.dy.density_L1())
            Ls.add(c["l1_weight"], "identity", self.st.density_L1())
        loss_s, loss_d = Ls.total(), Ld.total()
        self.terms = (Ld, Ls)
        return loss_d, loss_s

    def _pose_block(self, b, rays, oE, outE, poses, focal, c2w_all, grid, px, view, m, temp_disp_tv, temp_static, gt_depth,
                    to_depth, Ls):
        c = self.cfg
        S, rt, T, H, W = c["n_samples"], c["ray_type"], c["T"], c["H"], c["W"]
        ids, ts, fg = b["ids"], b["ts"], b["fg"]
        rng = self.rng
        weights_s, pts_ref_s, depth_s = outE[7], oE[3], outE[5]
        col, row = grid[:, 0], grid[:, 1]
        uv_P34 = (torch.stack([torch.clamp(col + 1.0, max=W - 0.5), row], -1),
                  torch.stack([col, torch.clamp(row + 1.0, max=H - 0.5)], -1))
        batched = None
        if self.batch_passes:
            rays_P = [self.rays_for(ids, poses, focal, uv=grid + b["flow_f"], view_shift=1),
                      self.rays_for(ids, poses, focal, uv=grid + b["flow_b"], view_shift=-1),
                      self.rays_for(ids, poses, focal, uv=uv_P34[0]), self.rays_for(ids, poses, focal, uv=uv_P34[1])]
            smp, coins = [], []
            for k, r in enumerate(rays_P):
                jit, jit_o = rng.jitter(S, rt, rays.device)
                smp.append(sampleXYZ(self.st if k < 2 else self.dy, r, S, ray_type=rt, is_train=True, jitter=jit,
                                     jitter_outer=jit_o))
                coins.append(rng.coin() if k >= 2 else None)
            PASSES.update(static=4, static_grad=4)
            ts_P = [ts] * 4
            ns = rays.shape[0] * smp[0][1].shape[1]
            o_P = [None] * 4
            for g in batch_groups(range(4), ns):
                for k, o in zip(g, batched_field(self.st, rays_P, ts_P, smp, g, rt, rgb=self._dead_rgb())):
                    o_P[k] = o
            d_P = [None, None]
            if self.dead_work:
                PASSES.update(dynamic=2, dynamic_dead=2)
                for g in batch_groups((2, 3), ns):
                    live = any(rays_P[k].requires_grad or smp[k][1].requires_grad for k in g)
                    for k, o in zip(g, batched_field(self.dy, rays_P, ts_P, smp, g, rt, grad=live, rgb="value")):
                        d_P[k - 2] = o
            batched = (rays_P, smp, coins, o_P, d_P)
        for k, (sgn, flow_t, mask_t) in enumerate(((1, b["flow_f"], b["mask_f"]), (-1, b["flow_b"], b["mask_b"]))):
            pose_n = gather_rows(c2w_all, (view + sgn).clamp(0, T - 1))
            mm = mask_t * m
            ind_flow, ind_disp = induce_flow(H, W, focal, pose_n, weights_s, pts_ref_s, px, rays, ray_type=rt)
            Ls.add(self._coef(0.01, "temp_static", temp_static), "abs", ind_flow, flow_t, w=mm, norm="weight")
            if batched:
                rays_n, o, xyz = batched[0][k], batched[3][k], batched[1][k][0]
            else:
                rays_n = self.rays_for(ids, poses, focal, uv=grid + flow_t, view_shift=sgn)
                jit, jit_o = rng.jitter(S, rt, rays.device)
                xyz, z, valid = sampleXYZ(self.st, rays_n, S, ray_type=rt, is_train=True, jitter=jit, jitter_outer=jit_o)
                PASSES.update(static=1, static_grad=1)
                o = self.st(rays_n, ts, None, xyz, z, valid, is_train=True, ray_type=rt, rgb=self._dead_rgb())
            _, ind_disp_n = induce_flow(H, W, focal, pose_n, o[4], xyz, px, rays_n, ray_type=rt)
            Ls.add(self._coef(0.04, "temp_static", temp_static), "abs", ind_disp, ind_disp_n, w=mm, norm="weight")
        if self._dyn is None:
            Ls.add(1.0, "identity", frame_depth_loss(to_depth(depth_s), gt_depth, view, T, mask=fg < 0.5,
                                                     coef=c["monodepth_static"] * temp_static, dp=self._dp()))
        else:
            Ls.add(self._coef(1.0, "temp_static", temp_static), "identity",
                   frame_depth_loss(to_depth(depth_s), gt_depth, view, T, mask=fg < 0.5, coef=c["monodepth_static"], dp=self._dp()))
        inv_d = 1.0 / torch.clamp(depth_s, min=1e-6)
        for k, uv_n in enumerate(uv_P34):
            if batched:
                rays_n, o_s, o_d, z = batched[0][2 + k], batched[3][2 + k], batched[4][k], batched[1][2 + k][1]
                if o_d is None:
# ... 240 lines not shown
```

Baseline: 455,200 rays/s.

## Skip saving blending-head activation rows for dynamic passes whose blending is value-only

Adds a SAVE_NO_BLEND flag so the dynamic forward can leave out the blending-branch rows (FB/HB) of the saved activation buffer when no gradient will flow through blending. The saved-row stride becomes a runtime k1_rows in the forward save, the backward read and the weight-gradient jobs, and the training step marks passes B (early stage), C and D as value-only for blending. This is meant to cut per-sample global-memory writes and the saved-buffer footprint. It adds a runtime stride in place of a compile-time constant, and the backward now infers which layout was saved from the buffer size.

```diff
diff --git a/include/rodynrf.h b/include/rodynrf.h
--- a/include/rodynrf.h
+++ b/include/rodynrf.h
@@ -70,6 +70,7 @@
 size_t rdrf_forward_workspace_bytes(int N, int S);
 size_t rdrf_saved_bytes(int kind, int N, int S);
 #define RDRF_SAVE_NO_APP 1
+#define RDRF_SAVE_NO_BLEND 2
 size_t rdrf_saved_bytes_ex(int kind, int N, int S, int flags);
 size_t rdrf_saved_row_bytes(int phase);
 
diff --git a/robust-dynrf_amd/_lib.py b/robust-dynrf_amd/_lib.py
--- a/robust-dynrf_amd/_lib.py
+++ b/robust-dynrf_amd/_lib.py
@@ -13,6 +13,7 @@
 ACTS = {"relu": 0, "softplus": 1}
 HEADS = {"MLP_Fea": 0, "MLP_Fea_TimeEmbedding": 1}
 SAVE_NO_APP = 1
+SAVE_NO_BLEND = 2
 
 fp = C.POINTER(C.c_float)
 
diff --git a/robust-dynrf_amd/csrc/rdrf_bwd.hip b/robust-dynrf_amd/csrc/rdrf_bwd.hip
--- a/robust-dynrf_amd/csrc/rdrf_bwd.hip
+++ b/robust-dynrf_amd/csrc/rdrf_bwd.hip
@@ -1564,7 +1564,7 @@
       const int idx = FLAT ? (act ? n * 32 + s : 0) : n * a.S + (act ? j : 0);
       const bool vld = act && (FEAT || a.valid[idx] != 0);
       const size_t tl = FLAT ? (size_t)n : (size_t)n * tpr + tli;
-      const float* svb = a.sp.act1 + tl * sv::K1_ROWS * 32;
+      const float* svb = a.sp.act1 + tl * a.sp.k1_rows * 32;
       float* gb = a.grows1 + tl * sv::K1G_ROWS * 32;
       if (PHASE == 0) {
         float g_fd, g_fb;
@@ -2847,32 +2847,32 @@
 }
 
 static void add_density_phase_dw(DwJobs& D, const float* grows1, const float* act1, const RdrfDynamicParams* G,
-                                 int T1, bool live_d = true, bool live_b = true, bool small_in_kernel = false) {
-  dw_add(D, grows1, sv::K1G_ROWS, sv::K1G_DZ3, 2, 64, 0, act1, sv::K1_ROWS, 93, 93, G->l3w, G->l3b, nullptr, T1);
+                                 int T1, int k1_rows, bool live_d = true, bool live_b = true, bool small_in_kernel = false) {
+  dw_add(D, grows1, sv::K1G_ROWS, sv::K1G_DZ3, 2, 64, 0, act1, k1_rows, 93, 93, G->l3w, G->l3b, nullptr, T1);
   dw_blk(D, sv::K1_X0, SEG_WARP3_X0, 0);
   dw_blk(D, sv::K1_X0 + 32, SEG_WARP3_X0, 32);
   dw_blk(D, sv::K1_T, SEG_WARP3_T, 0);
-  dw_add(D, grows1, sv::K1G_ROWS, sv::K1G_DZ4, 2, 64, 0, act1, sv::K1_ROWS, 64, 64, G->l4w, G->l4b, nullptr, T1);
+  dw_add(D, grows1, sv::K1G_ROWS, sv::K1G_DZ4, 2, 64, 0, act1, k1_rows, 64, 64, G->l4w, G->l4b, nullptr, T1);
   dw_blk(D, sv::K1_H3, SEG_IDENT, 0);
   dw_blk(D, sv::K1_H3 + 32, SEG_IDENT, 32);
   if (!small_in_kernel) {
-  dw_add(D, grows1, sv::K1G_ROWS, sv::K1G_SM, 1, 3, 0, act1, sv::K1_ROWS, 64, 64, G->l5w, G->l5b, nullptr, T1);
+  dw_add(D, grows1, sv::K1G_ROWS, sv::K1G_SM, 1, 3, 0, act1, k1_rows, 64, 64, G->l5w, G->l5b, nullptr, T1);
   dw_blk(D, sv::K1_H4, SEG_IDENT, 0);
   dw_blk(D, sv::K1_H4 + 32, SEG_IDENT, 32);
   if (live_d) {
-    dw_add(D, grows1, sv::K1G_ROWS, sv::K1G_SM, 1, 1, 3, act1, sv::K1_ROWS, 64, 64, G->dw2, G->db2, nullptr, T1);
+    dw_add(D, grows1, sv::K1G_ROWS, sv::K1G_SM, 1, 1, 3, act1, k1_rows, 64, 64, G->dw2, G->db2, nullptr, T1);
     dw_blk(D, sv::K1_HD, SEG_IDENT, 0);
     dw_blk(D, sv::K1_HD + 32, SEG_IDENT, 32);
   }
   if (live_b) {
-    dw_add(D, grows1, sv::K1G_ROWS, sv::K1G_SM, 1, 1, 4, act1, sv::K1_ROWS, 64, 64, G->bw2, G->bb2, nullptr, T1);
+    dw_add(D, grows1, sv::K1G_ROWS, sv::K1G_SM, 1, 1, 4, act1, k1_rows, 64, 64, G->bw2, G->bb2, nullptr, T1);
     dw_blk(D, sv::K1_HB, SEG_IDENT, 0);
     dw_blk(D, sv::K1_HB + 32, SEG_IDENT, 32);
   }
   }
   for (int head = 0; head < 2; ++head) {
     if (!(head ? live_b : live_d)) continue;
-    dw_add(D, grows1, sv::K1G_ROWS, head ? sv::K1G_DZB : sv::K1G_DZD, 2, 64, 0, act1, sv::K1_ROWS, 152, 152,
+    dw_add(D, grows1, sv::K1G_ROWS, head ? sv::K1G_DZB : sv::K1G_DZD, 2, 64, 0, act1, k1_rows, 152, 152,
            head ? G->bw1 : G->dw1, head ? G->bb1 : G->db1, nullptr, T1);
     const int f0 = head ? sv::K1_FB : sv::K1_FD;
     dw_blk(D, f0, SEG_IDENT72, 0);
@@ -2901,7 +2901,7 @@
   a.g_rays = g_rays; a.g_dists = g_dists; a.g_z = g_z;
   const int saved_kind = carve_saved_bwd(a.sp, saved, saved_bytes, 0, N, S);
   RDRF_CHECK(saved_kind >= 0, -3, "static_bwd: saved buffer too small");
-  RDRF_CHECK(saved_kind == 1 || g_rgb == nullptr, -1,
+  RDRF_CHECK(!(saved_kind & RDRF_SAVE_NO_APP) || g_rgb == nullptr, -1,
              "static_bwd: the forward saved no appearance rows (RDRF_SAVE_NO_APP): no gradient can flow through rgb");
   BwdWs b;
   int rc = carve_bwd(b, ws, ws_bytes, N, S, 0);
@@ -2993,8 +2993,10 @@
   a.small_dw = small_dw ? 1 : 0;
   const int saved_kind = carve_saved_bwd(a.sp, saved, saved_bytes, 1, N, S);
   RDRF_CHECK(saved_kind >= 0, -3, "dynamic_bwd: saved buffer too small");
-  RDRF_CHECK(saved_kind == 1 || g_rgb == nullptr, -1,
+  RDRF_CHECK(!(saved_kind & RDRF_SAVE_NO_APP) || g_rgb == nullptr, -1,
              "dynamic_bwd: the forward saved no appearance rows (RDRF_SAVE_NO_APP): no gradient can flow through rgb");
+  RDRF_CHECK(!(saved_kind & RDRF_SAVE_NO_BLEND) || g_blending == nullptr, -1,
+             "dynamic_bwd: the forward saved no blending rows (RDRF_SAVE_NO_BLEND): no gradient can flow through blending");
   BwdWs b;
   int rc = carve_bwd(b, ws, ws_bytes, N, S, 1);
   if (rc) return rc;
@@ -3093,7 +3095,7 @@
     RDRF_LAUNCH("time_branch_bwd", k_time_branch_bwd, dim3((N + TB_RPB - 1) / TB_RPB), dim3(128), stream, ts, w,
                 N, b.dtout, flat ? (const float*)b.dtp : nullptr, S, G->l1w, G->l1b, G->l2w, G->l2b);
     const bool small_in_kernel = a.small_dw != 0;
-    add_density_phase_dw(D, b.grows1, a.sp.act1, G, (int)t1, g_sigma != nullptr || g_weight != nullptr, g_blending != nullptr,
+    add_density_phase_dw(D, b.grows1, a.sp.act1, G, (int)t1, a.sp.k1_rows, g_sigma != nullptr || g_weight != nullptr, g_blending != nullptr,
                          small_in_kernel);
   }
   rc = dw_launch(D, stream, "dw_dyn");
@@ -3259,7 +3261,7 @@
   RDRF_LAUNCH("feat_dyn_warp_bwd", (k_dyn_density_bwd<1, true>), dim3(g.grid), dim3(g.block), stream, a, w, gw);
   RDRF_LAUNCH("time_branch_bwd", k_time_branch_bwd, dim3((M + TB_RPB - 1) / TB_RPB), dim3(128), stream, t, w, M,
               b.dtout, (const float*)nullptr, 32, G->l1w, G->l1b, G->l2w, G->l2b);
-  add_density_phase_dw(D, b.grows1, a.sp.act1, G, Np, g_density != nullptr, g_blending != nullptr);
+  add_density_phase_dw(D, b.grows1, a.sp.act1, G, Np, a.sp.k1_rows, g_density != nullptr, g_blending != nullptr);
   return dw_launch(D, stream, "feat_dw_dyn");
 }
 
diff --git a/robust-dynrf_amd/csrc/rdrf_fwd.hip b/robust-dynrf_amd/csrc/rdrf_fwd.hip
--- a/robust-dynrf_amd/csrc/rdrf_fwd.hip
+++ b/robust-dynrf_amd/csrc/rdrf_fwd.hip
@@ -100,6 +100,7 @@
   a.act = cfg->act;
   a.ray_type = cfg->ray_type;
   a.static_head = cfg->static_head;
+  a.k1_rows = sv::K1_ROWS;
 }
 
 void dyn_pack_jobs_fwd(PackJobs& J, const RdrfDynamicParams* P) {
@@ -223,6 +224,7 @@
     a.tout = sp.tout;
     a.raw = sp.raw;
     a.act1 = sp.act1;
+    a.k1_rows = sp.k1_rows;
     a.act3 = sp.act3;
   }
   return 0;
@@ -364,7 +366,7 @@
   hipStream_t stream = (hipStream_t)stream_;
   if (N == 0) return 0;
   RDRF_CHECK(P && cfg && N > 0 && S > 0, -1, "dynamic_fwd: bad arguments");
-  RDRF_CHECK((flags & ~RDRF_SAVE_NO_APP) == 0, -1, "dynamic_fwd: unknown flags 0x%x", flags);
+  RDRF_CHECK((flags & ~(RDRF_SAVE_NO_APP | RDRF_SAVE_NO_BLEND)) == 0, -1, "dynamic_fwd: unknown flags 0x%x", flags);
   RDRF_CHECK((size_t)N * S * 3 < (size_t)INT32_MAX, -1, "dynamic_fwd: N * S * 3 must stay below 2^31 (32-bit sample indices): render / train in smaller chunks");
   RDRF_CHECK(vm_ok(P->density, 16, 4) && vm_ok(P->blending, 16, 4) && vm_ok(P->app, 48, 12) && vm_same_grid(P->density, P->blending), -1,
              "dynamic_fwd: only density comps {16,4,4} / app comps {48,12,12}, the planes and lines of a set spanning one grid, are built");
@@ -435,6 +437,7 @@
     RDRF_CHECK(carve_saved_feat(sp, saved, saved_bytes, dynamic, M), -3,
                "features: saved buffer too small: need %zu have %zu", saved_bytes_feat(dynamic, M), saved_bytes);
     a.xw = sp.xw; a.tout = sp.tout; a.raw = sp.raw; a.act1 = sp.act1; a.act3 = sp.act3;
+    a.k1_rows = sp.k1_rows;
   }
   return 0;
 }
diff --git a/robust-dynrf_amd/csrc/rdrf_fwd_dev.hpp b/robust-dynrf_amd/csrc/rdrf_fwd_dev.hpp
--- a/robust-dynrf_amd/csrc/rdrf_fwd_dev.hpp
+++ b/robust-dynrf_amd/csrc/rdrf_fwd_dev.hpp
@@ -482,7 +482,7 @@
     const float xn2 = raw_in ? pz : norm_c(pz, a.box.lo[2], a.box.inv[2]);
     float X0[32];
     fill_x0(X0, xn0, xn1, xn2, t, h);
-    float* svb = (SAVE && a.act1) ? a.act1 + (FLAT ? (size_t)n : (size_t)n * ((a.S + 31) >> 5) + (j0 >> 5)) * sv::K1_ROWS * 32 : nullptr;
+    float* svb = (SAVE && a.act1) ? a.act1 + (FLAT ? (size_t)n : (size_t)n * ((a.S + 31) >> 5) + (j0 >> 5)) * a.k1_rows * 32 : nullptr;
     save_rows<32>(svb, sv::K1_X0, X0, s, h);
     save_rows<8>(svb, sv::K1_X1, X1, s, h);
     save_rows<16>(svb, sv::K1_T, T, s, h);
@@ -561,8 +561,10 @@
 #endif
       float Hd[32];
       acc_relu<2>(Hd, acc);
-      save_rows<36>(svb, sv::K1_FB, Fv, s, h);
-      save_rows<32>(svb, sv::K1_HB, Hd, s, h);
+      if (a.k1_rows > sv::K1_FB) {
+        save_rows<36>(svb, sv::K1_FB, Fv, s, h);
+        save_rows<32>(svb, sv::K1_HB, Hd, s, h);
+      }
       fb = dot_small<32>(Hd, pkw + pk::K1_BLE2, h) + w.bb2[0];
     }
     if constexpr (FEAT) {
diff --git a/robust-dynrf_amd/csrc/rdrf_kernels.hpp b/robust-dynrf_amd/csrc/rdrf_kernels.hpp
--- a/robust-dynrf_amd/csrc/rdrf_kernels.hpp
+++ b/robust-dynrf_amd/csrc/rdrf_kernels.hpp
@@ -24,6 +24,7 @@
   int in_norm;
   float* feat;
   int dynq;
+  int k1_rows;
 };
 
 struct StaticW {
@@ -113,6 +114,7 @@
   float* tout;
   float* raw;
   float* act1;
+  int k1_rows;
   float* act3;
 };
 
@@ -132,17 +134,19 @@
   p.xw = c.take<float>(mp * 3);
   p.tout = c.take<float>(mp * 32);
   p.raw = c.take<float>(mp * 2);
+  p.k1_rows = sv::K1_ROWS;
   p.act1 = dynamic ? c.take<float>(t * sv::K1_ROWS * 32) : nullptr;
   p.act3 = c.take<float>(t * (dynamic ? sv::K3_ROWS : sv::S3_ROWS) * 32);
   return c.ok();
 }
+static inline int k1_rows_for(int flags) { return (flags & RDRF_SAVE_NO_BLEND) ? sv::K1_FB : sv::K1_ROWS; }
 static inline size_t saved_bytes_field(int dynamic, int N, int S, int flags = 0) {
   size_t ns = (size_t)N * S, t1 = (size_t)N * ((S + 31) / 32), t3 = (ns + 31) / 32;
   size_t b = sizeof(SavedHdr) + 256;
   b += ns * 4 + 256;
   b += ns * 3 * 4 + 256 + (size_t)N * 32 * 4 + 256;
   b += ns * 2 * 4 + 256;
-  if (dynamic) b += t1 * sv::K1_ROWS * 32 * 4 + 256;
+  if (dynamic) b += t1 * k1_rows_for(flags) * 32 * 4 + 256;
   if (!(flags & RDRF_SAVE_NO_APP)) b += t3 * (dynamic ? sv::K3_ROWS : sv::S3_ROWS) * 32 * 4 + 256;
   return b;
 }
@@ -154,11 +158,18 @@
   p.xw = c.take<float>(ns * 3);
   p.tout = c.take<float>((size_t)N * 32);
   p.raw = c.take<float>(ns * 2);
-  p.act1 = dynamic ? c.take<float>(t1 * sv::K1_ROWS * 32) : nullptr;
+  p.k1_rows = k1_rows_for(flags);
+  p.act1 = dynamic ? c.take<float>(t1 * p.k1_rows * 32) : nullptr;
   p.act3 = (flags & RDRF_SAVE_NO_APP) ? nullptr : c.take<float>(t3 * (dynamic ? sv::K3_ROWS : sv::S3_ROWS) * 32);
   return c.ok();
 }
 static inline int carve_saved_bwd(SavedPtrs& p, void* saved, size_t bytes, int dynamic, int N, int S) {
-  if (carve_saved(p, saved, bytes, dynamic, N, S, 0)) return 1;
-  return carve_saved(p, saved, bytes, dynamic, N, S, RDRF_SAVE_NO_APP) ? 0 : -1;
+  int best = -1;
+  size_t best_bytes = 0;
+  for (int flags = 0; flags < (dynamic ? 4 : 2); ++flags) {
+    const size_t need = saved_bytes_field(dynamic, N, S, flags);
+    if (need <= bytes && (best < 0 || need > best_bytes)) { best = flags; best_bytes = need; }
+  }
+  if (best < 0 || !carve_saved(p, saved, bytes, dynamic, N, S, best)) return -1;
+  return best;
 }
diff --git a/robust-dynrf_amd/fields.py b/robust-dynrf_amd/fields.py
--- a/robust-dynrf_amd/fields.py
+++ b/robust-dynrf_amd/fields.py
@@ -174,19 +174,31 @@
         SAVE_STATS[(kind, "none")] += 1
         return None, 0
     nbytes = int(L.lib.rdrf_saved_bytes_ex(kind, N, S, flags))
-    SAVE_STATS[(kind, "no_app" if flags & L.SAVE_NO_APP else "full")] += 1
-    SAVE_STATS[(kind, "bytes")] += nbytes
+    mode = "no_app" if flags & L.SAVE_NO_APP else "full"
+    with_blend = int(L.lib.rdrf_saved_bytes_ex(kind, N, S, flags & ~L.SAVE_NO_BLEND))
+    SAVE_STATS[(kind, mode)] += 1
+    SAVE_STATS[(kind, "bytes")] += with_blend
+    if flags & L.SAVE_NO_BLEND:
+        SAVE_STATS[("no_blend", mode)] += 1
+        SAVE_STATS[("no_blend", "bytes")] += nbytes
+        SAVE_STATS[("no_blend", "dropped")] += with_blend - nbytes
     return torch.empty(nbytes, dtype=torch.uint8, device=dev), nbytes
 
 
 _RGB_SUFFIX = {True: "", False: "-norgb", "value": "-valrgb"}
 
 
-def _call_mode(ray_type, rgb):
+def _call_mode(ray_type, rgb, blending=True):
     rgb = rgb if isinstance(rgb, str) else bool(rgb)
     if rgb not in _RGB_SUFFIX:
         raise ValueError(f"forward(..., rgb=...) takes True, False or 'value', not {rgb!r}")
-    return ray_type + _RGB_SUFFIX[rgb] + ("" if torch.is_grad_enabled() else "-nograd")
+    if blending is not True and blending != "value":
+        raise ValueError(f"forward(..., blending=...) takes True or 'value', not {blending!r}")
+    return ray_type + _RGB_SUFFIX[rgb] + ("" if blending is True else "-valblend") + ("" if torch.is_grad_enabled() else "-nograd")
+
+
+def _parse_blend(mode):
+    return mode.replace("-valblend", ""), "value" if "-valblend" in mode else True
 
 
 def _parse_mode(mode):
@@ -279,8 +291,11 @@
         rays, ts, xyz, z, valid = _prep_inputs(rays, ts, xyz, z, valid)
         N, S = z.shape
         dev = z.device
+        ray_type, blend_mode = _parse_blend(ray_type)
         ray_type, rgb_mode, grad_mode = _parse_mode(ray_type)
         want_rgb, flags = rgb_mode is not False, L.SAVE_NO_APP if rgb_mode == "value" else 0
+        if blend_mode == "value":
+            flags |= L.SAVE_NO_BLEND
         rgb = torch.empty(N, S, 3, device=dev) if want_rgb else None
         xyz_prime = torch.empty(N, S, 3, device=dev)
         sigma, weight, dists, blending = (torch.empty(N, S, device=dev) for _ in range(4))
@@ -294,9 +309,11 @@
                                           L.ptr(xyz_prime), L.ptr(rgb), L.ptr(sigma), L.ptr(dists),
                                           L.ptr(saved), C.c_size_t(sbytes), L.ptr(ws),
                                           C.c_size_t(ws.numel()), L.stream_of(z), flags), "rdrf_dynamic_fwd")
-        if rgb_mode == "value":
-            ctx.mark_non_differentiable(rgb)
+        nondiff = ([rgb] if rgb_mode == "value" else []) + ([blending] if blend_mode == "value" else [])
+        if nondiff:
+            ctx.mark_non_differentiable(*nondiff)
         ctx.field, ctx.ray_type, ctx.saved, ctx.want_rgb = field, ray_type, saved, rgb_mode is True
+        ctx.want_blend = blend_mode is True
         ctx.save_for_backward(rays, ts, xyz, z, valid, *params)
         return blending, weight, xyz_prime, rgb, sigma, dists
 
@@ -305,6 +322,8 @@
         rays, ts, xyz, z, valid, *params = ctx.saved_tensors
         if g_rgb is not None and not ctx.want_rgb:
             raise L.RdrfError("forward(..., rgb=False | 'value') saved no appearance rows: no gradient can flow through rgb")
+        if g_blending is not None and not ctx.want_blend:
+            raise L.RdrfError("forward(..., blending='value') saved no blending rows: no gradient can flow through blending")
         need = ctx.needs_input_grad
         if all(g is None for g in (g_blending, g_weight, g_xyz_prime, g_rgb, g_sigma)) and not (need[2] or need[5]):
             ctx.saved = None
@@ -871,11 +890,11 @@
         return t
 
     def forward(self, rays_chunk, ts_chunk, timeembeddings_chunk, xyz_sampled, z_vals, ray_valid,
-                white_bg=True, is_train=False, ray_type="ndc", N_samples=-1, rgb=True):
+                white_bg=True, is_train=False, ray_type="ndc", N_samples=-1, rgb=True, blending=True):
         if timeembeddings_chunk is not None:
             raise NotImplementedError("timeembeddings_chunk is None at every reference call site")
         blending, weight, xyz_prime, rgb, sigma, dists = _DynamicFn.apply(
-            self, _call_mode(ray_type, rgb), rays_chunk, ts_chunk, xyz_sampled, z_vals, ray_valid,
+            self, _call_mode(ray_type, rgb, blending), rays_chunk, ts_chunk, xyz_sampled, z_vals, ray_valid,
             *self._param_list())
         return (None, None, blending, xyz_sampled, weight, xyz_prime, rgb, sigma, z_vals, dists)
 
diff --git a/robust-dynrf_amd/step.py b/robust-dynrf_amd/step.py
--- a/robust-dynrf_amd/step.py
+++ b/robust-dynrf_amd/step.py
@@ -256,7 +256,7 @@
 
 
 def ray_pass(st, dy, rays, ts, n_samples, ray_type, rng, is_train=True, static_grad=False, dynamic=True, rgb_s=True,
-             rgb_d=True):
+             rgb_d=True, blend_d=True):
     jit, jit_o = rng.jitter(n_samples, ray_type, rays.device) if is_train else (None, None)
     xyz, z, valid = sampleXYZ(dy, rays, n_samples, ray_type=ray_type, is_train=is_train, jitter=jit,
                               jitter_outer=jit_o)
@@ -273,7 +273,7 @@
         if dead and rgb_d is True:
             rgb_d = "value"
         with torch.set_grad_enabled(torch.is_grad_enabled() and (not dead or rays.requires_grad or z.requires_grad)):
-            o_d = dy(rays, ts, None, xyz, z, valid, is_train=is_train, ray_type=ray_type, rgb=rgb_d)
+            o_d = dy(rays, ts, None, xyz, z, valid, is_train=is_train, ray_type=ray_type, rgb=rgb_d, blending=blend_d)
         rgb_d, sigma_d, dists, blending, zv = _rgb_or_zeros(o_d[6], o_d[7]), o_d[7], o_d[9], o_d[2], o_d[8]
     else:
         o_d = None
@@ -296,21 +296,22 @@
     return [idxs[i:i + per] for i in range(0, len(idxs), per)]
 
 
-def batched_field(field, rays_list, ts_list, samples, idxs, ray_type, grad=True, rgb=True):
+def batched_field(field, rays_list, ts_list, samples, idxs, ray_type, grad=True, rgb=True, blend=True):
+    kw = {} if blend is True else dict(blending=blend)
     if len(idxs) == 1:
         k = idxs[0]
         with torch.set_grad_enabled(grad and torch.is_grad_enabled()):
-            return [field(rays_list[k], ts_list[k], None, *samples[k], is_train=True, ray_type=ray_type, rgb=rgb)]
+            return [field(rays_list[k], ts_list[k], None, *samples[k], is_train=True, ray_type=ray_type, rgb=rgb, **kw)]
     N = rays_list[idxs[0]].shape[0]
     cat = lambda ts: torch.cat([ts[k] for k in idxs])
     with torch.set_grad_enabled(grad and torch.is_grad_enabled()):
         o = field(cat(rays_list), cat(ts_list), None, *(torch.cat([samples[k][i] for k in idxs]) for i in range(3)),
-                  is_train=True, ray_type=ray_type, rgb=rgb)
+                  is_train=True, ray_type=ray_type, rgb=rgb, **kw)
     parts = [None if t is None else t.view(len(idxs), N, *t.shape[1:]).unbind(0) for t in o]
     return [tuple(None if pt is None else pt[j] for pt in parts) for j in range(len(idxs))]
 
 
-def ray_passes(st, dy, rays_list, ts_list, n_samples, ray_type, rng, groups, rgb=None):
+def ray_passes(st, dy, rays_list, ts_list, n_samples, ray_type, rng, groups, rgb=None, blend=None):
     P, N, dev = len(rays_list), rays_list[0].shape[0], rays_list[0].device
     PASSES.update(static=P, dynamic=P)
     samples, coins = [], []
@@ -320,6 +321,7 @@
         coins.append(rng.coin())
     ns = N * samples[0][1].shape[1]
     rgb = [True] * P if rgb is None else list(rgb)
+    blend = [True] * P if blend is None else list(blend)
     o_ss, o_ds = [None] * P, [None] * P
     runs, lo = [], 0
     want_s = [bool(f) for f in rgb]
@@ -334,8 +336,10 @@
     for group in groups:
         assert list(group) == list(range(group[0], group[0] + len(group)))
         assert all(rgb[k] == rgb[group[0]] for k in group), "a dynamic group must agree on its colour flag"
+        assert all(blend[k] == blend[group[0]] for k in group), "a dynamic group must agree on its blending flag"
         for g in batch_groups(group, ns):
-            for k, o in zip(g, batched_field(dy, rays_list, ts_list, samples, g, ray_type, rgb=rgb[group[0]])):
+            for k, o in zip(g, batched_field(dy, rays_list, ts_list, samples, g, ray_type, rgb=rgb[group[0]],
+                                              blend=blend[group[0]])):
                 o_ds[k] = o
     out = []
     for p in range(P):
@@ -476,9 +480,10 @@
             rays_n_of = {sgn: self.rays_for(ids, poses_d, focal_d, uv=grid + b["flow_f" if sgn > 0 else "flow_b"], view_shift=sgn)
                          for sgn in (1, -1)}
             groups = [[0], [1, 2, 3]] if not late else [[0], [1], [2, 3]]
+            blend_B = True if late else "value"
             pA, pB, pC, pD = ray_passes(self.st, self.dy, [rays_d, rays_d, rays_n_of[1], rays_n_of[-1]],
                                         [ts, b["ts_rand"], ts + dt, ts - dt], S, rt, rng, groups,
-                                        rgb=[True] + [self._dead_rgb()] * 3)
+                                        rgb=[True] + [self._dead_rgb()] * 3, blend=[True, blend_B, "value", "value"])
             osA, oA, outA, xyzA = pA
             batched = {"B": pB, 1: pC, -1: pD}
         else:
@@ -508,7 +513,8 @@
         if w_dist > 0:
             Ld.add(k_dist, "identity", distloss_rays(outA[11], oA[8].detach(), 1.0 / S))
         _, oB, outB, _ = batched["B"] if batched else ray_pass(self.st, self.dy, rays_d, b["ts_rand"], S, rt, rng,
-                                                               rgb_s=self._dead_rgb(), rgb_d=self._dead_rgb())
+                                                               rgb_s=self._dead_rgb(), rgb_d=self._dead_rgb(),
+                                                               blend_d=True if late else "value")
         if late:
             Ld.add(0.01, "identity", skewed(outB[12]))
             Ld.add(0.01, "abs", outB[12])
@@ -535,7 +541,7 @@
             else:
                 rays_n = self.rays_for(ids, poses_d, focal_d, uv=grid + flow_t, view_shift=sgn)
                 _, oN, outN, _ = ray_pass(self.st, self.dy, rays_n, ts + sgn * dt, S, rt, rng, rgb_s=self._dead_rgb(),
-                                          rgb_d=self._dead_rgb())
+                                          rgb_d=self._dead_rgb(), blend_d="value")
             _, ind_disp_n = induce_flow(H, W, focal_d, pose_n, outN[11], oN[3], px, rays_n, ray_type=rt)
             Ld.add(0.04 * temp, "abs", ind_disp, ind_disp_n, w=mask_t, norm="weight")
             if w_dist > 0:
```

After: 456,700 rays/s, median of 2. No clear change (+0.3%).
